# numericalEFT/MCIntegration.jl

Measured on AMD Instinct MI355X. Metric: Msamples/sec (whole node), 16-D Gaussian :vegas, higher is better.
Workload: dtype f64

## Files before the change

### include/mci.h

```cpp
#ifndef MCI_H
#define MCI_H

#include <stdint.h>

#ifdef __cplusplus
extern "C" {
#endif

#define MCI_OK 0
#define MCI_ERR_INVALID 1
#define MCI_ERR_HIP 2
#define MCI_ERR_COMPILE 3
#define MCI_ERR_NORMALIZATION 4
#define MCI_ERR_HISTOGRAM 5
#define MCI_ERR_COMM 6
#define MCI_ERR_NO_DEVICE 7

enum { MCI_CONTINUOUS = 0, MCI_DISCRETE = 1, MCI_FERMIK = 2 };
enum { MCI_VEGAS = 0, MCI_VEGASMC = 1, MCI_MCMC = 2 };
enum { MCI_VEGAS_PERSISTENT = 3 };
enum { MCI_VEGASMC_LANES = 5, MCI_MCMC_LANES = 6 };
enum { MCI_VEGAS_STRAT = 7 };
enum { MCI_VEGAS_SWEEP = 8 };
enum { MCI_VEGAS_SWEEP_LEAVES = 9 };
enum { MCI_VEGAS_SWEEP_STRAT = 10 };
enum { MCI_VEGASMC_SWEEP = 11 };
enum { MCI_MCMC_SWEEP = 12 };
enum { MCI_VEGASMC_SWEEP_CARRY = 13, MCI_MCMC_SWEEP_CARRY = 14 };
enum { MCI_SWEEP_ONE_GRID = 0, MCI_SWEEP_ALL_LEAVES = 1 };

typedef struct mci_ctx mci_ctx;
typedef struct mci_problem mci_problem;

typedef struct {
    int32_t kind;
    int32_t pool;
    double lower, upper;
    int32_t npoints;
    double alpha;
    int32_t adapt;
    const double *init;
} mci_leaf_desc;

typedef struct {
    int32_t nleaf;
    const mci_leaf_desc *leaves;
    int32_t npool;
    int32_t nintegrand;
    const int32_t *dof;
    const int32_t *obs_nbin;
    const int32_t *obs_bin_draw;
    const int32_t *neighbor_offsets;
    const int32_t *neighbor_list;
    int32_t ncomp;
} mci_problem_desc;

typedef struct {
    int32_t solver;
    int64_t neval;
    int32_t niter;
    int64_t block;
    int32_t ignore;
    int32_t adapt;
    double gamma;
    int64_t measurefreq;
    uint64_t seed;
    int64_t nchain;
    int32_t first_iteration;
    double thermal_ratio;
    const double *reweight_goal;
} mci_integrate_args;

typedef struct {
    int32_t niter, nobs;
    double *iter_mean;
    double *iter_std;
    double *mean;
    double *stdev;
    double *chi2;
    int64_t neval;
    double seconds;
    double *visited;
    int32_t correlated;
    int32_t warmup;
} mci_result;

int mci_ctx_create(int32_t device, mci_ctx **out);
int mci_ctx_destroy(mci_ctx *ctx);
const char *mci_last_error(void);
int mci_device_count(int32_t *count);
void *mci_ctx_stream(mci_ctx *ctx);

int mci_comm_unique_id(void *id128);
int mci_comm_init(mci_ctx *ctx, int32_t rank, int32_t nranks, const void *id128);
int mci_comm_rank(const mci_ctx *ctx, int32_t *rank, int32_t *nranks);
int mci_comm_sum(mci_problem *prob, double *v, int32_t n);

int mci_problem_create(mci_ctx *ctx, const mci_problem_desc *desc, mci_problem **out);
int mci_problem_destroy(mci_problem *prob);
int mci_set_integrand_source(mci_problem *prob, const char *body, const double *userdata, int32_t nuserdata);
typedef int (*mci_host_integrand_fn)(const double *x, double *w, int64_t n, int32_t ndraw, int32_t nw, void *user);
int mci_set_integrand_host(mci_problem *prob, mci_host_integrand_fn fn, void *user);
typedef int (*mci_host_integrand_idx_fn)(const int32_t *idx, const double *x, double *w, int64_t n, int32_t ndraw, int32_t ncomp, void *user);
int mci_set_integrand_host_indexed(mci_problem *prob, mci_host_integrand_idx_fn fn, void *user);
int mci_set_measure_source(mci_problem *prob, const char *body);
typedef int (*mci_host_measure_fn)(const double *x, const double *relw, int64_t n, int64_t stride, int32_t ndraw, int32_t nw,
                                   int64_t block, double *obs, int32_t nobs, void *user);
int mci_set_measure_host(mci_problem *prob, mci_host_measure_fn fn, void *user);
typedef int (*mci_host_measure_idx_fn)(const int32_t *idx, const double *x, const double *relw, int64_t n, int64_t stride, int32_t ndraw,
                                       int32_t ncomp, int64_t block, double *obs, int32_t nobs, void *user);
int mci_set_measure_host_indexed(mci_problem *prob, mci_host_measure_idx_fn fn, void *user);
int mci_compile(mci_problem *prob);
int mci_compile_solver(mci_problem *prob, int32_t solver);
int mci_kernel_code_object(mci_problem *prob, int32_t solver, char *buf, int32_t n);
int mci_set_launch(mci_problem *prob, int32_t threads_per_workgroup, int32_t workgroups_per_block);
int mci_problem_info(const mci_problem *prob, int32_t *ndraw, int32_t *nobs, int64_t *packed_size,
                     int32_t *table_mode, int64_t *lds_bytes);
int mci_get_histogram_copies(const mci_problem *prob, int32_t *copies);

int mci_iteration_run(mci_problem *prob, int32_t solver, int64_t neval_per_block, int64_t block_lo,
                      int64_t block_hi, int32_t iteration, uint64_t seed, int64_t measurefreq, int64_t nchain,
                      double thermal_ratio);
int mci_iteration_reduce(mci_problem *prob);
int mci_iteration_finish(mci_problem *prob, int32_t solver, int64_t block_total, int32_t adapt, double gamma,
                         double *mean, double *std);
int mci_check_status(mci_problem *prob);
int mci_integrate(mci_problem *prob, const mci_integrate_args *args, mci_result *result);
int mci_integrate_sweep(mci_problem *prob, const mci_integrate_args *args, int32_t npoint, const double *userdata, const uint64_t *seeds,
                        const double *maps_in, double *maps_out, mci_result *results, double *iter_mean, double *iter_std,
                        int32_t *status);
int mci_sweep_supported(const mci_problem *prob, const mci_integrate_args *args, char *why, int32_t n);
int mci_set_sweep_leaves(mci_problem *prob, int32_t mode);
int mci_set_sweep_chain_carry(mci_problem *prob, int32_t on);
int mci_get_sweep_chain_carry(const mci_problem *prob, int32_t *on);
int mci_sweep_map_doubles(const mci_problem *prob, int32_t *n);
int mci_integrate_sweep_strat(mci_problem *prob, const mci_integrate_args *args, int32_t npoint, const double *userdata, const uint64_t *seeds,
                              const double *maps_in, double *maps_out, const double *d_in, double *d_out, int64_t *counts_out,
                              mci_result *results, double *iter_mean, double *iter_std, int32_t *status);
int mci_sweep_strat_supported(const mci_problem *prob, const mci_integrate_args *args, char *why, int32_t n);
int mci_sweep_strat_doubles(const mci_problem *prob, const mci_integrate_args *args, int64_t *ncube);
int mci_integrate_sweep_chains(mci_problem *prob, const mci_integrate_args *args, int32_t npoint, const double *userdata, const uint64_t *seeds,
                               const double *maps_in, double *maps_out, const double *reweight_in, double *reweight_out, double *pa_out,
                               mci_result *results, double *iter_mean, double *iter_std, int32_t *status);
int mci_sweep_chains_supported(const mci_problem *prob, const mci_integrate_args *args, char *why, int32_t n);
int mci_integrate_sweep_mcmc(mci_problem *prob, const mci_integrate_args *args, int32_t npoint, const double *userdata, const uint64_t *seeds,
                             const double *maps_in, double *maps_out, const double *reweight_in, double *reweight_out, double *pa_out,
                             uint64_t *holds_out, mci_result *results, double *iter_mean, double *iter_std, int32_t *status);
int mci_sweep_mcmc_supported(const mci_problem *prob, const mci_integrate_args *args, char *why, int32_t n);

int mci_get_hold_histogram(mci_problem *prob, uint64_t *out64);
int mci_mcmc_launch_valid(mci_problem *prob, int32_t *valid, int32_t *warm, int64_t *chain_len, int64_t *hold_max);
int mci_iteration_discard(mci_problem *prob);
int mci_get_iteration_log(mci_problem *prob, int32_t nrows, double *out);
int mci_get_block_means(mci_problem *prob, int32_t rows, double *out, int64_t *nblocks, int32_t *carried);
int mci_reset_block_log(mci_problem *prob);
int mci_reserve_iteration_log(mci_problem *prob, int32_t rows);
int mci_get_packed(mci_problem *prob, double *out, int64_t n);
int mci_set_packed(mci_problem *prob, const double *in, int64_t n);
void *mci_packed_device_ptr(mci_problem *prob);
int mci_get_grid(mci_problem *prob, int32_t leaf, double *out, int32_t n);
int mci_set_grid(mci_problem *prob, int32_t leaf, const double *grid, int32_t n);
int mci_get_distribution(mci_problem *prob, int32_t leaf, double *distribution, double *accumulation, int32_t k);
int mci_set_distribution(mci_problem *prob, int32_t leaf, const double *distribution, int32_t k);
int mci_get_reweight(mci_problem *prob, double *out, int32_t n);
int mci_set_reweight(mci_problem *prob, const double *in, int32_t n);
int mci_set_reweight_goal(mci_problem *prob, const double *goal, int32_t n);
int mci_get_acceptance(mci_problem *prob, double *propose, double *accept, int32_t n);
int mci_save_state(mci_problem *prob, const char *path);
int mci_load_state(mci_problem *prob, const char *path);
int mci_set_rng_bits(mci_problem *prob, int32_t bits);
int mci_set_rng_rounds(mci_problem *prob, int32_t rounds);
int mci_set_train_walk(mci_problem *prob, int32_t mode);
int mci_set_deterministic(mci_problem *prob, int32_t on);
int mci_set_chain_carry(mci_problem *prob, int32_t mode);
int mci_set_stratification(mci_problem *prob, int32_t ndim, const int32_t *nstrat, double beta, int64_t max_nhcube);
int mci_set_stratification_carry(mci_problem *prob, int32_t on);
int mci_get_strat_carry(const mci_problem *prob, int32_t *on, int32_t *how);
int mci_set_stratification_off(mci_problem *prob);
int mci_get_stratification(const mci_problem *prob, int32_t *nstrat, int64_t *ncube, double *beta);
int mci_get_strat_counts(mci_problem *prob, int64_t *n_h, int64_t n);
int mci_strat_plan(int64_t neval, int32_t ndim, int64_t max_nhcube, int32_t *nstrat);
// ... 47 lines not shown
```

### mcintegration.jl_amd/csrc/mci_host_check.h

```cpp

namespace {
struct CheckLayout {
    std::vector<mci::CheckDraw> draw;
    std::vector<mci::CheckIntegrand> intg;
};
bool vegas_check_covers(const mci_problem *p) {
    const auto &s = p->shape;
    if (s.host_integrand || s.host_measure || s.ntile != 1 || p->has_fermik || p->strat.on) return false;
    for (int i = 0; i < s.ni; ++i)
        if (s.ncomp != 1 && s.obs_bin_draw[(size_t)i] >= 0) return false;
    return s.ndraw >= 1 && s.ndraw <= 64;
}
void vegas_check_layout(const mci_problem *p, CheckLayout *out) {
    const auto &s = p->shape;
    CheckLayout &L = *out;
    for (int k = 0; k < s.ndraw; ++k) {
        const int leaf = s.draw_leaf[(size_t)k];
        mci::CheckDraw d{};
        d.kind = s.leaf_kind[(size_t)leaf];
        d.off = s.leaf_eoff[(size_t)leaf];
        d.doff = s.leaf_doff[(size_t)leaf];
        d.nbin = s.leaf_nbin[(size_t)leaf];
        d.boff = s.leaf_boff[(size_t)leaf];
        d.hist = (s.leaf_adapt[(size_t)leaf] != 0 && s.cover_mask[(size_t)k] != 0ull) ? 1 : 0;
        d.scale = d.kind == 0 ? (double)d.nbin : 1.0;
        d.lower = s.leaf_lower[(size_t)leaf];
        L.draw.push_back(d);
    }
    for (int i = 0; i < s.ni; ++i) {
        mci::CheckIntegrand g{};
        g.own = s.own_mask[(size_t)i];
        g.obs_off = s.obs_off[(size_t)i];
        g.obs_nbin = s.obs_nbin[(size_t)i];
        g.obs_bin_draw = s.obs_bin_draw[(size_t)i];
        L.intg.push_back(g);
    }
}
struct DevFree {
    void *p = nullptr;
    ~DevFree() { if (p) (void)hipFree(p); }
};
}

static int sample_dump_device(mci_problem *p, int32_t iteration, uint64_t seed, int64_t first_index, int64_t n);

static int vegas_make_conservative(mci_problem *p, int slot) {
    p->vegas.make_conservative(p->deterministic);
    if (!p->deterministic) p->shape.hcopy = 1;
    p->kernel[MCI_VEGAS].drop();
    p->kernel[kSlotVegasAny].drop();
    p->vegas_check_done[0] = p->vegas_check_done[1] = false;
    return compile_solver(p, slot);
}

static int vegas_check_reference(mci_problem *p, int32_t iteration, uint64_t seed, int64_t nevalperblock, int64_t block_lo, int64_t nblocks,
                                 int64_t measurefreq, const double *hx, const double *hjac, const double *hw, double *packed, int64_t *bad,
                                 bool hist_offsets) {
    const auto &s = p->shape;
    if (!vegas_check_covers(p)) return fail(MCI_ERR_INVALID, "this layout has no static :vegas check (host closures, several histogram tiles, stratification)");
    if (nblocks < 1 || nevalperblock < 1 || nblocks * nevalperblock > 1024 || measurefreq < 1) return fail(MCI_ERR_INVALID, "the static :vegas check runs 1..1024 samples per launch");
    HIPCHK(hipSetDevice(p->ctx->device));
    hipStream_t st = p->ctx->stream;
    CheckLayout L;
    vegas_check_layout(p, &L);
    const int nw = s.ni * s.ncomp;
    const int64_t n = nevalperblock, per = s.ndraw + 1 + nw;
    const size_t nraw = (size_t)nblocks * s.ncols + (size_t)(s.nbin ? s.nbin : 1);
    DevFree d_draw, d_intg, d_raw, d_bad, d_in;
    HIPCHK(hipMalloc(&d_draw.p, L.draw.size() * sizeof(mci::CheckDraw)));
    HIPCHK(hipMalloc(&d_intg.p, L.intg.size() * sizeof(mci::CheckIntegrand)));
    HIPCHK(hipMalloc(&d_raw.p, nraw * sizeof(double)));
    HIPCHK(hipMalloc(&d_bad.p, 2 * sizeof(unsigned long long)));
    HIPCHK(hipMemcpyAsync(d_draw.p, L.draw.data(), L.draw.size() * sizeof(mci::CheckDraw), hipMemcpyHostToDevice, st));
    HIPCHK(hipMemcpyAsync(d_intg.p, L.intg.data(), L.intg.size() * sizeof(mci::CheckIntegrand), hipMemcpyHostToDevice, st));
    HIPCHK(hipMemsetAsync(d_raw.p, 0, nraw * sizeof(double), st));
    HIPCHK(hipMemsetAsync(d_bad.p, 0, 2 * sizeof(unsigned long long), st));
    if (hx) HIPCHK(hipMalloc(&d_in.p, (size_t)(nblocks * n * per) * sizeof(double)));
    mci::CheckArgs a{};
    a.draw = (const mci::CheckDraw *)d_draw.p;
    a.intg = (const mci::CheckIntegrand *)d_intg.p;
    a.ndraw = s.ndraw;
    a.ni = s.ni;
    a.ncomp = s.ncomp;
    a.nobs = s.nobs;
    a.ncols = s.ncols;
    a.rng_bits = s.rng_bits;
    a.rng_rounds = s.rng_rounds;
    a.with_obs = s.measure_body.empty() ? 1 : 0;
    fill_tables(p, a);
    a.seed = seed;
    a.iteration = (unsigned)iteration;
    a.neval_per_block = nevalperblock;
    a.measurefreq = measurefreq;
    a.hist = (double *)d_raw.p + (size_t)nblocks * s.ncols;
    a.bad = (unsigned long long *)d_bad.p;
    const int64_t total = nblocks * n;
    if (hx) {
        double *in = (double *)d_in.p;
        HIPCHK(hipMemcpyAsync(in, hx, (size_t)total * s.ndraw * sizeof(double), hipMemcpyHostToDevice, st));
        HIPCHK(hipMemcpyAsync(in + total * s.ndraw, hjac, (size_t)total * sizeof(double), hipMemcpyHostToDevice, st));
        HIPCHK(hipMemcpyAsync(in + total * (s.ndraw + 1), hw, (size_t)total * nw * sizeof(double), hipMemcpyHostToDevice, st));
        a.x = in;
    } else {
        if (int rc = sample_dump_device(p, iteration, seed, block_lo * nevalperblock, total)) return rc;
        p->check_launches += 1;
        a.x = p->d_dump;
    }
    a.jac = a.x + total * s.ndraw;
    a.w = a.jac + total;
    a.block_lo = block_lo;
    a.n = total;
    a.cols = (double *)d_raw.p;
    hipLaunchKernelGGL(mci::k_check_vegas, dim3((unsigned)((total + 255) / 256)), dim3(256), 0, st, a);
    HIPCHK(hipGetLastError());
    p->check_launches += 1;
    std::vector<double> raw(nraw);
    unsigned long long hbad[2] = {0ull, 0ull};
    HIPCHK(hipMemcpyAsync(raw.data(), d_raw.p, nraw * sizeof(double), hipMemcpyDeviceToHost, st));
    HIPCHK(hipMemcpyAsync(hbad, d_bad.p, sizeof(hbad), hipMemcpyDeviceToHost, st));
    HIPCHK(hipStreamSynchronize(st));
    if (bad) {
        bad[0] = (int64_t)hbad[0];
        bad[1] = (int64_t)hbad[1];
    }
    const int nobs = s.nobs, cnorm = nobs, cneval = nobs + 1, cvis = nobs + 2;
    for (int64_t i = 0; i < p->packed_n; ++i) packed[i] = 0.0;
    double norm = 1.0e-10, neval = 0.0;
    for (int64_t b = 0; b < nblocks; ++b) {
        const double *row = raw.data() + (size_t)b * s.ncols;
        const double nb = row[cnorm] + 1.0e-10;
        for (int o = 0; o < nobs; ++o) {
            const double m = row[o] / nb;
            packed[o] += m;
            packed[nobs + o] += m * m;
        }
        norm += nb;
        neval += row[cneval];
    }
    packed[2 * nobs] = norm;
    packed[2 * nobs + 1] = neval;
    for (int i = 0; i < s.ni + 1; ++i) {
        double v = 1.0e-8;
        for (int64_t b = 0; b < nblocks; ++b) v += raw[(size_t)b * s.ncols + cvis + i] + 1.0e-8;
        packed[2 * nobs + 2 + i] = v;
    }
    for (int i = 0; i < s.nbin; ++i) packed[p->nstat + i] = (hist_offsets ? (double)(nblocks + 1) * 1.0e-10 : 0.0) + raw[(size_t)nblocks * s.ncols + i];
    for (int e = 0; e < 2 * p->npa && p->nstat + s.nbin + e < p->packed_n; ++e)
        packed[p->nstat + s.nbin + e] = (double)(nblocks + 1) * (e < p->npa ? 1.0e-8 : 1.0e-10);
    return MCI_OK;
}

static int vegas_check_round(mci_problem *p, int slot, int64_t npb, int64_t block_lo, int64_t nb, int32_t iteration, uint64_t seed, int64_t mf, PackedDiff *df,
                             int64_t *bad, bool *differs) {
    std::vector<double> got((size_t)p->packed_n, 0.0), ref((size_t)p->packed_n, 0.0);
    p->check_slot = slot;
    int rc = mci_iteration_run(p, MCI_VEGAS, npb, block_lo, block_lo + nb, iteration, seed, mf, 1, 0.0);
    p->check_slot = -1;
    if (!rc) p->check_launches += 1;
    if (!rc) rc = mci_get_packed(p, got.data(), p->packed_n);
    if (!rc) rc = vegas_check_reference(p, iteration, seed, npb, block_lo, nb, mf, nullptr, nullptr, nullptr, ref.data(), bad, false);
    if (rc) return rc;
    const size_t skip = p->shape.measure_body.empty() ? 0 : (size_t)(2 * p->shape.nobs);
    compare_packed(got.data(), ref.data(), (size_t)p->nstat, (size_t)p->packed_n, skip, df, (long)p->shape.nbin);
    *differs = df->bad != 0 || bad[0] != 0 || bad[1] != 0;
    return MCI_OK;
}

static int vegas_self_check(mci_problem *p, int slot, int64_t nevalperblock, int64_t block_lo, int64_t block_hi, int32_t iteration, uint64_t seed,
                            int64_t measurefreq) {
    const int u = slot == kSlotVegasAny ? 1 : 0;
    const int64_t nb = block_hi - block_lo < 2 ? block_hi - block_lo : 2, npb = nevalperblock < 512 ? nevalperblock : 512;
    const int64_t mf = measurefreq * 4 <= npb ? measurefreq : 1;
    const mci_problem::LaunchState saved = p->launch;
    const int kernel_timing = p->kernel_timing;
    int rc = flush_merge(p);
    if (rc) return rc;
    int h_status[4] = {0, 0, 0, 0};
    HIPCHK(hipStreamSynchronize(p->ctx->stream));
    HIPCHK(hipMemcpy(h_status, p->d_status, sizeof(h_status), hipMemcpyDeviceToHost));
    p->in_self_check = true;
    p->kernel_timing = 0;
    if (!p->shape.measure_body.empty()) p->vegas_check_flags |= 1;
    int state = 0;
    for (int round = 0; round < 2 && !rc; ++round) {
        PackedDiff df;
        int64_t bad[2] = {0, 0};
        bool differs = false;
        const std::string object = p->kernel[slot].code_object;
        rc = vegas_check_round(p, slot, npb, block_lo, nb, iteration, seed, mf, &df, bad, &differs);
        if (rc) break;
        if (!differs) {
            state = round == 0 ? 1 : -1;
            bool takes = false;
            for (int k = 0; k < p->shape.ndraw; ++k)
                takes = takes || (p->shape.leaf_adapt[(size_t)p->shape.draw_leaf[(size_t)k]] != 0 && p->shape.cover_mask[(size_t)k] != 0ull);
            if (takes && !(df.hist_top > 0.0)) {
                p->vegas_check_flags |= 4;
                if (round == 0) state = 0;
                break;
            }
            const std::string id = mcijit::compiler_id() + "\n";
            mcijit::write_file_atomic(object + ".ok", id.data(), id.size());
            break;
        }
        fprintf(stderr, "mci: the :vegas sample kernel of this problem (%s%s) does not reproduce the library's static :vegas kernel on a %lld-block, "
                        "%lld-sample check: %ld of %lld packed entries differ (first at %ld; statistics %ld, histogram %ld), draws of %lld samples and "
                        "Jacobians of %lld differ.  A miscompiled code object -- %s; mci_vegas_check_status reports %d.\n",
                object.c_str(), round ? ", the conservative layout" : "", (long long)nb, (long long)npb, df.bad, (long long)p->packed_n, df.first_bad,
                df.bad_sec[0], df.bad_sec[1], (long long)bad[0], (long long)bad[1],
                round ? "no layout of this unit agrees, its results are not to be trusted" : "the problem compiles its :vegas units again in the plain layout (plain loop, one histogram copy)",
                round ? -2 : -1);
        state = -2;
        if (round == 0) {
            rc = vegas_make_conservative(p, slot);
        }
    }
    p->in_self_check = false;
    p->launch = saved;
    p->kernel_timing = kernel_timing;
    if (p->d_status) (void)hipMemcpy(p->d_status, h_status, sizeof(h_status), hipMemcpyHostToDevice);
    p->merge.hist_no_offset = 0;
    p->vegas_check_done[u] = true;
    if (rc) {
        fprintf(stderr, "mci: the self-check of this problem's :vegas code object (%s) could not run: %s -- nothing was verified "
                        "(mci_vegas_check_status stays %d)\n", p->kernel[slot].code_object.c_str(), mci_last_error(), state == -2 ? -2 : 0);
        p->merge_pending = false;
        if (state == -2) p->vegas_check_state[u] = -2;
        return MCI_OK;
    }
    p->vegas_check_state[u] = state;
    return MCI_OK;
}

static int vegas_check_gate(mci_problem *p, int slot, int64_t nevalperblock, int64_t block_lo, int64_t block_hi, int32_t iteration, uint64_t seed,
                            int64_t measurefreq) {
    const int u = slot == kSlotVegasAny ? 1 : 0;
    const bool force = g_over.vegas_self_check.on && g_over.vegas_self_check.v == 1;
    if (g_over.vegas_self_check.on && g_over.vegas_self_check.v == 0) return MCI_OK;
    if (!vegas_check_covers(p) || p->ctx->offline) {
        p->vegas_check_done[u] = true;
        return MCI_OK;
    }
    if (!force && access((p->kernel[slot].code_object + ".ok").c_str(), F_OK) == 0) {
        if (p->vegas_check_state[u] == 0) {
            p->vegas_check_state[u] = 1;
            p->vegas_check_flags |= 2;
        }
        p->vegas_check_done[u] = true;
        return MCI_OK;
    }
    return vegas_self_check(p, slot, nevalperblock, block_lo, block_hi, iteration, seed, measurefreq);
}

int mci_vegas_check_status(const mci_problem *p, int32_t *status, int32_t *flags) {
    if (!p || !status) return fail(MCI_ERR_INVALID, "NULL argument");
    const int a = p->vegas_check_state[0], b = p->vegas_check_state[1];
    *status = (a < 0 || b < 0) ? (a < b ? a : b) : (a > b ? a : b);
    if (flags) *flags = p->vegas_check_flags;
    return MCI_OK;
}

int mci_debug_vegas_check(mci_problem *p, int32_t iteration, uint64_t seed, int64_t nevalperblock, int64_t block_lo, int64_t nblocks, int64_t measurefreq,
                          const double *x, const double *jac, const double *w, double *packed, int64_t *bad) {
    if (!p || !packed) return fail(MCI_ERR_INVALID, "NULL argument");
    if (p->ctx->offline) return fail(MCI_ERR_NO_DEVICE, "offline context");
    if ((x || jac || w) && !(x && jac && w)) return fail(MCI_ERR_INVALID, "x, jac and w come together");
    int rc = flush_merge(p);
    if (rc) return rc;
    return vegas_check_reference(p, iteration, seed, nevalperblock, block_lo, nblocks, measurefreq, x, jac, w, packed, bad, true);
}

int mci_debug_vegas_check_launches(const mci_problem *p, int64_t *launches) {
    if (!p || !launches) return fail(MCI_ERR_INVALID, "NULL argument");
    *launches = p->check_launches;
    return MCI_OK;
}

int mci_debug_vegas_check_layout(const mci_problem *p, int32_t *head, int32_t *draws, double *scales, uint64_t *own, int32_t *obs) {
    if (!p || !head) return fail(MCI_ERR_INVALID, "NULL argument");
    const auto &s = p->shape;
    CheckLayout L;
    vegas_check_layout(p, &L);
    head[0] = s.ndraw;
    head[1] = s.ni;
    head[2] = s.ncomp;
    head[3] = s.nobs;
    head[4] = s.ncols;
    head[5] = s.nbin;
    head[6] = vegas_check_covers(p) ? 1 : 0;
    head[7] = s.measure_body.empty() ? 1 : 0;
    for (size_t k = 0; k < L.draw.size(); ++k) {
        if (draws) {
            const mci::CheckDraw &d = L.draw[k];
            const int v[6] = {d.kind, d.off, d.doff, d.nbin, d.boff, d.hist};
            for (int j = 0; j < 6; ++j) draws[6 * k + j] = v[j];
        }
        if (scales) scales[k] = L.draw[k].scale;
    }
    for (size_t i = 0; i < L.intg.size(); ++i) {
        if (own) own[i] = L.intg[i].own;
        if (obs) {
            obs[3 * i] = L.intg[i].obs_off;
            obs[3 * i + 1] = L.intg[i].obs_nbin;
            obs[3 * i + 2] = L.intg[i].obs_bin_draw;
        }
    }
    return MCI_OK;
}
```

### mcintegration.jl_amd/csrc/mci_host_iteration.h

```cpp

static int reserve_launch_buffers(mci_problem *p, const LaunchRequest &rq, const LaunchPlan &pl) {
    const auto &s = p->shape;
    int rc = ensure_capacity(p, pl.nrows, rq.nblocks);
    if (!rc && rq.solver != MCI_VEGAS) rc = p->d_part_pa.reserve(pl.nrows * 2 * p->npa);
    if (rc || !pl.split) return rc;
    const int64_t words = p->tdraw_words > 0 ? p->tdraw_words : 1, bytes = parked_bytes_per_sample(p);
    const int64_t nsamp = rq.nblocks * pl.chunk_len;
    if (nsamp > p->cap_tile) {
        tile_release(p);
        const size_t wbytes = (((size_t)nsamp * s.ni * sizeof(double)) + 255) & ~(size_t)255;
        if ((rc = tile_alloc(p, wbytes + (size_t)nsamp * words * sizeof(uint32_t)))) return rc;
        p->d_tile_bins = (uint32_t *)((char *)p->d_tile_w + wbytes);
        p->cap_tile = nsamp;
    }
    p->launch.last_split_chunks = pl.nchunks;
    p->launch.last_split_bytes = nsamp * bytes;
    return MCI_OK;
}

static mci::BatchArgs request_args(const mci_problem *p, const LaunchRequest &rq, const LaunchPlan &pl) {
    mci::BatchArgs a{};
    fill_batch(p, a);
    a.part_pa = p->d_part_pa;
    a.seed = rq.seed;
// ... 185 lines not shown
    if ((rc = p->d_hx.reserve(n * s.ndraw)) || (rc = p->d_hw.reserve(n * s.ni * s.ncomp)) || (rc = p->h_hx.reserve(n * s.ndraw)) ||
        (rc = p->h_hw.reserve(n * s.ni * s.ncomp)))
        return rc;
    if (rq.solver == MCI_VEGAS) {
    mci::DumpArgs d{};
    fill_tables(p, d);
    d.ud = p->d_ud;
    d.x = p->d_hx;
    d.soa = 1;
    d.seed = rq.seed;
    d.iteration = (mci::u32)rq.iteration;
    d.first_index = rq.block_lo * rq.nevalperblock;
    d.n = n;
    void *dargs[] = {&d};
    const unsigned dgrid = (unsigned)((n + 255) / 256 < 4096 ? (n + 255) / 256 : 4096);
    hipStream_t hs = p->ctx->stream;
    HIPCHK(hipModuleLaunchKernel(p->kernel[kSlotDump].f, dgrid, 1, 1, 256, 1, 1, (unsigned)p->lds_bytes, hs, dargs, nullptr));
    HIPCHK(hipMemcpyAsync(p->h_hx, p->d_hx, (size_t)n * s.ndraw * sizeof(double), hipMemcpyDeviceToHost, hs));
    HIPCHK(hipStreamSynchronize(hs));
    if ((rc = eval_host_integrand(p, nullptr, p->h_hx, p->h_hw, n))) return rc;
    HIPCHK(hipMemcpyAsync(p->d_hw, p->h_hw, (size_t)n * s.ni * s.ncomp * sizeof(double), hipMemcpyHostToDevice, hs));
    }
    a.host_w = p->d_hw;
    return MCI_OK;
}

static int prepare_host_measure(mci_problem *p, const LaunchRequest &rq, const LaunchPlan &pl, mci::BatchArgs &a) {
    const auto &s = p->shape;
    const int nw = s.ni * s.ncomp;
    const int64_t n = rq.nblocks * pl.hm_n > 0 ? rq.nblocks * pl.hm_n : 1;
    if ((double)n * (double)(s.ndraw + nw + 1) * 8.0 > 8.0 * 1024 * 1024 * 1024)
        return fail(MCI_ERR_INVALID, "a host measure over %lld records of %d doubles per launch (more than 8 GiB): lower neval, raise measurefreq "
                                     "or give the measure as device source (mci_set_measure_source)", (long long)n, s.ndraw + nw);
    int rc;
    if ((rc = p->d_mx.reserve(n * s.ndraw)) || (rc = p->d_mrelw.reserve(n * nw)) || (rc = p->d_midx.reserve(n)) || (rc = p->h_mx.reserve(n * s.ndraw)) ||
        (rc = p->h_mrelw.reserve(n * nw)) || (rc = p->h_midx.reserve(n)) || (rc = p->d_mobs.reserve(rq.nblocks * s.nobs)))
        return rc;
    a.host_mx = p->d_mx;
    a.host_relw = p->d_mrelw;
    a.host_midx = p->d_midx;
    a.hm_first = pl.hm_first;
    a.hm_count = pl.hm_count;
    a.hm_stride = rq.nblocks * pl.hm_n;
    if (rq.solver != MCI_VEGAS) {
        HIPCHK(hipMemsetAsync(p->d_mx, 0, (size_t)n * s.ndraw * sizeof(double), p->ctx->stream));
        HIPCHK(hipMemsetAsync(p->d_mrelw, 0, (size_t)n * pl.hm_rows * sizeof(double), p->ctx->stream));
        HIPCHK(hipMemsetAsync(p->d_midx, 0xFF, (size_t)n * sizeof(int32_t), p->ctx->stream));
    }
    return MCI_OK;
}

static int prepare_cursor(mci_problem *p, const LaunchRequest &rq, const LaunchPlan &pl, mci::BatchArgs &a) {
    mci::CursorRule r;
    r.units = (mci::u64)((rq.nevalperblock + 127) >> 7);
    r.waves = (mci::u32)(pl.wpb * (pl.T / 64));
    r.log2_big = (mci::u32)(g_over.cursor_log2_big.on && g_over.cursor_log2_big.v >= 1 && g_over.cursor_log2_big.v <= 16 ? g_over.cursor_log2_big.v : mci_problem::kCursorLog2Big);
    r.ones = (mci::u32)(g_over.cursor_ones.on && g_over.cursor_ones.v >= 1 && g_over.cursor_ones.v <= 4096 ? g_over.cursor_ones.v : mci_problem::kCursorOnes);
    if (rq.nblocks != p->cursor_nblocks) {
        if (int rc = p->d_cursor.reserve(rq.nblocks * mci::kCursorStride)) return rc;
        HIPCHK(hipMemsetAsync(p->d_cursor, 0, (size_t)rq.nblocks * mci::kCursorStride * sizeof(unsigned long long), p->ctx->stream));
        p->cursor_nblocks = rq.nblocks;
        p->cursor_base = 0;
    }
    a.cursor = p->d_cursor;
    a.cursor_base = p->cursor_base;
    a.cursor_log2_big = r.log2_big;
    a.cursor_ones = r.ones;
    p->cursor_base += mci::cursor_tickets(r) + r.waves;
    return MCI_OK;
}

static int launch_host_closure_steps(mci_problem *p, const LaunchRequest &rq, const LaunchPlan &pl, mci::BatchArgs &a, hipFunction_t f) {
    const auto &s = p->shape;
    hipStream_t st = p->ctx->stream;
    void *args[] = {&a};
    int rc;
    const int64_t nc = rq.nblocks * pl.nchain, steps = rq.nevalperblock / pl.nchain;
    const int nw = s.ni * s.ncomp, nd = s.ndraw;
    if (nc >= ((int64_t)1 << 31) || steps + pl.nburn >= ((int64_t)1 << 31) - 1) return fail(MCI_ERR_INVALID, "too many chains or steps for the host-closure path");
    if ((rc = p->d_hstep.reserve(nc * (int64_t)((3 * nd + nw + 4) * sizeof(double) + (2 * nd + 7) * sizeof(int)) + 16)) || (rc = p->h_hidx.reserve(nc + 1))) return rc;
    {
        double *dp = (double *)p->d_hstep.get();
        a.hs.cx = dp; dp += (size_t)nd * nc;
        a.hs.cprob = dp; dp += (size_t)nd * nc;
        a.hs.pprob = dp; dp += (size_t)nd * nc;
        a.hs.cw = dp; dp += (size_t)nw * nc;
        a.hs.cprobability = dp; dp += nc;
        a.hs.pprop = dp; dp += nc;
        a.hs.puacc = dp; dp += nc;
        a.hs.cwabs = dp; dp += nc;
        int *ip = (int *)dp;
        a.hs.cbin = ip; ip += (size_t)nd * nc;
        a.hs.pbin = ip; ip += (size_t)nd * nc;
        a.hs.pvi = ip; ip += nc;
        a.hs.ccurr = ip; ip += nc;
        a.hs.cit = ip; ip += nc;
        a.hs.ctr = ip; ip += nc;
        a.hs.pnew = ip; ip += nc;
        a.hs.put = ip; ip += nc;
        a.hs.hidx = ip; ip += nc;
        a.hs.done = ip;
    }
    a.hs.hx = p->d_hx;
    a.hs.nc = nc;
    a.hs.steps = steps;
    HIPCHK(hipMemsetAsync(p->d_part_cols, 0, (size_t)pl.nrows * s.ncols * sizeof(double), st));
    if (pl.hist_lds && s.nbin > 0) HIPCHK(hipMemsetAsync(p->d_part_hist, 0, (size_t)pl.nrows * s.nbin * sizeof(double), st));
    HIPCHK(hipMemsetAsync(p->d_part_pa, 0, (size_t)pl.nrows * 2 * p->npa * sizeof(double), st));
    HIPCHK(hipMemsetAsync(a.hs.done, 0, sizeof(int), st));
    if (rq.solver == MCI_VEGASMC) {
        for (int64_t ne = 0; ne <= steps + 1; ++ne) {
            a.hs.ne = ne;
            HIPCHK(hipModuleLaunchKernel(f, (unsigned)pl.nwg, 1, 1, (unsigned)pl.T, 1, 1, (unsigned)solver_lds(p, rq.solver), st, args, nullptr));
            if (ne > steps) break;
            HIPCHK(hipMemcpyAsync(p->h_hx, p->d_hx, (size_t)nc * nd * sizeof(double), hipMemcpyDeviceToHost, st));
            HIPCHK(hipStreamSynchronize(st));
            if ((rc = eval_host_integrand(p, nullptr, p->h_hx, p->h_hw, nc))) return rc;
            HIPCHK(hipMemcpyAsync(p->d_hw, p->h_hw, (size_t)nc * nw * sizeof(double), hipMemcpyHostToDevice, st));
        }
    } else {
        const int64_t limit = steps + pl.nburn + 2 + 10000;
        for (int64_t ne = 0;; ++ne) {
            a.hs.ne = ne;
            HIPCHK(hipModuleLaunchKernel(f, (unsigned)pl.nwg, 1, 1, (unsigned)pl.T, 1, 1, (unsigned)solver_lds(p, rq.solver), st, args, nullptr));
            HIPCHK(hipMemcpyAsync(p->h_hidx, a.hs.hidx, (size_t)(nc + 1) * sizeof(int32_t), hipMemcpyDeviceToHost, st));
            HIPCHK(hipMemcpyAsync(p->h_hx, p->d_hx, (size_t)nc * nd * sizeof(double), hipMemcpyDeviceToHost, st));
            HIPCHK(hipStreamSynchronize(st));
            if (p->h_hidx[nc] >= nc) break;
            if (ne > limit) return fail(MCI_ERR_INVALID, "host-closure :mcmc chains did not finish (%d of %lld)", (int)p->h_hidx[nc], (long long)nc);
            if ((rc = eval_host_integrand(p, p->h_hidx, p->h_hx, p->h_hw, nc))) return rc;
            HIPCHK(hipMemcpyAsync(p->d_hw, p->h_hw, (size_t)nc * s.ncomp * sizeof(double), hipMemcpyHostToDevice, st));
        }
    }
    return MCI_OK;
}

static int launch_replay(mci_problem *p, const LaunchRequest &rq, const LaunchPlan &pl, mci::BatchArgs &a) {
    const auto &s = p->shape;
    void *args[] = {&a};
    HIPCHK(hipModuleLaunchKernel(p->f_tiles[rq.kern == kSlotVegasAny ? 1 : 0], (unsigned)(((pl.hist_rows + 7) / 8) * 8 * (s.ntile - (s.split_all ? 0 : 1))), 1, 1, (unsigned)pl.T, 1, 1, (unsigned)p->lds_bytes, p->ctx->stream, args, nullptr));
    return MCI_OK;
}

static int launch_sample_chunks(mci_problem *p, const LaunchRequest &rq, const LaunchPlan &pl, mci::BatchArgs &a, hipFunction_t f) {
    hipStream_t st = p->ctx->stream;
    void *args[] = {&a};
    int rc;
    for (int64_t c = 0; c < pl.nchunks; ++c) {
        if (pl.nchunks > 1) {
            a.chunk_lo = c * pl.chunk_len;
            a.chunk_hi = a.chunk_lo + pl.chunk_len < rq.nevalperblock ? a.chunk_lo + pl.chunk_len : rq.nevalperblock;
            a.accum = c > 0 ? 1 : 0;
        }
        HIPCHK(hipModuleLaunchKernel(f, (unsigned)pl.nwg, 1, 1, (unsigned)pl.T_launch, 1, 1, (unsigned)solver_lds(p, rq.solver), st, args, nullptr));
        if (pl.split && c + 1 < pl.nchunks && (rc = launch_replay(p, rq, pl, a))) return rc;
    }
    return MCI_OK;
}

static int finish_host_measure(mci_problem *p, const LaunchRequest &rq, const LaunchPlan &pl) {
    const auto &s = p->shape;
    hipStream_t st = p->ctx->stream;
    const int64_t n = rq.nblocks * pl.hm_n;
    const int nw = s.ni * s.ncomp, nc = s.ncomp;
    std::vector<double> obs((size_t)rq.nblocks * s.nobs, 0.0);
    if (n > 0 && !p->in_self_check) {
        HIPCHK(hipMemcpyAsync(p->h_mx, p->d_mx, (size_t)n * s.ndraw * sizeof(double), hipMemcpyDeviceToHost, st));
        HIPCHK(hipMemcpyAsync(p->h_mrelw, p->d_mrelw, (size_t)n * pl.hm_rows * sizeof(double), hipMemcpyDeviceToHost, st));
        if (rq.solver == MCI_MCMC) HIPCHK(hipMemcpyAsync(p->h_midx, p->d_midx, (size_t)n * sizeof(int32_t), hipMemcpyDeviceToHost, st));
        HIPCHK(hipStreamSynchronize(st));
        const double *relw = p->h_mrelw;
        if (rq.solver == MCI_MCMC && p->hmeas_fn) {
            p->h_mtmp.assign((size_t)n * nw, 0.0);
            for (int64_t i = 0; i < n; ++i)
                if (p->h_midx[i] >= 0)
                    for (int q = 0; q < nc; ++q) p->h_mtmp[(size_t)(p->h_midx[i] * nc + q) * n + i] = p->h_mrelw[(size_t)q * n + i];
            relw = p->h_mtmp.data();
        }
        if (rq.solver != MCI_MCMC && p->hmeas_idx_fn) p->h_mitmp.resize((size_t)pl.hm_n);
        const bool squeeze = rq.solver == MCI_VEGAS && rq.measurefreq > 1;
        const int64_t keep = squeeze ? rq.nevalperblock / rq.measurefreq : pl.hm_n;
        std::vector<double> sx, sw;
        if (squeeze) {
            sx.resize((size_t)(keep > 0 ? keep : 1) * s.ndraw);
            sw.resize((size_t)(keep > 0 ? keep : 1) * nw);
        }
        for (int64_t b = 0; b < rq.nblocks; ++b) {
            const int64_t off = b * pl.hm_n;
            double *ob = obs.data() + (size_t)b * s.nobs;
            int hrc = 0;
            if (squeeze) {
                for (int k = 0; k < s.ndraw; ++k)
                    for (int64_t j = 0; j < keep; ++j) sx[(size_t)k * keep + j] = p->h_mx[(size_t)k * n + off + (j + 1) * rq.measurefreq - 1];
                for (int q = 0; q < nw; ++q)
                    for (int64_t j = 0; j < keep; ++j) sw[(size_t)q * keep + j] = relw[(size_t)q * n + off + (j + 1) * rq.measurefreq - 1];
                if (p->hmeas_fn) hrc = p->hmeas_fn(sx.data(), sw.data(), keep, keep, s.ndraw, nw, rq.block_lo + b, ob, s.nobs, p->hmeas_user);
                else {
                    p->h_mitmp.resize((size_t)(keep > 0 ? keep : 1));
                    for (int j = 0; j < s.ni && !hrc; ++j) {
                        std::fill(p->h_mitmp.begin(), p->h_mitmp.end(), (int32_t)j);
                        hrc = p->hmeas_idx_fn(p->h_mitmp.data(), sx.data(), sw.data() + (size_t)j * nc * keep, keep, keep, s.ndraw, nc, rq.block_lo + b, ob,
                                              s.nobs, p->hmeas_user);
                    }
                }
            } else if (p->hmeas_fn) {
                hrc = p->hmeas_fn(p->h_mx + off, relw + off, pl.hm_n, n, s.ndraw, nw, rq.block_lo + b, ob, s.nobs, p->hmeas_user);
            } else if (rq.solver == MCI_MCMC) {
                hrc = p->hmeas_idx_fn(p->h_midx + off, p->h_mx + off, relw + off, pl.hm_n, n, s.ndraw, nc, rq.block_lo + b, ob, s.nobs, p->hmeas_user);
            } else {
                for (int j = 0; j < s.ni && !hrc; ++j) {
                    std::fill(p->h_mitmp.begin(), p->h_mitmp.end(), (int32_t)j);
                    hrc = p->hmeas_idx_fn(p->h_mitmp.data(), p->h_mx + off, relw + (size_t)j * nc * n + off, pl.hm_n, n, s.ndraw, nc, rq.block_lo + b, ob,
                                          s.nobs, p->hmeas_user);
                }
            }
            if (hrc) return fail(MCI_ERR_INVALID, "the host measure failed (%d)", hrc);
        }
    }
    HIPCHK(hipMemcpyAsync(p->d_mobs, obs.data(), obs.size() * sizeof(double), hipMemcpyHostToDevice, st));
    hipLaunchKernelGGL(mci::k_add_host_obs, dim3((unsigned)((rq.nblocks * s.nobs + 255) / 256)), dim3(256), 0, st, p->d_mobs, (int)rq.nblocks, s.nobs, s.ncols, pl.wpb,
                       p->d_part_cols);
    HIPCHK(hipGetLastError());
    HIPCHK(hipStreamSynchronize(st));
    return MCI_OK;
}

static int queue_merge(mci_problem *p, const LaunchRequest &rq, const LaunchPlan &pl, const unsigned long long *hold_hist) {
    const auto &s = p->shape;
    hipStream_t st = p->ctx->stream;
    int rc;
    const int nb256 = (s.nbin + 255) / 256;
    if (pl.hist_lds && s.nbin > 0 && !pl.atomic_flush)
        hipLaunchKernelGGL(mci::k_hist_stage1, dim3(nb256, mci_problem::kGroups), dim3(256), 0, st, p->d_part_hist, (int)pl.hist_rows, s.nbin,
                           (int)mci_problem::kGroups, p->d_stage1);
    HIPCHK(hipGetLastError());
    mci::MergeArgs &m = p->merge;
    m = merge_args(p, rq.nblocks, pl.wpb, pl.nrows);
    m.use_ghist = (pl.hist_lds && !pl.atomic_flush) ? 0 : pl.atomic_flush ? pl.ghist_buffers : 1;
    m.part_pa = rq.solver != MCI_VEGAS ? p->d_part_pa.get() : nullptr;
    m.hist_no_offset = (p->in_self_check && p->check_slot >= 0) ? 1 : 0;
    m.hold = hold_hist;
    if (rq.solver != MCI_VEGAS && !p->in_self_check) {
        const int64_t stride = rq.nblocks * s.nobs;
        if (stride != p->launch.blk_stride || rq.block_lo != p->launch.blk_lo) {
            p->launch.blk_rows = 0;
            p->launch.blk_carried = 0;
            p->launch.blk_stride = stride;
            p->launch.blk_lo = rq.block_lo;
        }
        if ((rc = grow_block_log(p, p->launch.blk_rows + 1))) return rc;
        m.block_means = p->d_blocklog + (size_t)p->launch.blk_rows * stride;
        p->launch.blk_rows += 1;
        p->launch.blk_carried += p->launch.last_carried ? 1 : 0;
    }
    p->merge_pending = true;
    return MCI_OK;
}

int mci_iteration_run(mci_problem *p, int32_t solver, int64_t nevalperblock, int64_t block_lo, int64_t block_hi,
                      int32_t iteration, uint64_t seed, int64_t measurefreq, int64_t nchain, double thermal_ratio) {
    if (p->ctx->offline) return fail(MCI_ERR_NO_DEVICE, "offline context: no device to run on");
    if (solver != MCI_VEGAS && solver != MCI_VEGASMC && solver != MCI_MCMC) return fail(MCI_ERR_INVALID, "Solver %d is not supported!", solver);
    if (measurefreq <= 0) return fail(MCI_ERR_INVALID, "measurefreq must be positive");
    const int64_t nblocks = block_hi - block_lo;
    if (nblocks < 1 || nevalperblock < 1) return fail(MCI_ERR_INVALID, "empty iteration");
    if (p->has_fermik && solver != MCI_MCMC) return fail(MCI_ERR_INVALID, "FermiK variables work with solver=:mcmc only");
    if (p->strat.on) {
        if (solver != MCI_VEGAS) return fail(MCI_ERR_INVALID, "stratification works with solver = :vegas only (mci_set_stratification_off first)");
        return strat_run(p, nevalperblock, block_lo, block_hi, iteration, seed, measurefreq);
    }
    const int kern = (p->in_self_check && p->check_slot >= 0 && solver == MCI_VEGAS) ? p->check_slot : kslot(solver, measurefreq);
    const LaunchRequest rq{solver, nevalperblock, block_lo, block_hi, nblocks, iteration, seed, measurefreq, thermal_ratio, nchain <= 0, kern};
    int rc = (rq.solver == MCI_VEGAS || p->deterministic || p->shape.host_integrand || p->spec_lanes == 1) ? compile_solver(p, rq.kern) : MCI_OK;
    if (rc) return rc;
    if (rq.solver == MCI_VEGAS && !p->in_self_check && !p->vegas_check_done[rq.kern == kSlotVegasAny ? 1 : 0] &&
        (rc = vegas_check_gate(p, rq.kern, rq.nevalperblock, rq.block_lo, rq.block_hi, rq.iteration, rq.seed, rq.measurefreq)))
        return rc;
    if (rq.solver == MCI_VEGAS && (rc = compile_solver(p, rq.kern))) return rc;
    if (rq.solver == MCI_VEGAS && p->shape.host_integrand && (rc = ensure_dump(p))) return rc;
    if ((rc = flush_merge(p))) return rc;
    HIPCHK(hipSetDevice(p->ctx->device));
    const auto &s = p->shape;
    LaunchPlan pl;
    pl.nchain = nchain;
    plan_threads(p, rq, pl);
    pl.units = nevalperblock;
    if (rq.solver != MCI_VEGAS && (rq.block_hi > 4096 || rq.iteration >= 131072 || rq.iteration < 0))
        return fail(MCI_ERR_INVALID, "chain solvers address a chain by (block < 4096, iteration < 131072): got block_hi=%lld, iteration=%d",
                    (long long)rq.block_hi, (int)rq.iteration);
    pl.may_carry = plan_may_carry(p, rq);
    if (solver == MCI_VEGASMC) rc = plan_vegasmc_chains(p, rq, g_over, pl);
    else if (solver == MCI_MCMC) {
        if (!(rq.thermal_ratio >= 0.0)) return fail(MCI_ERR_INVALID, "thermal_ratio must be non-negative");
        if (rq.auto_chains && (rc = hold_consume(p))) return rc;
        rc = plan_mcmc_chains(p, rq, pl);
    } else pl.nchain = 1;
    if (rc) return rc;
    plan_spec_lanes(p, rq, pl);
    pl.T_launch = pl.T;
    if (pl.G > 1 && p->spec_state[rq.solver - 1] < 0) pl.G = 1;
    if (pl.G > 1) {
        rc = compile_spec(p, rq.solver);
        if (rc == MCI_ERR_COMPILE && p->spec_lanes == -1) {
            fprintf(stderr, "mci: the several-lanes-per-chain kernel of this problem did not compile; one lane per chain instead\n%s\n", mci_last_error());
            p->spec_state[rq.solver - 1] = -2;
            pl.G = 1;
        } else if (rc) return rc;
    }
    if (pl.G > 1 && !p->in_self_check && ((p->spec_need_check[rq.solver - 1] && !(g_over.spec_self_check.on && g_over.spec_self_check.v == 0)) ||
                                       (g_over.spec_self_check.on && g_over.spec_self_check.v == 1 && p->spec_state[rq.solver - 1] == 0))) {
        if ((rc = spec_self_check(p, rq.solver, pl.G, rq.nevalperblock, rq.block_lo, rq.block_hi, rq.iteration, rq.seed, rq.measurefreq, rq.thermal_ratio))) return rc;
        if (p->spec_state[rq.solver - 1] < 0) pl.G = 1;
    }
    if (pl.G > 1) {
        if ((rc = spec_upload(p, rq.solver, pl.G, p->spec_accept, p->spec_maxacc))) return rc;
        pl.spec_maxacc = p->spec_tab_maxacc;
        pl.units = pl.nchain * pl.G;
        pl.T_launch = pl.units >= 256 ? 256 : (int)((pl.units + 63) / 64) * 64;
    }
    if (pl.G == 1 && (rc = compile_solver(p, rq.kern))) return rc;
    p->launch.last_spec_lanes = pl.G;
    p->launch.last_spec_maxacc = pl.spec_maxacc;
    plan_grid(p, rq, pl);
    if (const int candidate = plan_cursor_candidate(p, rq, g_over, pl)) {
        int resident = 0;
        if (candidate == 1) pl.cursor = true;
        else if ((rc = cursor_resident(p, rq.kern, pl.T, &resident))) return rc;
        else plan_cursor_grid(rq, resident, pl);
    }
    plan_tiles(p, rq, g_over, pl);
    plan_replay(p, rq, pl);
    plan_host_measure(p, rq, pl);
    plan_timing(p, rq, pl);
    if ((rc = reserve_launch_buffers(p, rq, pl))) return rc;
    mci::BatchArgs a = request_args(p, rq, pl);
    if (solver != MCI_VEGAS && (rc = prepare_carried_chains(p, rq, pl, a))) return rc;
    if ((rc = prepare_chain_tables(p, rq, pl, a))) return rc;
    geometry_args(p, rq, pl, a);
    if (s.host_integrand && (rc = prepare_host_integrand(p, rq, pl, a))) return rc;
    if (s.host_measure && (rc = prepare_host_measure(p, rq, pl, a))) return rc;
    if (pl.cursor && (rc = prepare_cursor(p, rq, pl, a))) return rc;
    p->launch.last_cursor = pl.cursor;
    hipFunction_t f = p->kernel[pl.G > 1 ? (rq.solver == MCI_VEGASMC ? kSlotVegasmcSpec : kSlotMcmcSpec) : rq.kern].f;
    hipStream_t st = p->ctx->stream;
    const int slot = (int)(p->launch.launches % mci_problem::kEvRing);
    p->launch.time_this_launch = pl.time_this_launch;
    if (p->launch.time_this_launch && rq.solver == MCI_VEGAS) {
        if (!p->d_clocks) {
            if ((rc = p->d_clocks.reserve(2 * mci_problem::kEvRing))) return rc;
            HIPCHK(hipMemsetAsync(p->d_clocks, 0, (size_t)2 * mci_problem::kEvRing * sizeof(unsigned long long), st));
        }
        a.clock_out = p->d_clocks + 2 * slot;
    }
    if (p->launch.time_this_launch) HIPCHK(hipEventRecord(p->evs[2 * slot], st));
    if (solver != MCI_VEGAS && s.host_integrand) rc = launch_host_closure_steps(p, rq, pl, a, f);
    else rc = launch_sample_chunks(p, rq, pl, a, f);
    if (rc) return rc;
    if (rq.solver == MCI_MCMC) p->launch.hold_measured = a.hold_hist != nullptr;
    if (a.hold_hist && rq.auto_chains && (rc = hold_publish(p, rq.nevalperblock / pl.nchain, rq.solver != MCI_VEGAS && p->launch.last_carried))) return rc;
    if (pl.split && (rc = launch_replay(p, rq, pl, a))) return rc;
    if (p->launch.time_this_launch) HIPCHK(hipEventRecord(p->evs[2 * slot + 1], st));
    p->launch.ev_valid[slot] = p->launch.time_this_launch;
    p->launch.clock_valid[slot] = a.clock_out != nullptr && !pl.split && s.ntile == 1;
    p->launch.launches += 1;
    if (s.host_measure && (rc = finish_host_measure(p, rq, pl))) return rc;
    record_launch(p, nblocks * nevalperblock, pl.nwg, pl.T_launch, nblocks);
    if (solver != MCI_VEGAS) p->launch.last_nchain = pl.nchain;
    return queue_merge(p, rq, pl, a.hold_hist);
}

static int flush_merge(mci_problem *p) {
    if (!p->merge_pending) return MCI_OK;
    p->merge_pending = false;
    HIPCHK(hipSetDevice(p->ctx->device));
    const int nb256 = (p->shape.nbin + 255) / 256;
    hipLaunchKernelGGL(mci::k_finalize, dim3(nb256 + 1 + (2 * p->npa + 3) / 4), dim3(256), 0, p->ctx->stream, p->merge);
    HIPCHK(hipGetLastError());
    return MCI_OK;
}

int mci_iteration_reduce(mci_problem *p) {
    if (p->ctx->offline) return fail(MCI_ERR_NO_DEVICE, "offline context");
    if (!p->ctx->comm) return MCI_OK;
    int rc = flush_merge(p);
    if (rc) return rc;
    const bool timed = p->launch.time_this_launch;
    const int slot = (int)(p->reduces % mci_problem::kCevRing);
    if (timed) {
        if (p->cevs.empty()) {
            p->cevs.resize(2 * mci_problem::kCevRing);
            for (auto &e : p->cevs) HIPCHK(hipEventCreate(&e));
        }
        HIPCHK(hipEventRecord(p->cevs[2 * slot], p->ctx->stream));
    }
    const size_t count = (size_t)p->packed_n + (p->launch.hold_deferred ? 64 : 0);
    int r = g_rccl.AllReduce(p->d_packed, p->d_packed, count, kNcclFloat64, kNcclSum, p->ctx->comm, p->ctx->stream);
    if (r) return fail(MCI_ERR_COMM, "ncclAllReduce: %s", g_rccl.GetErrorString ? g_rccl.GetErrorString(r) : "?");
    p->ctx->collectives += 1;
    p->ctx->last_count = (long long)count;
    if (p->launch.hold_deferred && (rc = hold_publish_reduced(p))) return rc;
    if (timed) HIPCHK(hipEventRecord(p->cevs[2 * slot + 1], p->ctx->stream));
    p->cev_valid[slot] = timed;
    p->reduces += 1;
    return MCI_OK;
}

int mci_comm_collectives(const mci_ctx *c, int64_t *calls, int64_t *last_count) {
    if (!c) return fail(MCI_ERR_INVALID, "NULL argument");
    if (calls) *calls = c->collectives;
    if (last_count) *last_count = c->last_count;
    return MCI_OK;
}

int mci_external_reduce_done(mci_problem *p) {
    if (!p) return fail(MCI_ERR_INVALID, "NULL argument");
    if (p->ctx->offline) return fail(MCI_ERR_NO_DEVICE, "offline context");
    if (!p->launch.hold_ext_pending) return MCI_OK;
    p->launch.hold_ext_pending = false;
    HIPCHK(hipSetDevice(p->ctx->device));
    return hold_publish_reduced(p);
}

int mci_reduce_size(const mci_problem *p, int64_t *n) {
    if (!p || !n) return fail(MCI_ERR_INVALID, "NULL argument");
    *n = p->packed_n + 64;
    return MCI_OK;
}

int mci_comm_times_ms(mci_problem *p, float *ms, int32_t n, int32_t *got) {
    if (!p || !ms || !got) return fail(MCI_ERR_INVALID, "NULL argument");
    if (p->ctx->offline) return fail(MCI_ERR_NO_DEVICE, "offline context");
    HIPCHK(hipStreamSynchronize(p->ctx->stream));
    int64_t have = p->reduces < mci_problem::kCevRing ? p->reduces : mci_problem::kCevRing;
    if (have > n) have = n;
    int32_t k = 0;
    for (int64_t i = 0; i < have; ++i) {
        const int slot = (int)((p->reduces - have + i) % mci_problem::kCevRing);
        if (!p->cev_valid[slot]) continue;
        float t = 0.f;
        HIPCHK(hipEventElapsedTime(&t, p->cevs[2 * slot], p->cevs[2 * slot + 1]));
        ms[k++] = t;
    }
    *got = k;
    return MCI_OK;
}

static int launch_train(mci_problem *p, int do_train, int do_reweight, double gamma, double *log_row) {
    const auto &s = p->shape;
    int maxn = 1;
    for (auto &L : p->leaves) maxn = L.nbin > maxn ? L.nbin : maxn;
    mci::TrainArgs a{};
    fill_train(p, a);
    a.iter_log_row = log_row;
    a.goal = p->h_goal.empty() ? nullptr : p->d_goal.get();
    a.do_reweight = do_reweight;
    a.gamma = gamma;
    a.do_train = do_train;
    if (do_train) p->ntrain += 1;
    a.serial_walk = p->train_serial >= 0 ? p->train_serial : (p->launch.last_samples == 0 || p->launch.last_samples >= mci_problem::kSerialWalkSamples) ? 1 : 0;
    if (p->debug_wrong_decision && a.serial_walk == 1) a.serial_walk = 3;
    a.maxn = maxn;
    a.spare = (size_t)(mci::train_lds_doubles(maxn) + mci::train_spare_doubles(maxn)) * sizeof(double) <= (size_t)kTrainLdsMax ? 1 : 0;
    const size_t sm = (size_t)(mci::train_lds_doubles(maxn) + (a.spare ? mci::train_spare_doubles(maxn) : maxn)) * sizeof(double);
    const unsigned tt = maxn > 256 ? 512u : 256u;
    if (sm > 64 * 1024 && !p->train_lds_raised) {
        HIPCHK(hipFuncSetAttribute((const void *)mci::k_train, hipFuncAttributeMaxDynamicSharedMemorySize, (int)kTrainLdsMax));
        HIPCHK(hipFuncSetAttribute((const void *)mci::k_finish, hipFuncAttributeMaxDynamicSharedMemorySize, (int)kTrainLdsMax));
        p->train_lds_raised = true;
    }
    if (p->merge_pending) {
        p->merge_pending = false;
        hipLaunchKernelGGL(mci::k_finish, dim3(s.nleaf + 1 + (2 * p->npa + 3) / 4), dim3(tt), sm, p->ctx->stream, p->merge, a);
    } else {
        hipLaunchKernelGGL(mci::k_train, dim3(s.nleaf + 1), dim3(tt), sm, p->ctx->stream, a);
    }
    HIPCHK(hipGetLastError());
    return MCI_OK;
}

static int grow_iteration_log(mci_problem *p, int64_t need) {
    return grow_keeping(p, p->d_iterlog, need, 64, p->nstat);
}

int mci_reserve_iteration_log(mci_problem *p, int32_t rows) {
    if (!p || rows < 0) return fail(MCI_ERR_INVALID, "bad argument");
    if (p->ctx->offline) return fail(MCI_ERR_NO_DEVICE, "offline context");
    HIPCHK(hipSetDevice(p->ctx->device));
    return grow_iteration_log(p, (int64_t)p->log_row + rows);
}

int mci_iteration_finish(mci_problem *p, int32_t solver, int64_t block_total, int32_t adapt, double gamma, double *mean, double *std) {
    if (p->ctx->offline) return fail(MCI_ERR_NO_DEVICE, "offline context");
    HIPCHK(hipSetDevice(p->ctx->device));
    const auto &s = p->shape;
    if (int grc = grow_iteration_log(p, (int64_t)p->log_row + 1)) return grc;
    double *row = p->d_iterlog + (size_t)p->log_row * p->nstat;
    const bool strat = p->strat.last_run;
    int rc = launch_train(p, adapt ? 1 : 0, (solver == MCI_VEGASMC || solver == MCI_MCMC) ? 1 : 0, gamma, row);
    if (rc) return rc;
    if (strat && (rc = strat_finish(p, row, adapt))) return rc;
    p->log_row += 1;
    if (mean || std) {
        std::vector<double> h(p->nstat);
        HIPCHK(hipMemcpyAsync(h.data(), row, (size_t)p->nstat * sizeof(double), hipMemcpyDeviceToHost, p->ctx->stream));
        if ((rc = check_status(p))) return rc;
        std::vector<double> m(s.nobs), e(s.nobs);
        if (strat) strat_mean_std(h.data(), s.nobs, m.data(), e.data());
        else
        mci_mean_std(h.data(), h.data() + s.nobs, s.nobs, block_total, m.data(), e.data());
        if (mean) memcpy(mean, m.data(), s.nobs * sizeof(double));
        if (std) memcpy(std, e.data(), s.nobs * sizeof(double));
    }
    return MCI_OK;
}

int mci_train(mci_problem *p) {
    if (p->ctx->offline) return fail(MCI_ERR_NO_DEVICE, "offline context");
    int rc = flush_merge(p);
    if (rc) return rc;
    rc = launch_train(p, 1, 0, 1.0, nullptr);
// ... 5 lines not shown
```

### mcintegration.jl_amd/csrc/mci_host_jit.h

```cpp
enum { kSlotVegasAny = 3, kSlotDump = 4, kSlotVegasmcSpec = 5, kSlotMcmcSpec = 6 };
static int kslot(int solver, int64_t measurefreq) { return solver == MCI_VEGAS && measurefreq != 1 ? kSlotVegasAny : solver; }
static int slot_solver(int slot) { return slot == kSlotVegasAny ? MCI_VEGAS : slot == kSlotVegasmcSpec ? MCI_VEGASMC : slot == kSlotMcmcSpec ? MCI_MCMC : slot; }

namespace {
struct Candidate {
    std::string src;
    int threads = 256;
    int unit = mcijit::kUnitSolver;
    std::vector<char> code;
    std::string log, path;
    bool cached = false;
    int rc = 0;
    long vgprs() const { return mcijit::kernel_vgprs(code, "mci_vegas_batch"); }
    long scratch() const { return mcijit::kernel_scratch_bytes(code, "mci_vegas_batch"); }
    int build(bool cache_only = false) { return rc = mcijit::compile(src, threads, code, log, cached, &path, unit, cache_only); }
    int failed(const std::string &of = "") const { return fail(MCI_ERR_COMPILE, "integrand failed to compile for gfx950%s:\n%s", of.c_str(), log.c_str()); }
};
void compile_all(const std::vector<Candidate *> &cs) {
    std::vector<std::thread> th;
    for (size_t i = 1; i < cs.size(); ++i) th.emplace_back([c = cs[i]] { c->build(); });
    if (!cs.empty()) cs[0]->build();
    for (auto &t : th) t.join();
}

int KernelUnit::load(const mci_ctx *ctx, Candidate &c, const char *kernel, int64_t lds, const Rules &rules) {
    const long static_lds = mcijit::max_static_lds_bytes(c.code);
    if (static_lds != 0 || (rules.no_scratch && mcijit::kernel_scratch_bytes(c.code, kernel) != 0)) {
        if (!rules.refusal.empty()) return fail(MCI_ERR_COMPILE, "%s", rules.refusal.c_str());
        return fail(MCI_ERR_COMPILE, "the code object declares static LDS (%ld bytes): the sample kernels expect their dynamic segment at LDS address 0", static_lds);
    }
    code_object = c.path;
    threads = c.threads;
    if (!ctx->offline) {
        HIPCHK(hipSetDevice(ctx->device));
        if (rules.stale == kFail) HIPCHK(hipModuleLoadData(&module, c.code.data()));
        else if (hipModuleLoadData(&module, c.code.data()) != hipSuccess) {
            if (c.cached) unlink(c.path.c_str());
            if (!c.cached || rules.stale == kUnlinkAndFail) return fail(MCI_ERR_HIP, "hipModuleLoadData failed for %s", rules.what.c_str());
            if (c.build()) return c.failed();
            HIPCHK(hipModuleLoadData(&module, c.code.data()));
        }
        if (int rc = entry(&f, kernel, lds)) return rc;
    }
    compiled = true;
    return MCI_OK;
}
}

static const KernelUnit::Rules kSlotRules = {KernelUnit::kRecompileOnce, false, "", "a freshly compiled code object"};
static const char *unit_kernel(int unit, int solver) {
    if (const char *k = mcijit::kUnits[unit].kernel) return k;
    if (unit == mcijit::kUnitDump) return "mci_sample_dump";
    if (unit == mcijit::kUnitSpec) return solver == MCI_VEGASMC ? "mci_vegasmc_spec" : "mci_mcmc_spec";
    return solver == MCI_VEGAS ? "mci_vegas_batch" : solver == MCI_VEGASMC ? "mci_vegasmc_chains" : "mci_mcmc_chains";
}
static int load_slot(mci_problem *p, int slot, Candidate &c, int64_t lds) {
    KernelUnit &u = p->kernel[slot];
    if (int rc = u.load(p->ctx, c, unit_kernel(c.unit, slot_solver(slot)), lds, kSlotRules)) return rc;
    if (p->ctx->offline) return MCI_OK;
    if (slot == MCI_VEGASMC || slot == kSlotVegasmcSpec)
        if (int rc = u.entry(&p->f_carryw[slot == MCI_VEGASMC ? 0 : 1], "mci_vegasmc_carry_weights", lds)) return rc;
    if (slot_solver(slot) == MCI_VEGAS && slot != kSlotDump && p->shape.ntile > 1)
        if (int rc = u.entry(&p->f_tiles[slot == kSlotVegasAny ? 1 : 0], "mci_vegas_tiles", p->lds_bytes)) return rc;
    return MCI_OK;
}

static int ensure_dump(mci_problem *p) {
    if (p->kernel[kSlotDump].compiled) return MCI_OK;
    Candidate c;
    mcijit::ProblemShape sh = p->shape;
    sh.hcopy = 1;
    sh.det = 0;
    c.unit = mcijit::kUnitDump;
    c.src = mcijit::generate_source(sh, MCI_VEGAS, mcijit::kUnitDump);
    c.threads = 256;
    if (c.build()) return c.failed();
    return load_slot(p, kSlotDump, c, p->lds_bytes);
}

static int default_measure_fits(const mci_problem *p) {
    for (int i = 0; i < p->ni && p->shape.measure_body.empty() && !p->shape.host_measure; ++i)
        if (p->shape.obs_bin_draw[i] < 0 && p->shape.obs_nbin[i] != p->shape.ncomp)
            return fail(MCI_ERR_INVALID, "the default measure can only handle observable as Vector with %d scalar elements!", p->ni);
    return MCI_OK;
}

static const char *const kVegasPlainLoop = "#define MCI_VEGAS_PLAIN_LOOP 1\n";
static const char *const kVgprKeys = "#define MCI_PIPE_VGPR_KEYS 1\n";
static int compile_solver(mci_problem *p, int slot) {
    if (slot < 0 || slot > kSlotVegasAny) return fail(MCI_ERR_INVALID, "Solver %d is not supported!", slot);
    if (p->kernel[slot].compiled) return MCI_OK;
    const int solver = slot_solver(slot);
    const int unit = slot == MCI_VEGAS ? mcijit::kUnitVegasMf1 : mcijit::kUnitSolver;
    auto gen = [&](const mcijit::ProblemShape &sh, bool keys = false) {
        return std::string(keys ? kVgprKeys : "") + (p->vegas.conservative && solver == MCI_VEGAS ? kVegasPlainLoop : "") + mcijit::generate_source(sh, solver, unit);
    };
    if (int rc = default_measure_fits(p)) return rc;
    struct Built { VegasVariant v; Candidate c; };
    std::deque<Built> built;
    auto add = [&](const VegasVariant &v) {
        built.push_back({v, {}});
        Candidate &c = built.back().c;
        mcijit::ProblemShape sh = p->shape;
        sh.hcopy = v.copies;
        c.unit = unit;
        c.src = gen(sh, v.keys);
        c.threads = v.threads;
        return &c;
    };
    Candidate *chosen = nullptr;
    int64_t lds = p->lds_bytes;
    if (p->deterministic) {
        if (p->shape.ntile > 1 || p->shape.table_mode == 1 || p->shape.table_mode == 2 || p->shape.ec_doubles > 0)
            return fail(MCI_ERR_INVALID, "deterministic mode keeps one copy of the workgroup's histograms per wave in LDS: %d bins (%d tile(s)) do not fit",
                        p->shape.nbin, p->shape.ntile);
        int T = solver == MCI_VEGAS ? 512 : (p->threads < 512 ? p->threads : 512);
        while (T > 64 && det_lds(p, T) > 159 * 1024) T >>= 1;
        if (det_lds(p, T) > 159 * 1024) return fail(MCI_ERR_INVALID, "deterministic mode: the tables do not fit one CU's LDS");
        p->threads_det[solver] = T;
        p->shape.det = 1;
        p->shape.hcopy = T / 64;
        lds = det_lds(p, T);
    } else p->shape.det = 0;
    if (p->deterministic || solver != MCI_VEGAS) {
        chosen = add({p->shape.hcopy, false, p->deterministic ? p->threads_det[solver] : p->threads});
        if (chosen->build()) return chosen->failed();
    } else {
        const auto &s = p->shape;
        const VegasRuleIn in = {p->threads, p->threads_explicit, s.ndraw, s.host_integrand != 0, p->deterministic, g_over.hist_copies.on, sixteen_copies_fit(p), s.hcopy};
        size_t batch = 0;
        auto build = [&](const std::vector<VegasVariant> &vs, std::vector<VegasBuilt> &out) {
            batch = built.size();
            std::vector<Candidate *> cs;
            for (const VegasVariant &v : vs) cs.push_back(add(v));
            compile_all(cs);
            out.clear();
            for (Candidate *c : cs) out.push_back({c->rc ? 0 : c->vgprs(), c->rc ? 0 : c->scratch(), c->rc == 0});
        };
        VegasVariant v{};
        const int rc = vegas_kernel_rule(p->vegas, in, build, &v);
        p->shape.hcopy = v.copies;
        for (size_t i = batch; rc && i < built.size(); ++i)
            if (built[i].c.rc) return built[i].c.failed();
        for (Built &b : built)
            if (b.v.copies == v.copies && b.v.keys == v.keys && b.v.threads == v.threads) chosen = &b.c;
        lds = vegas_lds(p);
        if (s.ec_doubles > 0 && p->lds_bytes_k1 > lds) lds = p->lds_bytes_k1;
        if (p->lds_bytes > lds) lds = p->lds_bytes;
    }
    return load_slot(p, slot, *chosen, lds);
}

static int compile_spec(mci_problem *p, int solver) {
    const int slot = solver == MCI_VEGASMC ? kSlotVegasmcSpec : kSlotMcmcSpec;
    if (p->kernel[slot].compiled) return MCI_OK;
    if (int rc = default_measure_fits(p)) return rc;
    p->shape.det = 0;
    Candidate c, lane;
    c.unit = mcijit::kUnitSpec;
    c.src = mcijit::generate_source(p->shape, solver, mcijit::kUnitSpec);
    c.threads = 256;
    const bool cached = c.build(true) == 0;
    const bool verified = cached && access((c.path + ".ok").c_str(), F_OK) == 0;
    std::thread side;
    if (!verified && !p->kernel[solver].compiled && !p->ctx->offline && !(g_over.spec_self_check.on && g_over.spec_self_check.v == 0)) {
        lane.src = mcijit::generate_source(p->shape, solver, mcijit::kUnitSolver);
        lane.threads = p->threads;
        side = std::thread([&lane] { lane.build(); });
    }
    if (!cached) {
        if (c.build() == 2) {
            std::string log2;
            Candidate d;
            d.unit = c.unit;
            d.src = c.src;
            d.threads = c.threads;
            d.rc = mcijit::compile(d.src, d.threads, d.code, log2, d.cached, &d.path, mcijit::kUnitSpec, false, true);
            if (d.rc == 0) {
                d.log = c.log;
                c = std::move(d);
            }
        }
    }
    if (side.joinable()) side.join();
    if (c.rc) return c.failed();
    if (int rc = load_slot(p, slot, c, p->lds_bytes)) return rc;
    p->spec_need_check[solver - 1] = !verified;
    if (verified && p->spec_state[solver - 1] == 0) p->spec_state[solver - 1] = 1;
    return MCI_OK;
}

namespace {
struct PackedDiff {
    long bad = 0, first_bad = -1;
    long bad_sec[3] = {0, 0, 0};
    double worst = 0.0;
    double hist_top = 0.0;
};
void compare_packed(const double *x, const double *y, size_t nstat, size_t n, size_t skip, PackedDiff *out, long nhist = -1) {
    PackedDiff r;
    const size_t hend = nhist >= 0 ? nstat + (size_t)nhist : n;
    for (int sec = 0; sec < (nhist >= 0 ? 3 : 2); ++sec) {
        const size_t lo = sec == 0 ? skip : sec == 1 ? nstat : hend, hi = sec == 0 ? nstat : sec == 1 ? hend : n;
        const double tol = sec ? 1e-8 : 1e-9;
        double top = 0.0;
        for (size_t i = lo; i < hi; ++i) top = std::fmax(top, std::fmax(std::fabs(x[i]), std::fabs(y[i])));
        if (sec == 1 && nhist >= 0) r.hist_top = top;
        for (size_t i = lo; i < hi; ++i) {
            const double a = x[i], b = y[i];
            const double d = std::fabs(a - b), lim = tol * (std::fmax(std::fabs(a), std::fabs(b)) + 1e-3 * top);
            const bool ok = (std::isfinite(a) && std::isfinite(b)) ? d <= lim : (std::isnan(a) == std::isnan(b) && (std::isnan(a) || a == b));
            if (!ok) {
                if (r.first_bad < 0) r.first_bad = (long)i;
                ++r.bad;
                ++r.bad_sec[sec];
                if (top > 0.0 && d / top > r.worst) r.worst = d / top;
            }
        }
    }
    *out = r;
}
}

static int spec_self_check(mci_problem *p, int solver, int G, int64_t nevalperblock, int64_t block_lo, int64_t block_hi, int32_t iteration,
                           uint64_t seed, int64_t measurefreq, double thermal_ratio) {
    const int slot = solver == MCI_VEGASMC ? kSlotVegasmcSpec : kSlotMcmcSpec;
    const int64_t nb = block_hi - block_lo < 2 ? block_hi - block_lo : 2, npb = nevalperblock < 512 ? nevalperblock : 512;
    const int64_t mf = measurefreq * 4 <= npb ? measurefreq : 1;
    const mci_problem::LaunchState saved = p->launch;
    const int spec_lanes = p->spec_lanes, kernel_timing = p->kernel_timing;
    int rc = flush_merge(p);
    if (rc) return rc;
    int h_status[4] = {0, 0, 0, 0};
    HIPCHK(hipStreamSynchronize(p->ctx->stream));
    HIPCHK(hipMemcpy(h_status, p->d_status, sizeof(h_status), hipMemcpyDeviceToHost));
    std::vector<double> got[2];
    p->in_self_check = true;
    p->kernel_timing = 0;
    for (int pass = 0; pass < 2 && !rc; ++pass) {
        p->spec_lanes = pass == 0 ? G : 1;
        got[pass].assign((size_t)p->packed_n, 0.0);
        rc = mci_iteration_run(p, solver, npb, block_lo, block_lo + nb, iteration, seed, mf, 1, thermal_ratio);
        if (!rc) rc = mci_get_packed(p, got[pass].data(), p->packed_n);
    }
    p->in_self_check = false;
    p->launch = saved;
    p->spec_lanes = spec_lanes;
    p->kernel_timing = kernel_timing;
    if (p->d_status) (void)hipMemcpy(p->d_status, h_status, sizeof(h_status), hipMemcpyHostToDevice);
    if (rc) return rc;
    PackedDiff df;
    compare_packed(got[0].data(), got[1].data(), (size_t)(2 * p->shape.nobs + 2 + p->ni + 1), (size_t)p->packed_n, 0, &df);
    const long bad = df.bad, first_bad = df.first_bad;
    const double worst = df.worst;
    p->spec_need_check[solver - 1] = false;
    if (bad == 0) {
        p->spec_state[solver - 1] = 1;
        const std::string id = mcijit::compiler_id() + "\n";
        mcijit::write_file_atomic(p->kernel[slot].code_object + ".ok", id.data(), id.size());
        return MCI_OK;
    }
    p->spec_state[solver - 1] = -1;
    fprintf(stderr, "mci: the several-lanes-per-chain kernel of this problem (%s, %s) does not reproduce its lane-per-chain kernel on a %lld-block, %lld-step "
                    "check: %ld of %lld packed entries differ (first at %ld, largest difference %.3g of its section's maximum).  A miscompiled code object -- "
                    "this problem keeps one lane per chain (same chains, slower for launches of few chains); mci_chain_speculation_status reports -1.\n",
            solver == MCI_VEGASMC ? ":vegasmc" : ":mcmc", p->kernel[slot].code_object.c_str(), (long long)nb, (long long)npb, bad, (long long)p->packed_n, first_bad, worst);
    return MCI_OK;
}

static const int kSpecMaxLevels = 12;
static void spec_build(int lanes, double accept, int limit, std::vector<mci::SpecNode> &tab, int *maxacc) {
    struct Cand { double prob; int parent; bool via_acc; long seq; };
    std::vector<Cand> front;
    front.push_back({1.0, -1, false, 0});
    long seq = 1;
    tab.clear();
    *maxacc = 0;
    while ((int)tab.size() < lanes && !front.empty()) {
        size_t best = 0;
        for (size_t i = 1; i < front.size(); ++i)
            if (front[i].prob > front[best].prob || (front[i].prob == front[best].prob && front[i].seq < front[best].seq)) best = i;
        const Cand cd = front[best];
        front.erase(front.begin() + (long)best);
        mci::SpecNode nd{};
        if (cd.parent < 0) {
            nd.depth = 0;
            nd.anc = -1;
            nd.nacc = 0;
            nd.needacc = nd.needrej = nd.accdepth = 0ull;
        } else {
            const mci::SpecNode &pn = tab[(size_t)cd.parent];
            nd.depth = pn.depth + 1;
            nd.anc = cd.via_acc ? cd.parent : pn.anc;
            nd.nacc = pn.nacc + (cd.via_acc ? 1 : 0);
            nd.needacc = pn.needacc | (cd.via_acc ? 1ull << cd.parent : 0ull);
            nd.needrej = pn.needrej | (cd.via_acc ? 0ull : 1ull << cd.parent);
            nd.accdepth = pn.accdepth | (cd.via_acc ? 1ull << pn.depth : 0ull);
        }
        const int me = (int)tab.size();
        tab.push_back(nd);
        if (nd.nacc > *maxacc) *maxacc = nd.nacc;
        front.push_back({cd.prob * (1.0 - accept), me, false, seq++});
        if ((limit < 0 || nd.nacc + 1 <= limit) && nd.nacc + 1 <= kSpecMaxLevels) front.push_back({cd.prob * accept, me, true, seq++});
    }
    int deepest = 0;
    for (auto &nd : tab) deepest = nd.depth > deepest ? nd.depth : deepest;
    unsigned long long any = 0ull;
    for (auto &nd : tab) any |= nd.accdepth;
    for (auto &nd : tab) {
        nd.levels = *maxacc | (deepest << 8);
        nd.anydepth = any;
    }
}

static int spec_upload(mci_problem *p, int solver, int lanes, double accept, int limit) {
    const double key = accept > 0.0 ? accept : -(double)(solver + 1);
    if (p->d_spec_tab && p->spec_tab_lanes == lanes && p->spec_tab_accept == key && p->spec_tab_limit == limit) return MCI_OK;
    static const double fam_vegasmc[7] = {0.03, 0.12, 0.3, 0.5, 0.7, 0.85, 0.93}, fam_mcmc[6] = {0.03, 0.1, 0.2, 0.35, 0.55, 0.8};
    std::vector<mci::SpecNode> all;
    p->spec_ntree = 0;
    p->spec_tab_maxacc = 0;
    auto add = [&](double acc, int lim) {
        std::vector<mci::SpecNode> tab;
        int maxacc = 0;
        spec_build(lanes, acc, lim, tab, &maxacc);
        all.insert(all.end(), tab.begin(), tab.end());
        p->spec_accepts[p->spec_ntree++] = (float)acc;
        if (maxacc > p->spec_tab_maxacc) p->spec_tab_maxacc = maxacc;
    };
    if (accept > 0.0) {
        add(accept, limit);
        p->spec_first = 0;
    } else if (solver == MCI_VEGASMC) {
        for (double acc : fam_vegasmc) add(acc, limit);
        p->spec_first = 3;
    } else {
        for (double acc : fam_mcmc) add(acc, limit >= 0 ? limit : (acc >= 0.5 ? 3 : 2));
        p->spec_first = 3;
    }
    if (int rc = p->d_spec_tab.reserve(8 * 64)) return rc;
    HIPCHK(hipMemcpyAsync(p->d_spec_tab, all.data(), all.size() * sizeof(mci::SpecNode), hipMemcpyHostToDevice, p->ctx->stream));
    HIPCHK(hipStreamSynchronize(p->ctx->stream));
    p->spec_tab_lanes = lanes;
    p->spec_tab_accept = key;
    p->spec_tab_limit = limit;
    return MCI_OK;
}

int mci_set_chain_speculation(mci_problem *p, int32_t lanes, double accept, int32_t max_accepts) {
    if (!p) return fail(MCI_ERR_INVALID, "NULL argument");
    if (lanes != -1 && (lanes < 1 || lanes > 64 || (lanes & (lanes - 1)))) return fail(MCI_ERR_INVALID, "lanes per chain: -1 (automatic), 1 (one lane per chain) or a power of two up to 64");
    if (accept >= 1.0) return fail(MCI_ERR_INVALID, "the acceptance a speculation tree is built for lies in (0, 1); <= 0: the solver's default");
    p->spec_lanes = lanes;
    p->spec_accept = accept > 0.0 ? accept : 0.0;
    p->spec_maxacc = max_accepts < 0 ? -1 : max_accepts;
    return MCI_OK;
}

int mci_last_integrate_discarded(const mci_problem *p, int64_t *neval, int32_t *launches) {
    if (!p) return fail(MCI_ERR_INVALID, "NULL argument");
    if (neval) *neval = p->last_discarded_neval;
    if (launches) *launches = p->last_discarded_launches;
    return MCI_OK;
}

int mci_chain_speculation_status(const mci_problem *p, int32_t solver, int32_t *status) {
    if (!p || !status || (solver != MCI_VEGASMC && solver != MCI_MCMC)) return fail(MCI_ERR_INVALID, "solver MCI_VEGASMC or MCI_MCMC");
    *status = p->spec_state[solver - 1];
    return MCI_OK;
}

int mci_last_chain_speculation(const mci_problem *p, int32_t *lanes, int32_t *max_accepts) {
    if (!p) return fail(MCI_ERR_INVALID, "NULL argument");
    if (lanes) *lanes = p->launch.last_spec_lanes;
    if (max_accepts) *max_accepts = p->launch.last_spec_maxacc;
    return MCI_OK;
}

int mci_speculation_tree(int32_t lanes, double accept, int32_t max_accepts, int32_t *depth, int32_t *anc, int32_t *nacc, uint64_t *needacc, uint64_t *needrej) {
    if (lanes < 1 || lanes > 64 || !(accept > 0.0 && accept < 1.0)) return fail(MCI_ERR_INVALID, "speculation tree: 1..64 lanes, acceptance in (0, 1)");
    std::vector<mci::SpecNode> tab;
    int maxacc = 0;
    spec_build(lanes, accept, max_accepts, tab, &maxacc);
    for (int i = 0; i < lanes; ++i) {
        if (depth) depth[i] = tab[(size_t)i].depth;
        if (anc) anc[i] = tab[(size_t)i].anc;
        if (nacc) nacc[i] = tab[(size_t)i].nacc;
        if (needacc) needacc[i] = tab[(size_t)i].needacc;
        if (needrej) needrej[i] = tab[(size_t)i].needrej;
    }
    return MCI_OK;
}

int mci_compile_chain_speculation(mci_problem *p, int32_t solver) {
    if (!p) return fail(MCI_ERR_INVALID, "NULL argument");
    if (solver != MCI_VEGASMC && solver != MCI_MCMC) return fail(MCI_ERR_INVALID, "several lanes per chain: solver MCI_VEGASMC or MCI_MCMC");
    if (p->shape.host_integrand) return fail(MCI_ERR_INVALID, "a host integrand keeps one lane per chain");
    return compile_spec(p, solver);
}

int mci_compile(mci_problem *p) { return compile_solver(p, MCI_VEGAS); }

int mci_kernel_code_object(mci_problem *p, int32_t solver, char *buf, int32_t n) {
    if (!p || !buf || n < 1) return fail(MCI_ERR_INVALID, "NULL argument");
    int k = -1;
    std::string what = "solver " + std::to_string(solver);
    if (solver == MCI_VEGAS_PERSISTENT) k = mci_problem::kPersist, what = "the persistent :vegas kernel";
    else if (solver == MCI_VEGASMC_LANES || solver == MCI_MCMC_LANES) k = solver == MCI_VEGASMC_LANES ? kSlotVegasmcSpec : kSlotMcmcSpec, what = "the several-lanes-per-chain kernel";
    else if (solver == MCI_VEGAS_STRAT) k = mci_problem::kStrat, what = "the stratified :vegas kernel";
    else if (const int w = sweep_unit_of(solver); w >= 0) k = mci_problem::kSweep + w, what = std::string("the sweep kernel") + kSweepUnits[w].for_what;
    else if (solver < 0 || solver > 2) return fail(MCI_ERR_INVALID, "Solver %d is not supported!", solver);
    else k = (solver == MCI_VEGAS && !p->kernel[solver].compiled && p->kernel[kSlotVegasAny].compiled) ? kSlotVegasAny : solver;
    if (!p->kernel[k].compiled) return fail(MCI_ERR_INVALID, "%s has not been compiled yet", what.c_str());
    snprintf(buf, (size_t)n, "%s", p->kernel[k].code_object.c_str());
    return MCI_OK;
}

int mci_set_rng_bits(mci_problem *p, int32_t bits) {
    if (!p) return fail(MCI_ERR_INVALID, "NULL argument");
    if (bits != 52 && bits != 32) return fail(MCI_ERR_INVALID, "rng bits must be 52 (default: the resolution of rand(Float64)) or 32");
    if (p->shape.rng_bits != bits) {
        p->shape.rng_bits = bits;
        drop_modules(p);
    }
    return MCI_OK;
}

int mci_set_rng_rounds(mci_problem *p, int32_t rounds) {
    if (!p) return fail(MCI_ERR_INVALID, "NULL argument");
    if (rounds != 10 && rounds != 7) return fail(MCI_ERR_INVALID, "Philox4x32 rounds must be 10 (default) or 7 (the fewest that pass BigCrush)");
    if (p->shape.rng_rounds != rounds) {
        p->shape.rng_rounds = rounds;
        drop_modules(p);
    }
    return MCI_OK;
}

int mci_set_train_walk(mci_problem *p, int32_t mode) {
    if (!p) return fail(MCI_ERR_INVALID, "NULL argument");
    if (mode < -1 || mode > 2) return fail(MCI_ERR_INVALID, "train walk mode must be -1 (automatic), 0 (prefix scan), 1 (serial recurrence) or 2 (serial recurrence, general form only)");
    p->train_serial = mode;
    return MCI_OK;
}

int mci_debug_plant_wrong_decision(mci_problem *p, int32_t on) {
    if (!p) return fail(MCI_ERR_INVALID, "NULL argument");
    p->debug_wrong_decision = on != 0;
    return MCI_OK;
}

int mci_debug_override(const char *key, int64_t value, int32_t on) {
    Override *o = override_slot(key);
    if (!o) return fail(MCI_ERR_INVALID, "no such override: %s", key ? key : "(null)");
    o->on = on != 0;
    o->v = value;
    return MCI_OK;
}

int mci_debug_split_chunks(const mci_problem *p, int64_t *chunks, int64_t *bytes) {
    if (!p) return fail(MCI_ERR_INVALID, "NULL argument");
    if (chunks) *chunks = p->launch.last_split_chunks;
    if (bytes) *bytes = p->launch.last_split_bytes;
    return MCI_OK;
}

int mci_debug_vegas_cursor(const mci_problem *p, int32_t *used, uint64_t *base) {
    if (!p) return fail(MCI_ERR_INVALID, "NULL argument");
    if (used) *used = p->launch.last_cursor ? 1 : 0;
    if (base) *base = p->cursor_base;
    return MCI_OK;
}

int mci_debug_compiler_id(const char *set, char *out, int32_t n) {
    if (set) mcijit::compiler_id_override() = set;
    if (out && n > 0) snprintf(out, (size_t)n, "%s", mcijit::compiler_id().c_str());
    return MCI_OK;
}

int mci_debug_mcmc_policy(int64_t pilot_steps, int64_t grow, int64_t carry_holds, int64_t carry_half_floors) {
    if (pilot_steps > 0) mci_problem::kMcmcPilotSteps = pilot_steps;
    if (grow > 0) mci_problem::kMcmcGrow = grow;
    if (carry_holds > 0) mci_problem::kMcmcCarryHolds = carry_holds;
    if (carry_half_floors > 0) mci_problem::kMcmcCarryHalfFloors = carry_half_floors;
    return MCI_OK;
}

int mci_debug_persist_spin_ticks(mci_problem *p, unsigned long long ticks) {
    if (!p || ticks == 0) return fail(MCI_ERR_INVALID, "bad argument");
    p->persist_spin_ticks = ticks;
    return MCI_OK;
}

int mci_set_deterministic(mci_problem *p, int32_t on) {
    if (!p) return fail(MCI_ERR_INVALID, "NULL argument");
    const bool want = on != 0;
    if (want != p->deterministic) {
        p->deterministic = want;
        p->shape.det = want ? 1 : 0;
        drop_modules(p);
    }
    return MCI_OK;
}

int mci_set_chain_carry(mci_problem *p, int32_t mode) {
    if (!p) return fail(MCI_ERR_INVALID, "NULL argument");
    if (mode < -1 || mode > 1) return fail(MCI_ERR_INVALID, "chain carry mode must be -1 (automatic) or 1 (many-chain launches of :vegasmc and :mcmc continue the chains of the iteration before) or 0 (every launch starts its chains afresh)");
    p->chain_carry = mode;
    if (mode == 0) p->launch.chain_valid = false;
    return MCI_OK;
}

int mci_set_iteration_counted(mci_problem *p, int32_t counted) {
    if (!p) return fail(MCI_ERR_INVALID, "NULL argument");
    p->launch_counted = counted != 0;
    return MCI_OK;
}

int mci_set_persistent(mci_problem *p, int32_t mode) {
    if (!p) return fail(MCI_ERR_INVALID, "NULL argument");
    if (mode < -1 || mode > 1) return fail(MCI_ERR_INVALID, "persistent mode must be -1 (automatic: launch-bound :vegas calls), 0 (one launch chain per iteration) or 1 (whenever the layout allows)");
    p->persistent = mode;
    return MCI_OK;
}

int mci_debug_persist_words(mci_problem *p, unsigned long long *out, int32_t n) {
    if (!p || !out || !p->d_persist) return fail(MCI_ERR_INVALID, "no persistent launch yet");
    HIPCHK(hipStreamSynchronize(p->ctx->stream));
    HIPCHK(hipMemcpy(out, p->d_persist, (size_t)(n < (int)kPersistWords ? n : (int)kPersistWords) * sizeof(unsigned long long), hipMemcpyDeviceToHost));
    return MCI_OK;
}

int mci_debug_walk_counts(mci_problem *p, int64_t *out) {
    if (!p || !out || !p->d_status) return fail(MCI_ERR_INVALID, "NULL argument");
    int h[2] = {0, 0};
    HIPCHK(hipStreamSynchronize(p->ctx->stream));
    HIPCHK(hipMemcpy(h, p->d_status + 1, sizeof(h), hipMemcpyDeviceToHost));
    out[0] = h[0];
    out[1] = h[1];
    return MCI_OK;
}

int mci_last_integrate_persistent(const mci_problem *p, int32_t *persistent) {
    if (!p || !persistent) return fail(MCI_ERR_INVALID, "NULL argument");
    *persistent = p->last_persistent ? 1 : 0;
    return MCI_OK;
}

int mci_last_chain_launch(const mci_problem *p, int64_t *nchain, int32_t *carried) {
    if (!p) return fail(MCI_ERR_INVALID, "NULL argument");
    if (nchain) *nchain = p->launch.last_nchain;
    if (carried) *carried = p->launch.last_carried ? 1 : 0;
    return MCI_OK;
}

int mci_check_status(mci_problem *p) {
    if (!p) return fail(MCI_ERR_INVALID, "NULL argument");
    if (p->ctx->offline) return fail(MCI_ERR_NO_DEVICE, "offline context");
    return check_status(p);
}
static int compile_persist(mci_problem *p, bool background);
static bool persist_layout_ok(const mci_problem *p);
static int compile_strat(mci_problem *p);
static int compile_sweep_unit(mci_problem *p, int which);
static bool sweep_leaves_unit(const mci_problem *p);
int mci_compile_solver(mci_problem *p, int32_t solver) {
    if (solver == MCI_VEGAS_PERSISTENT) {
        if (!persist_layout_ok(p)) return fail(MCI_ERR_INVALID, "this layout has no persistent :vegas kernel (mci_set_persistent)");
        return compile_persist(p, false);
    }
    if (solver == MCI_VEGASMC_LANES || solver == MCI_MCMC_LANES) return mci_compile_chain_speculation(p, solver == MCI_VEGASMC_LANES ? MCI_VEGASMC : MCI_MCMC);
    if (solver == MCI_VEGAS_STRAT) {
        if (!p->strat.on) return fail(MCI_ERR_INVALID, "the problem is not stratified (mci_set_stratification)");
        return compile_strat(p);
    }
    if (const int w = sweep_unit_of(solver); w >= 0) {
        mci_integrate_args a{};
        a.solver = MCI_VEGAS;
        a.measurefreq = 1;
        a.niter = 1;
        if (w == mci_problem::Sweep::kChains || w == mci_problem::Sweep::kChainsCarry) {
            a.solver = MCI_VEGASMC;
            a.nchain = 1;
            a.neval = (int64_t)1 << 40;
            a.block = 1;
            if (int rc = mci_sweep_chains_supported(p, &a, nullptr, 0)) return rc;
        } else if (w == mci_problem::Sweep::kMcmc || w == mci_problem::Sweep::kMcmcCarry) {
            a.solver = MCI_MCMC;
            a.nchain = 1;
            a.neval = (int64_t)1 << 30;
            a.block = 1;
            a.thermal_ratio = 0.1;
            if (int rc = mci_sweep_mcmc_supported(p, &a, nullptr, 0)) return rc;
        } else if (w == mci_problem::Sweep::kStrat) {
            a.neval = (int64_t)1 << 40;
            a.block = 1;
            if (int rc = mci_sweep_strat_supported(p, &a, nullptr, 0)) return rc;
        } else {
            if (int rc = mci_sweep_supported(p, &a, nullptr, 0)) return rc;
            if (w == mci_problem::Sweep::kOne && sweep_leaves_unit(p))
                return fail(MCI_ERR_INVALID, "a sweep of this problem runs the sweep kernel for several leaves (MCI_VEGAS_SWEEP_LEAVES; mci_set_sweep_leaves)");
            if (w == mci_problem::Sweep::kLeaves && !sweep_leaves_unit(p))
                return fail(MCI_ERR_INVALID, "a sweep of this problem runs the one-grid sweep kernel (MCI_VEGAS_SWEEP; mci_set_sweep_leaves)");
        }
        return compile_sweep_unit(p, w);
    }
    if (solver < 0 || solver > 2) return fail(MCI_ERR_INVALID, "Solver %d is not supported!", solver);
    return compile_solver(p, solver);
}

int mci_get_histogram_copies(const mci_problem *p, int32_t *copies) {
    if (!p || !copies) return fail(MCI_ERR_INVALID, "NULL argument");
    *copies = (p->kernel[MCI_VEGAS].compiled || p->kernel[kSlotVegasAny].compiled) ? p->shape.hcopy : planned_hcopy(p, nullptr);
    return MCI_OK;
}

int mci_problem_info(const mci_problem *p, int32_t *ndraw, int32_t *nobs, int64_t *packed_size, int32_t *table_mode, int64_t *lds_bytes) {
    if (ndraw) *ndraw = p->shape.ndraw;
    if (nobs) *nobs = p->shape.nobs;
    if (packed_size) *packed_size = p->packed_n;
    if (table_mode) *table_mode = p->shape.table_mode;
    if (lds_bytes) *lds_bytes = p->lds_bytes;
    return MCI_OK;
}
```

### mcintegration.jl_amd/csrc/mci_host_plan.h

```cpp
namespace {

struct LaunchRequest {
    int32_t solver;
    int64_t nevalperblock, block_lo, block_hi, nblocks;
    int32_t iteration;
    uint64_t seed;
    int64_t measurefreq;
    double thermal_ratio;
    bool auto_chains;
    int kern;
};

struct LaunchPlan {
    int T = 0;
    bool may_carry = false;
    int64_t nchain = 1;
    double burnin = 0.0;
    int64_t nburn = 0;
    int64_t units = 0;
    int G = 1, spec_maxacc = 0;
    int T_launch = 0;
    int wpb = 0;
    bool cursor = false;
    bool hist_lds = false, split = false, atomic_flush = false;
    int ghist_buffers = 0;
    int64_t nrows = 0, nwg = 0;
    int64_t chunk_len = 0, nchunks = 1;
    int64_t hist_rows = 0;
    int tiles_wpb = 0;
    int64_t hm_n = 0, hm_first = 0, hm_count = 0;
    int hm_rows = 0;
    bool time_this_launch = false;
    bool carried() const { return may_carry && nchain > 1; }
};

void plan_threads(const mci_problem *p, const LaunchRequest &rq, LaunchPlan &pl) {
    pl.T = solver_threads(p, rq.solver);
    if (rq.solver == MCI_VEGAS && p->vegas.wide && !p->vegas.threads_vegas && p->wg_per_block <= 0 && rq.nblocks * rq.nevalperblock < ((int64_t)1 << 22) &&
        rq.nblocks * rq.nevalperblock * p->shape.ndraw >= ((int64_t)1 << 19))
        pl.T = 512;
}

bool plan_may_carry(const mci_problem *p, const LaunchRequest &rq) {
    return rq.solver != MCI_VEGAS && p->chain_carry != 0 && p->launch.chain_valid && p->launch.chain_solver == rq.solver &&
           p->launch.chain_lo == rq.block_lo && p->launch.chain_hi == rq.block_hi && p->launch.chain_nchain > 1 &&
           (rq.solver != MCI_VEGASMC || p->launch.chain_ntrain >= 1 || p->launch.chain_ntrain == p->ntrain) &&
           ((p->launch.chain_iteration & (kRepeatStride - 1)) + 1 == (rq.iteration & (kRepeatStride - 1)) ||
            ((p->launch.chain_iteration & (kRepeatStride - 1)) == (rq.iteration & (kRepeatStride - 1)) && rq.iteration > p->launch.chain_iteration));
}

int plan_vegasmc_chains(const mci_problem *p, const LaunchRequest &rq, const Overrides &ov, LaunchPlan &pl) {
    int nslots = 0;
    for (int v = 0; v < p->npool; ++v) nslots += p->maxdof[v];
    if (pl.nchain <= 0) {
        const int64_t fl = 64 * (int64_t)nslots > 128 ? 64 * (int64_t)nslots : 128;
        const int64_t fresh = ov.fresh_floors.on ? ov.fresh_floors.v : (p->launch_counted && p->ntrain == 0) ? 64 : 8;
        pl.nchain = rq.nevalperblock / ((pl.may_carry ? 2 : fresh) * fl);
        const int64_t cap = mci_problem::kChainFill / rq.nblocks > 64 ? mci_problem::kChainFill / rq.nblocks : 64;
        if (pl.nchain > cap) pl.nchain = cap;
        if (pl.nchain < 1) pl.nchain = 1;
    }
    if (pl.nchain > rq.nevalperblock) return fail(MCI_ERR_INVALID, "nchain=%lld exceeds the %lld steps of a block", (long long)pl.nchain, (long long)rq.nevalperblock);
    pl.burnin = mci_chain_burnin(rq.nevalperblock / pl.nchain, (pl.may_carry && pl.nchain > 1) ? 1 : pl.nchain, nslots);
    if (ov.fresh_burnin_pct.on && !pl.may_carry && pl.nchain > 1 && rq.auto_chains) {
        const double b = (double)(rq.nevalperblock / pl.nchain) * (double)ov.fresh_burnin_pct.v / 100.0;
        if (b > pl.burnin) pl.burnin = b;
    }
    pl.units = pl.nchain;
    return MCI_OK;
}

int plan_mcmc_chains(const mci_problem *p, const LaunchRequest &rq, LaunchPlan &pl) {
    int nslots = 0;
    for (int v = 0; v < p->npool; ++v) nslots += p->maxdof[v];
    if (pl.nchain <= 0) {
        const int64_t hold_eff = p->launch.mcmc_warm && p->launch.hold_prev > p->launch.hold_max ? p->launch.hold_prev : p->launch.hold_max;
        pl.nchain = mci_mcmc_auto_chains(rq.nevalperblock, rq.nblocks, nslots, p->ni + 1, p->npool, hold_eff, p->launch.mcmc_warm && p->launch.hold_valid ? 0 : p->launch.hold_len,
                                      pl.may_carry ? 1 : 0);
    }
    if (pl.nchain > rq.nevalperblock) return fail(MCI_ERR_INVALID, "nchain=%lld exceeds the %lld steps of a block", (long long)pl.nchain, (long long)rq.nevalperblock);
    pl.nburn = (pl.may_carry && pl.nchain > 1) ? 0 : mci_mcmc_burnin(rq.nevalperblock / pl.nchain, pl.nchain, nslots, p->ni + 1, p->npool, rq.thermal_ratio);
    pl.units = pl.nchain;
    return MCI_OK;
}

void plan_spec_lanes(const mci_problem *p, const LaunchRequest &rq, LaunchPlan &pl) {
    const auto &s = p->shape;
    if (rq.solver != MCI_VEGAS && !s.host_integrand && !p->deterministic && p->spec_lanes != 1) {
        if (p->spec_lanes > 1) pl.G = p->spec_lanes;
        else {
            pl.G = 64;
            while (pl.G > 1 && rq.nblocks * pl.nchain * pl.G > mci_problem::kSpecFill) pl.G >>= 1;
            if (pl.G < 8) pl.G = 1;
        }
    }
}

void plan_grid(const mci_problem *p, const LaunchRequest &rq, LaunchPlan &pl) {
    const auto &s = p->shape;
    pl.wpb = p->wg_per_block;
    if (pl.G > 1) {
        if (pl.wpb <= 0) pl.wpb = (int)((2048 + rq.nblocks - 1) / rq.nblocks);
        const int64_t maxw = (pl.units + pl.T_launch - 1) / pl.T_launch;
        if (pl.wpb > maxw) pl.wpb = (int)maxw;
        if (pl.wpb < 1) pl.wpb = 1;
    } else
    if (pl.wpb <= 0) {
        const int64_t big = pl.T >= 1024 ? 1024 : pl.T >= 512 ? 2048 : 4096;
        int64_t target = (pl.units * rq.nblocks >= (int64_t)1 << 25 && p->lds_bytes <= 32 * 1024) ? big : 2048;
        if (rq.solver == MCI_VEGAS && pl.units * rq.nblocks < ((int64_t)1 << 22) && target > 256) target = 256;
        if (rq.solver == MCI_VEGAS && pl.units * rq.nblocks * s.ndraw < ((int64_t)1 << 19) && target > 64) target = 64;
        pl.wpb = (int)((target + rq.nblocks - 1) / rq.nblocks);
        const int64_t maxw = (pl.units + pl.T - 1) / pl.T;
        if (pl.wpb > maxw) pl.wpb = (int)maxw;
        if (pl.wpb < 1) pl.wpb = 1;
    }
}

int plan_cursor_candidate(const mci_problem *p, const LaunchRequest &rq, const Overrides &ov, const LaunchPlan &pl) {
    if (!(rq.solver == MCI_VEGAS && pl.G == 1 && !p->in_self_check && vegas_pipe_unit(p) && !(ov.vegas_cursor.on && ov.vegas_cursor.v == 0))) return 0;
    if (ov.vegas_cursor.on && ov.vegas_cursor.v == 1) return 1;
    return p->wg_per_block <= 0 && pl.units * rq.nblocks >= ((int64_t)1 << 25) ? 2 : 0;
}
void plan_cursor_grid(const LaunchRequest &rq, int resident, LaunchPlan &pl) {
    if (resident >= rq.nblocks && (resident / rq.nblocks) * rq.nblocks > kAtomicRows) {
        pl.cursor = true;
        pl.wpb = (int)(resident / rq.nblocks);
        const int64_t maxw = (pl.units + pl.T - 1) / pl.T;
        if (pl.wpb > maxw) pl.wpb = (int)maxw;
    }
}

int64_t parked_bytes_per_sample(const mci_problem *p) { return (int64_t)p->shape.ni * 8 + (int64_t)(p->tdraw_words > 0 ? p->tdraw_words : 1) * 4; }

void plan_tiles(const mci_problem *p, const LaunchRequest &rq, const Overrides &ov, LaunchPlan &pl) {
    const auto &s = p->shape;
    pl.hist_lds = (s.table_mode == 0 || s.table_mode == 3);
    pl.split = rq.solver == MCI_VEGAS && s.ntile > 1;
    if (!pl.split && pl.wpb * s.ntile > 4096 / rq.nblocks && s.ntile > 1) pl.wpb = (int)(4096 / rq.nblocks / s.ntile) > 0 ? (int)(4096 / rq.nblocks / s.ntile) : 1;
    pl.nrows = rq.nblocks * pl.wpb;
    pl.atomic_flush = rq.solver == MCI_VEGAS && pl.hist_lds && s.ntile == 1 && atomic_rows_ok(p) && pl.nrows <= kAtomicRows && !s.host_integrand;
    pl.nwg = pl.split ? pl.nrows : pl.nrows * s.ntile;
    pl.ghist_buffers = pl.atomic_flush ? (pl.nrows > 64 ? 3 : 1) : 0;
    pl.chunk_len = rq.nevalperblock;
    pl.nchunks = 1;
    if (pl.split && !s.host_integrand && !s.host_measure) {
        const int64_t bytes = parked_bytes_per_sample(p);
        int64_t cap = (int64_t)1 << 27;
        if (cap * bytes > (int64_t)7500000000) cap = (int64_t)7500000000 / bytes;
        if (ov.split_chunk.on && ov.split_chunk.v > 0) cap = ov.split_chunk.v;
        int64_t per = (cap / rq.nblocks) & ~(int64_t)3;
        if (per < 4) per = 4;
        if (per < pl.chunk_len) {
            pl.chunk_len = per;
            pl.nchunks = (rq.nevalperblock + pl.chunk_len - 1) / pl.chunk_len;
        }
    }
}

void plan_replay(const mci_problem *p, const LaunchRequest &rq, LaunchPlan &pl) {
    const auto &s = p->shape;
    pl.hist_rows = pl.nrows;
    if (pl.split && s.split_all) {
        int64_t rwpb = 512 / (rq.nblocks * s.ntile);
        if (rwpb > pl.wpb) rwpb = pl.wpb;
        if (rwpb < 1) rwpb = 1;
        pl.tiles_wpb = (int)rwpb;
        pl.hist_rows = rq.nblocks * rwpb;
    }
}

void plan_host_measure(const mci_problem *p, const LaunchRequest &rq, LaunchPlan &pl) {
    const auto &s = p->shape;
    if (!s.host_measure) return;
    const int nw = s.ni * s.ncomp;
    if (rq.solver == MCI_VEGAS) {
        pl.hm_n = rq.nevalperblock;
        pl.hm_rows = nw;
    } else {
        const int64_t mfq = rq.measurefreq > 0 ? rq.measurefreq : 1;
        const int64_t last = rq.solver == MCI_VEGASMC ? rq.nevalperblock / pl.nchain : rq.nevalperblock / pl.nchain + pl.nburn;
        pl.hm_first = 1;
        if (rq.solver == MCI_VEGASMC) {
            pl.hm_first = (int64_t)(pl.burnin / (double)mfq);
            if (pl.hm_first < 1) pl.hm_first = 1;
            while (pl.hm_first > 1 && (double)((pl.hm_first - 1) * mfq) >= pl.burnin) --pl.hm_first;
            while ((double)(pl.hm_first * mfq) < pl.burnin) ++pl.hm_first;
        } else if (pl.nburn > 0) {
            pl.hm_first = (pl.nburn + mfq - 1) / mfq;
            if (pl.hm_first < 1) pl.hm_first = 1;
        }
        pl.hm_count = last / mfq - pl.hm_first + 1;
        if (pl.hm_count < 0) pl.hm_count = 0;
        pl.hm_n = pl.nchain * pl.hm_count;
        pl.hm_rows = rq.solver == MCI_MCMC ? s.ncomp : nw;
    }
}

void plan_timing(const mci_problem *p, const LaunchRequest &rq, LaunchPlan &pl) {
    pl.time_this_launch = p->kernel_timing > 0 || (p->kernel_timing < 0 && rq.nblocks * rq.nevalperblock >= ((int64_t)1 << 20));
}

}
```

### mcintegration.jl_amd/csrc/mci_host_problem.h

```cpp
int mci_problem_create(mci_ctx *ctx, const mci_problem_desc *d, mci_problem **out) {
    if (!ctx || !d || !out) return fail(MCI_ERR_INVALID, "NULL argument");
    if (d->nleaf < 1 || d->npool < 1 || d->nintegrand < 1) return fail(MCI_ERR_INVALID, "At least one integrand is required.");
    if (d->nintegrand > 31) return fail(MCI_ERR_INVALID, "at most 31 integrands are supported");
    mci_problem *p = new mci_problem();
    p->ctx = ctx;
    p->npool = d->npool;
    p->ni = d->nintegrand;
    const int Nd = p->ni + 1;
    p->dof.assign((size_t)Nd * p->npool, 0);
    for (int i = 0; i < p->ni * p->npool; ++i) {
        if (d->dof[i] < 0) { delete p; return fail(MCI_ERR_INVALID, "dof must be non-negative"); }
        p->dof[i] = d->dof[i];
    }
    p->maxdof.assign(p->npool, 0);
    mci_maxdof(p->dof.data(), Nd, p->npool, p->maxdof.data());
    p->pool_leaf0.assign(p->npool, -1);
    p->pool_nleaf.assign(p->npool, 0);
    auto &s = p->shape;
    int eoff = 0, aoff = 0, doff = 0, boff = 0;
    for (int l = 0; l < d->nleaf; ++l) {
        const mci_leaf_desc &ld = d->leaves[l];
        if (ld.pool < 0 || ld.pool >= p->npool) { delete p; return fail(MCI_ERR_INVALID, "leaf %d: pool out of range", l); }
        if (p->pool_leaf0[ld.pool] < 0) p->pool_leaf0[ld.pool] = l;
        else if (p->pool_leaf0[ld.pool] + p->pool_nleaf[ld.pool] != l) { delete p; return fail(MCI_ERR_INVALID, "leaves of pool %d are not contiguous", ld.pool); }
// ... 289 lines not shown
    p->h_reweight.assign(Nd, 1.0 / Nd);
    s.body = "w[0] = 1.0;";
    if (!ctx->offline) {
        HIPCHK(hipSetDevice(ctx->device));
        int rc = upload(p);
        if (!rc) rc = p->d_packed.reserve(p->packed_n + 64);
        if (!rc) rc = p->d_ghist.reserve(3 * (int64_t)(s.nbin ? s.nbin : 1));
        if (!rc) rc = p->d_stage1.reserve((int64_t)mci_problem::kGroups * (s.nbin ? s.nbin : 1));
        if (!rc) rc = p->d_status.reserve(4);
        std::vector<mci::LeafDev> ld;
        for (auto &L : p->leaves) ld.push_back({L.kind, L.nbin, L.eoff, L.doff, L.boff, L.adapt, L.alpha});
        if (!rc) rc = p->d_leaves.reserve((int64_t)ld.size());
        if (rc) { delete p; return rc; }
        HIPCHK(hipMemset(p->d_packed, 0, (size_t)(p->packed_n + 64) * sizeof(double)));
        HIPCHK(hipMemset(p->d_ghist, 0, 3 * (size_t)(s.nbin ? s.nbin : 1) * sizeof(double)));
        HIPCHK(hipMemset(p->d_status, 0, 4 * sizeof(int)));
        HIPCHK(hipMemcpy(p->d_leaves, ld.data(), ld.size() * sizeof(mci::LeafDev), hipMemcpyHostToDevice));
        p->evs.resize(2 * mci_problem::kEvRing);
        for (auto &e : p->evs) HIPCHK(hipEventCreate(&e));
    }
    *out = p;
    return MCI_OK;
}

int mci_problem_destroy(mci_problem *p) {
    if (!p) return MCI_OK;
    if (!p->ctx->offline) {
        (void)hipStreamSynchronize(p->ctx->stream);
        for (KernelUnit &u : p->kernel) u.drop();
    }
    persist_job_drop(p);
    if (!p->ctx->offline) {
        if (p->hold_ev) (void)hipEventDestroy(p->hold_ev);
        for (auto &e : p->cevs) (void)hipEventDestroy(e);
        tile_release(p);
        for (auto &e : p->evs) (void)hipEventDestroy(e);
    }
    delete p;
    return MCI_OK;
}

int mci_set_integrand_source(mci_problem *p, const char *body, const double *ud, int32_t nud) {
    if (!p || !body) return fail(MCI_ERR_INVALID, "NULL argument");
    p->shape.body = body;
    p->shape.host_integrand = 0;
    p->host_fn = nullptr;
    p->h_ud.assign(ud, ud + (nud > 0 ? nud : 0));
    drop_modules(p);
    if (!p->ctx->offline) {
        p->d_ud.reset();
        if (int rc = p->d_ud.reserve(p->h_ud.size() ? p->h_ud.size() : 1)) return rc;
        if (p->h_ud.size()) HIPCHK(hipMemcpy(p->d_ud, p->h_ud.data(), p->h_ud.size() * sizeof(double), hipMemcpyHostToDevice));
    }
    return MCI_OK;
}

int mci_set_integrand_host(mci_problem *p, mci_host_integrand_fn fn, void *user) {
    if (!p || !fn) return fail(MCI_ERR_INVALID, "NULL argument");
    p->host_fn = fn;
    p->host_user = user;
    p->host_idx_fn = nullptr;
    p->shape.host_integrand = 1;
    p->shape.body = "";
    p->h_ud.clear();
    drop_modules(p);
    return p->ctx->offline ? MCI_OK : p->d_ud.reserve(1);
}

int mci_set_integrand_host_indexed(mci_problem *p, mci_host_integrand_idx_fn fn, void *user) {
    if (!p || !fn) return fail(MCI_ERR_INVALID, "NULL argument");
    p->host_idx_fn = fn;
    p->host_fn = nullptr;
    p->host_user = user;
    p->shape.host_integrand = 1;
    p->shape.body = "";
    p->h_ud.clear();
    drop_modules(p);
    return p->ctx->offline ? MCI_OK : p->d_ud.reserve(1);
}

static int eval_host_integrand(mci_problem *p, const int32_t *idx, const double *x, double *w, int64_t n) {
    const auto &s = p->shape;
    const int nw = s.ni * s.ncomp, nc = s.ncomp;
    int hrc = 0;
    if (!idx) {
        memset(w, 0, (size_t)n * nw * sizeof(double));
        if (p->host_fn) hrc = p->host_fn(x, w, n, s.ndraw, nw, p->host_user);
        else {
            std::vector<int32_t> which((size_t)n);
            for (int j = 0; j < s.ni && !hrc; ++j) {
                std::fill(which.begin(), which.end(), j);
                hrc = p->host_idx_fn(which.data(), x, w + (size_t)j * nc * n, n, s.ndraw, nc, p->host_user);
            }
        }
    } else if (p->host_idx_fn) {
        memset(w, 0, (size_t)n * nc * sizeof(double));
        hrc = p->host_idx_fn(idx, x, w, n, s.ndraw, nc, p->host_user);
    } else {
        p->h_tmp.assign((size_t)n * nw, 0.0);
        hrc = p->host_fn(x, p->h_tmp.data(), n, s.ndraw, nw, p->host_user);
        for (int q = 0; q < nc; ++q)
            for (int64_t i = 0; i < n; ++i) w[(size_t)q * n + i] = idx[i] >= 0 ? p->h_tmp[((size_t)idx[i] * nc + q) * n + i] : 0.0;
    }
    if (hrc) return fail(MCI_ERR_INVALID, "the host integrand failed (%d)", hrc);
    return MCI_OK;
}

int mci_set_measure_source(mci_problem *p, const char *body) {
    if (!p) return fail(MCI_ERR_INVALID, "NULL argument");
    p->shape.measure_body = body ? body : "";
    p->shape.host_measure = 0;
    p->hmeas_fn = nullptr;
    p->hmeas_idx_fn = nullptr;
    drop_modules(p);
    return MCI_OK;
}

int mci_set_measure_host(mci_problem *p, mci_host_measure_fn fn, void *user) {
    if (!p) return fail(MCI_ERR_INVALID, "NULL argument");
    p->hmeas_fn = fn;
    p->hmeas_idx_fn = nullptr;
    p->hmeas_user = user;
    p->shape.host_measure = fn ? 1 : 0;
    if (fn) p->shape.measure_body = "";
    drop_modules(p);
    return MCI_OK;
}

int mci_set_measure_host_indexed(mci_problem *p, mci_host_measure_idx_fn fn, void *user) {
    if (!p) return fail(MCI_ERR_INVALID, "NULL argument");
    p->hmeas_idx_fn = fn;
    p->hmeas_fn = nullptr;
    p->hmeas_user = user;
    p->shape.host_measure = fn ? 1 : 0;
    if (fn) p->shape.measure_body = "";
    drop_modules(p);
    return MCI_OK;
}

int mci_set_launch(mci_problem *p, int32_t threads, int32_t wg_per_block) {
    if (threads > 0) {
        if (threads % 64 || threads > 1024) return fail(MCI_ERR_INVALID, "threads per workgroup must be a multiple of 64, <= 1024");
        p->threads_explicit = true;
        if (threads != p->threads || p->vegas.threads_vegas) {
            p->threads = threads;
            p->vegas.explicit_threads(threads, g_over.hist_copies.on);
            drop_modules(p);
        }
    }
    if (wg_per_block >= 0) p->wg_per_block = wg_per_block;
    return MCI_OK;
}

static bool sixteen_copies_fit(const mci_problem *p) {
    const auto &s = p->shape;
    return s.rng_bits == 32 && s.rng_rounds == 7 && p->lds_bytes + (int64_t)s.htile * 8 * 15 <= 159 * 1024;
}
static int planned_hcopy(const mci_problem *p, int *threads) { return p->vegas.planned_copies(sixteen_copies_fit(p), threads); }

static int64_t vegas_lds(const mci_problem *p) {
    const auto &s = p->shape;
    return (s.ec_doubles > 0 ? p->lds_bytes_k1 : p->lds_bytes) + (int64_t)s.htile * 8 * (s.hcopy - 1);
}

static const int64_t kAtomicRows = 256;
static bool atomic_rows_ok(const mci_problem *p) { return !p->deterministic && kAtomicRows > 0; }

static int solver_threads(const mci_problem *p, int solver) {
    if (p->deterministic && p->threads_det[solver]) return p->threads_det[solver];
    return solver == MCI_VEGAS ? p->vegas.threads(p->threads) : p->threads;
}
static int64_t det_lds(const mci_problem *p, int threads) {
    const auto &s = p->shape;
    return p->lds_bytes + ((int64_t)s.htile + s.nobs) * 8 * (threads / 64 - 1);
}
static int64_t solver_lds(const mci_problem *p, int solver) {
    if (p->deterministic) return det_lds(p, solver_threads(p, solver));
    return solver == MCI_VEGAS ? vegas_lds(p) : p->lds_bytes;
}

static bool vegas_pipe_unit(const mci_problem *p) {
    const auto &s = p->shape;
    if (p->vegas.conservative || p->deterministic || s.det) return false;
    if (s.ndraw < 8 || s.ndraw > 16 || !s.pair_table || s.table_mode != 0 || s.ntile != 1) return false;
    if (s.host_integrand || s.host_measure || s.ec_doubles > 0) return false;
    for (const auto &l : p->leaves)
        if (l.kind != 0) return false;
    return true;
}
static int cursor_resident(mci_problem *p, int kern, int threads, int *out) {
    hipFunction_t f = p->kernel[kern].f;
    const int64_t lds = solver_lds(p, MCI_VEGAS);
    if (f != p->cursor_occ_f || threads != p->cursor_occ_threads || lds != p->cursor_occ_lds) {
        int per_cu = 0, cus = 0;
        HIPCHK(hipModuleOccupancyMaxActiveBlocksPerMultiprocessor(&per_cu, f, threads, (size_t)lds));
        HIPCHK(hipDeviceGetAttribute(&cus, hipDeviceAttributeMultiprocessorCount, p->ctx->device));
        p->cursor_occ_f = f;
        p->cursor_occ_threads = threads;
        p->cursor_occ_lds = lds;
        p->cursor_occ_resident = per_cu * cus;
    }
    *out = p->cursor_occ_resident;
    return MCI_OK;
}
```

### mcintegration.jl_amd/csrc/mci_host_types.h

```cpp
namespace {

struct Id128 { char b[128]; };
struct Rccl {
    void *h = nullptr;
    int (*GetUniqueId)(void *) = nullptr;
    int (*CommInitRank)(void **, int, Id128 , int) = nullptr;
    int (*AllReduce)(const void *, void *, size_t, int, int, void *, hipStream_t) = nullptr;
    int (*CommDestroy)(void *) = nullptr;
    const char *(*GetErrorString)(int) = nullptr;
};
Rccl g_rccl;
const int kNcclFloat64 = 8, kNcclSum = 0;

int find_loaded_rccl(struct dl_phdr_info *info, size_t, void *out) {
    const char *n = info->dlpi_name;
    if (n && strstr(n, "librccl.so")) {
        *(std::string *)out = n;
        return 1;
    }
    return 0;
}

int rccl_load() {
    if (g_rccl.h) return MCI_OK;
    void *h = nullptr;
    std::string loaded;
    dl_iterate_phdr(find_loaded_rccl, &loaded);
    if (!loaded.empty()) h = dlopen(loaded.c_str(), RTLD_NOW | RTLD_GLOBAL);
    if (!h) h = dlopen("librccl.so", RTLD_NOW | RTLD_GLOBAL);
    if (!h) h = dlopen("librccl.so.1", RTLD_NOW | RTLD_GLOBAL);
    if (!h) return fail(MCI_ERR_COMM, "cannot load librccl.so: %s", dlerror());
    g_rccl.GetUniqueId = (int (*)(void *))dlsym(h, "ncclGetUniqueId");
    g_rccl.CommInitRank = (int (*)(void **, int, Id128, int))dlsym(h, "ncclCommInitRank");
    g_rccl.AllReduce = (int (*)(const void *, void *, size_t, int, int, void *, hipStream_t))dlsym(h, "ncclAllReduce");
    g_rccl.CommDestroy = (int (*)(void *))dlsym(h, "ncclCommDestroy");
    g_rccl.GetErrorString = (const char *(*)(int))dlsym(h, "ncclGetErrorString");
    if (!g_rccl.GetUniqueId || !g_rccl.CommInitRank || !g_rccl.AllReduce || !g_rccl.CommDestroy)
        return fail(MCI_ERR_COMM, "librccl.so lacks the nccl* entry points");
    g_rccl.h = h;
    return MCI_OK;
}

}

struct mci_ctx {
    int device = -1;
    bool offline = false;
    hipStream_t stream = nullptr;
    void *comm = nullptr;
    int rank = 0, nranks = 1;
    long long collectives = 0, last_count = 0;
    std::mutex spare_mu;
    void *spare = nullptr;
    size_t spare_bytes = 0;
};

namespace {
const int64_t kTrainLdsMax = 160 * 1024 - 4096;
const int kMaxLeafBins = 4400;
struct Leaf {
    int kind, pool, npts, nbin, adapt, eoff, doff, boff;
    double lower, upper, alpha;
    int width = 1;
};

template <class T, bool kPinned> struct Buf {
    Buf() = default;
    Buf(const Buf &) = delete;
    Buf &operator=(const Buf &) = delete;
    ~Buf() { reset(); }
    T *get() const { return ptr; }
    operator T *() const { return ptr; }
    int64_t capacity() const { return cap; }
    void reset() { adopt(nullptr, 0); }
    void adopt(T *q, int64_t n) {
        if (ptr) (void)(kPinned ? hipHostFree(ptr) : hipFree(ptr));
        ptr = q;
        cap = n;
    }
    int reserve(int64_t n) {
        if (n <= cap) return MCI_OK;
        reset();
        void *q = nullptr;
        HIPCHK(kPinned ? hipHostMalloc(&q, (size_t)n * sizeof(T), hipHostMallocDefault) : hipMalloc(&q, (size_t)n * sizeof(T)));
        ptr = (T *)q;
        cap = n;
        return MCI_OK;
    }

  private:
    T *ptr = nullptr;
    int64_t cap = 0;
};
template <class T> using DevBuf = Buf<T, false>;
template <class T> using PinBuf = Buf<T, true>;

struct Candidate;
struct KernelUnit {
    hipModule_t module = nullptr;
    hipFunction_t f = nullptr;
    bool compiled = false;
    std::string code_object;
    int threads = 0;
    enum Stale { kRecompileOnce, kUnlinkAndFail, kFail };
    struct Rules {
        Stale stale;
        bool no_scratch;
        std::string refusal;
        std::string what;
    };
    int load(const mci_ctx *ctx, Candidate &c, const char *kernel, int64_t lds, const Rules &rules);
    int entry(hipFunction_t *out, const char *name, int64_t lds) const {
        HIPCHK(hipModuleGetFunction(out, module, name));
        if (lds > 64 * 1024) HIPCHK(hipFuncSetAttribute((const void *)*out, hipFuncAttributeMaxDynamicSharedMemorySize, (int)lds));
        return MCI_OK;
    }
    void drop() {
        compiled = false;
        f = nullptr;
        if (module) (void)hipModuleUnload(module);
        module = nullptr;
    }
};
}

struct mci_problem {
    mci_ctx *ctx = nullptr;
    std::vector<Leaf> leaves;
    int npool = 0, ni = 0;
    std::vector<int> dof, maxdof, pool_leaf0, pool_nleaf;
    mcijit::ProblemShape shape;
    int nstat = 0;
    int64_t packed_n = 0;
    int64_t lds_bytes = 0;
    int64_t lds_bytes_k1 = 0;
    std::vector<double> h_edges, h_dacc, h_ddist, h_reweight, h_ud;
    DevBuf<double> d_edges, d_dacc, d_ddist, d_reweight, d_ud;
    DevBuf<double> d_part_cols, d_part_hist, d_ghist, d_stage1, d_packed;
    DevBuf<double> d_scratch, d_iterlog, d_dump;
    DevBuf<int> d_status;
    DevBuf<mci::LeafDev> d_leaves;
    enum { kSlots = 7, kPersist = kSlots, kStrat, kSweep, kKernels = kSweep + 7 };
    KernelUnit kernel[kKernels];
    VegasKernelPlan vegas;
    int spec_lanes = -1, spec_maxacc = -1;
    double spec_accept = 0.0;
    DevBuf<mci::SpecNode> d_spec_tab;
    int spec_tab_lanes = 0, spec_tab_limit = -2, spec_tab_maxacc = 0;
    int spec_ntree = 0, spec_first = 0;
    float spec_accepts[8] = {};
    double spec_tab_accept = -1.0;
    int spec_state[2] = {0, 0};
    bool spec_need_check[2] = {false, false};
    bool in_self_check = false;
    int vegas_check_state[2] = {0, 0};
    bool vegas_check_done[2] = {false, false};
    int vegas_check_flags = 0;
    int check_slot = -1;
    int64_t check_launches = 0;
    int64_t last_discarded_neval = 0;
    int32_t last_discarded_launches = 0;
    static const int64_t kSpecFill = 65536;
    std::vector<double> h_goal;
    DevBuf<double> d_goal;
    int npa = 0;
    DevBuf<double> d_part_pa;
    DevBuf<unsigned long long> d_hold;
    double *d_tile_w = nullptr;
    uint32_t *d_tile_bins = nullptr;
    size_t tile_bytes = 0;
    int64_t cap_tile = 0;
    int ntdraw = 0;
    int tdraw_words = 0;
    hipFunction_t f_tiles[2] = {nullptr, nullptr};
    mci::MergeArgs merge{};
    bool merge_pending = false;
    bool has_fermik = false;
    mci_host_integrand_fn host_fn = nullptr;
    mci_host_integrand_idx_fn host_idx_fn = nullptr;
    PinBuf<int32_t> h_hidx;
    std::vector<double> h_tmp;
    void *host_user = nullptr;
    DevBuf<double> d_hx, d_hw;
    PinBuf<double> h_hx, h_hw;
    DevBuf<char> d_hstep;
    mci_host_measure_fn hmeas_fn = nullptr;
    mci_host_measure_idx_fn hmeas_idx_fn = nullptr;
    void *hmeas_user = nullptr;
    DevBuf<double> d_mx, d_mrelw, d_mobs;
    PinBuf<double> h_mx, h_mrelw;
    DevBuf<int32_t> d_midx;
    PinBuf<int32_t> h_midx;
    std::vector<double> h_mtmp;
    std::vector<int32_t> h_mitmp;
    int threads = 256, wg_per_block = 0;
    bool threads_explicit = false;
    int kernel_timing = -1;
    bool deterministic = false;
    int threads_det[3] = {0, 0, 0};
    int train_serial = -1;
    bool debug_wrong_decision = false;
    static const int64_t kSerialWalkSamples = (int64_t)1 << 26;
    bool train_lds_raised = false;
    std::vector<hipEvent_t> cevs;
    bool cev_valid[64] = {};
    int64_t reduces = 0;
    static const int kCevRing = 64;
    PinBuf<unsigned long long> h_hold;
    PinBuf<double> h_hold_d;
    hipEvent_t hold_ev = nullptr;
    DevBuf<double> d_blocklog;
    DevBuf<double> d_chain_x[2];
    DevBuf<double> d_chain_P[2];
    DevBuf<double> d_carry_w;
    hipFunction_t f_carryw[2] = {nullptr, nullptr};
    DevBuf<int> d_chain_curr[2];
    int64_t chain_stride(int b) const { return d_chain_curr[b].capacity(); }
    int chain_carry = -1;
    int64_t ntrain = 0;
    bool launch_counted = false;
    DevBuf<double> d_reweight_used, d_carry_W;
    DevBuf<int> d_carry_src;
    DevBuf<unsigned long long> d_clocks;
    std::vector<hipEvent_t> evs;
    static const int kEvRing = 512;
    int log_row = 0;
    PinBuf<double> h_log;
    bool persist_failed = false;
    struct PersistJob;
    PersistJob *persist_job = nullptr;
    DevBuf<unsigned long long> d_persist;
    DevBuf<double> d_edges_backup;
    unsigned long long persist_arrive = 0, persist_done = 0;
    unsigned long long persist_spin_ticks = 200000000ull;
    int persistent = -1;
    bool last_persistent = false;
    static const int kGroups = mci::kMergeGroups;
    static const int kCursorLog2Big = 4, kCursorOnes = 4;
    DevBuf<unsigned long long> d_cursor;
    int64_t cursor_nblocks = 0;
    unsigned long long cursor_base = 0;
    hipFunction_t cursor_occ_f = nullptr;
    int cursor_occ_threads = 0, cursor_occ_resident = 0;
    int64_t cursor_occ_lds = 0;
    static const int64_t kChainFill = 131072;
    static int64_t kMcmcPilotSteps, kMcmcGrow;
    static int64_t kMcmcCarryHolds, kMcmcCarryHalfFloors;
    struct LaunchState {
        int last_wg = 0, last_threads = 0, last_nblocks = 0;
        int64_t last_samples = 0;
        int64_t last_nchain = 0;
        int last_spec_lanes = 1, last_spec_maxacc = 0;
        bool last_carried = false;
        bool last_cursor = false;
        int64_t last_split_chunks = 0, last_split_bytes = 0;
        int64_t launches = 0;
        bool time_this_launch = true;
        bool ev_valid[kEvRing] = {};
        bool clock_valid[kEvRing] = {};
        int chain_cur = 0;
        bool chain_valid = false;
        int chain_solver = -1, chain_iteration = -1;
        int64_t chain_lo = 0, chain_hi = 0, chain_nchain = 0;
        int64_t chain_ntrain = 0;
        int64_t blk_rows = 0, blk_stride = 0, blk_lo = -1;
        int blk_carried = 0;
        int64_t hold_max = 0;
        int64_t hold_len = 0;
        int64_t hold_prev = 0;
        bool hold_valid = false;
        bool hold_measured = false;
        bool mcmc_warm = false;
        bool hold_inflight = false;
        bool hold_from_packed = false;
        bool hold_deferred = false;
        bool hold_ext_pending = false;
        int64_t hold_launches = 0;
        int64_t hold_len_inflight = 0;
        bool hold_carried_inflight = false;
    } launch;
    static_assert(std::is_trivially_copyable<LaunchState>::value, "the launch record holds values only");
    struct Strat {
        bool on = false;
        std::vector<int> want;
        double beta = 0.75;
        int64_t max_nhcube = (int64_t)1 << 24;
        std::vector<int> nstrat;
        int64_t ncube = 0, nsamp = 0;
        DevBuf<long long> d_off;
        bool ran = false;
        bool alloc_valid = false;
        bool alloc_pending = false;
        DevBuf<double> d_d;
        bool carry = false;
        bool c_valid = false;
        std::vector<int> c_nstrat;
        int64_t c_ncube = 0;
        double c_beta = 0.0;
        std::vector<double> c_host;
        int carry_how = 0;
        DevBuf<double> d_tsum;
        DevBuf<double> d_part, d_rec_s, d_stat;
        DevBuf<long long> d_rec_h;
        int64_t last_nchunk = 0;
        bool last_run = false;
        int compiled_det = -1;
        double *hx = nullptr, *hy = nullptr, *hjac = nullptr, *hw = nullptr;
        long long *hh = nullptr;
        int64_t hn = 0;
        double *hstart = nullptr;
        int64_t hstart_n = 0;
    } strat;
    struct Sweep {
        enum { kOne = 0, kLeaves = 1, kStrat = 2, kChains = 3, kMcmc = 4, kChainsCarry = 5, kMcmcCarry = 6, kUnits = 7 };
        int grid = 0;
        int want_threads = 0;
        int last_grid = 0, last_threads = 0;
        int leaves_mode = 0;
        int chain_carry = 0;
    } sweep;
    KernelUnit &sweep_unit(int which) { return kernel[kSweep + which]; }
    static_assert(kKernels == kSweep + Sweep::kUnits, "one handle per sweep unit");
};

struct SweepUnitDesc {
    int jit_unit;
    int32_t solver;
    int32_t runs;
    const char *tag;
    const char *for_what;
    bool alpha;
    bool want_threads;
};
static const SweepUnitDesc kSweepUnits[mci_problem::Sweep::kUnits] = {
    {mcijit::kUnitSweep, MCI_VEGAS_SWEEP, MCI_VEGAS, "", "", true, true},
    {mcijit::kUnitSweepLeaves, MCI_VEGAS_SWEEP_LEAVES, MCI_VEGAS, "several leaves", " for several leaves", false, false},
    {mcijit::kUnitSweepStrat, MCI_VEGAS_SWEEP_STRAT, MCI_VEGAS, "stratified points", " for stratified points", true, false},
    {mcijit::kUnitSweepChains, MCI_VEGASMC_SWEEP, MCI_VEGASMC, ":vegasmc points", " for :vegasmc points", false, false},
    {mcijit::kUnitSweepMcmc, MCI_MCMC_SWEEP, MCI_MCMC, ":mcmc points", " for :mcmc points", false, false},
    {mcijit::kUnitSweepChainsCarry, MCI_VEGASMC_SWEEP_CARRY, MCI_VEGASMC, ":vegasmc points, carried chains", " for :vegasmc points with carried chains", false, false},
    {mcijit::kUnitSweepMcmcCarry, MCI_MCMC_SWEEP_CARRY, MCI_MCMC, ":mcmc points, carried chains", " for :mcmc points with carried chains", false, false},
};
static int sweep_unit_of(int32_t solver) {
    for (int w = 0; w < mci_problem::Sweep::kUnits; ++w)
        if (kSweepUnits[w].solver == solver) return w;
    return -1;
}

static const int kRepeatStride = 16384, kMaxRepeats = 7;

int64_t mci_problem::kMcmcPilotSteps = 4096;
int64_t mci_problem::kMcmcGrow = 2;
int64_t mci_problem::kMcmcCarryHolds = 4;
int64_t mci_problem::kMcmcCarryHalfFloors = 2;

namespace {
struct Override { bool on = false; int64_t v = 0; };
struct Overrides { Override table_mode, hist_tile_bins, no_split_all, l1_phase, train_walk, hist_copies, fresh_floors, fresh_burnin_pct, spec_self_check, split_chunk, vegas_self_check, vegas_cursor, cursor_log2_big, cursor_ones; } g_over;
Override *override_slot(const char *key) {
    if (!key) return nullptr;
    if (!strcmp(key, "table_mode")) return &g_over.table_mode;
    if (!strcmp(key, "hist_tile_bins")) return &g_over.hist_tile_bins;
    if (!strcmp(key, "no_split_all")) return &g_over.no_split_all;
    if (!strcmp(key, "l1_phase")) return &g_over.l1_phase;
    if (!strcmp(key, "train_walk")) return &g_over.train_walk;
    if (!strcmp(key, "hist_copies")) return &g_over.hist_copies;
    if (!strcmp(key, "fresh_floors")) return &g_over.fresh_floors;
    if (!strcmp(key, "fresh_burnin_pct")) return &g_over.fresh_burnin_pct;
    if (!strcmp(key, "spec_self_check")) return &g_over.spec_self_check;
    if (!strcmp(key, "split_chunk")) return &g_over.split_chunk;
    if (!strcmp(key, "vegas_self_check")) return &g_over.vegas_self_check;
    if (!strcmp(key, "vegas_cursor")) return &g_over.vegas_cursor;
    if (!strcmp(key, "cursor_log2_big")) return &g_over.cursor_log2_big;
    if (!strcmp(key, "cursor_ones")) return &g_over.cursor_ones;
    return nullptr;
}
}

static void persist_job_drop(mci_problem *p);
namespace { void persist_orphans_join(); }
static const size_t kPersistWords = 8 + 3 * 8 * 8 + 16;

namespace {

int tile_alloc(mci_problem *p, size_t bytes) {
    mci_ctx *c = p->ctx;
    void *base = nullptr;
    {
        std::lock_guard<std::mutex> g(c->spare_mu);
        if (c->spare && c->spare_bytes >= bytes && c->spare_bytes <= 2 * bytes + ((size_t)64 << 20)) {
            base = c->spare;
            p->tile_bytes = c->spare_bytes;
            c->spare = nullptr;
            c->spare_bytes = 0;
        }
    }
    if (!base) {
        HIPCHK(hipMalloc(&base, bytes));
        p->tile_bytes = bytes;
    }
    p->d_tile_w = (double *)base;
    return MCI_OK;
}
void tile_release(mci_problem *p) {
    if (!p->d_tile_w) return;
    mci_ctx *c = p->ctx;
    void *drop = p->d_tile_w;
    {
        std::lock_guard<std::mutex> g(c->spare_mu);
        if (p->tile_bytes > c->spare_bytes) {
            drop = c->spare;
            c->spare = p->d_tile_w;
            c->spare_bytes = p->tile_bytes;
        }
    }
    if (drop) (void)hipFree(drop);
    p->d_tile_w = nullptr;
    p->d_tile_bins = nullptr;
    p->tile_bytes = 0;
    p->cap_tile = 0;
}

int upload(mci_problem *p) {
    if (p->ctx->offline) return MCI_OK;
    auto up = [&](DevBuf<double> &d, const std::vector<double> &h) -> int {
        if (!d)
            if (int rc = d.reserve(h.size() ? h.size() : 1)) return rc;
        if (h.size()) HIPCHK(hipMemcpyAsync(d, h.data(), h.size() * sizeof(double), hipMemcpyHostToDevice, p->ctx->stream));
        return MCI_OK;
    };
    int rc;
    if ((rc = up(p->d_edges, p->h_edges))) return rc;
    if ((rc = up(p->d_dacc, p->h_dacc))) return rc;
    if ((rc = up(p->d_ddist, p->h_ddist))) return rc;
    if ((rc = up(p->d_reweight, p->h_reweight))) return rc;
    HIPCHK(hipStreamSynchronize(p->ctx->stream));
    return MCI_OK;
}

int ensure_capacity(mci_problem *p, int64_t nwg, int64_t nblocks) {
    const auto &s = p->shape;
    int rc = p->d_part_cols.reserve(nwg * s.ncols);
    if (!rc && (s.table_mode == 0 || s.table_mode == 3)) rc = p->d_part_hist.reserve(nwg * (s.nbin ? s.nbin : 1));
    if (!rc) rc = p->d_scratch.reserve(nblocks * s.ncols);
    return rc;
}

template <class Args> void fill_tables(const mci_problem *p, Args &a) {
    a.edges = p->d_edges;
    a.dacc = p->d_dacc;
    a.ddist = p->d_ddist;
}
void fill_batch(const mci_problem *p, mci::BatchArgs &a) {
    fill_tables(p, a);
    a.reweight = p->d_reweight;
    a.ud = p->d_ud;
    a.part_cols = p->d_part_cols;
    a.part_hist = p->d_part_hist;
    a.ghist = p->d_ghist;
}
mci::MergeArgs merge_args(const mci_problem *p, int64_t nblocks, int wpb, int64_t nrows) {
    const auto &s = p->shape;
    mci::MergeArgs m{};
    m.part_cols = p->d_part_cols;
    m.ncols = s.ncols;
    m.nobs = s.nobs;
    m.ni = s.ni;
    m.nblocks = (int)nblocks;
    m.wg_per_block = wpb;
    m.stage1 = p->d_stage1;
    m.ngroup = (int)mci_problem::kGroups;
    m.ghist = p->d_ghist;
    m.nbin = s.nbin;
    m.packed = p->d_packed;
    m.status = p->d_status;
    m.scratch = p->d_scratch;
    m.npa = p->npa;
    m.nrows = (int)nrows;
    return m;
}
void fill_train(const mci_problem *p, mci::TrainArgs &t) {
    fill_tables(p, t);
    t.leaves = p->d_leaves;
    t.nleaf = p->shape.nleaf;
    t.packed = p->d_packed;
    t.nstat = p->nstat;
    t.reweight = p->d_reweight;
    t.nd = p->shape.ni + 1;
    t.status = p->d_status;
}
void record_launch(mci_problem *p, int64_t samples, int64_t nwg, int threads, int64_t nblocks) {
    p->launch.last_samples = samples;
    p->launch.last_wg = (int)nwg;
    p->launch.last_threads = threads;
    p->launch.last_nblocks = (int)nblocks;
}

int check_status(mci_problem *p) {
    int st = 0;
    HIPCHK(hipMemcpyAsync(&st, p->d_status, sizeof(int), hipMemcpyDeviceToHost, p->ctx->stream));
    HIPCHK(hipStreamSynchronize(p->ctx->stream));
    if (!st) return MCI_OK;
    HIPCHK(hipMemsetAsync(p->d_status, 0, sizeof(int), p->ctx->stream));
    if (st & mci::ST_PERSIST_STALL) {
        HIPCHK(hipMemsetAsync(p->d_persist, 0, 3 * sizeof(unsigned long long), p->ctx->stream));
        HIPCHK(hipMemsetAsync(p->d_ghist, 0, 3 * (size_t)(p->shape.nbin ? p->shape.nbin : 1) * sizeof(double), p->ctx->stream));
        p->persist_arrive = p->persist_done = 0;
        p->persist_failed = true;
        return fail(MCI_ERR_HIP, "the persistent :vegas launch stalled (is the device shared with other long-running kernels?); "
                                 "the iterations of this call are void -- later calls launch per iteration (mci_set_persistent(prob, 0))");
    }
    if (st & mci::ST_MCMC_INIT) return fail(MCI_ERR_INVALID, "Cannot find the variables that makes the integrand nonzero!");
    if (st & mci::ST_NORMALIZATION) return fail(MCI_ERR_NORMALIZATION, "Block normalization is not positively defined!");
    if (st & mci::ST_HIST_NONFINITE) return fail(MCI_ERR_HISTOGRAM, "histogram should be all finite");
    if (st & mci::ST_HIST_NONPOSITIVE) return fail(MCI_ERR_HISTOGRAM, "histogram should be all positive and non-zero");
    return fail(MCI_ERR_HISTOGRAM, "distribution is not all finite");
}

int persist_recover(mci_problem *p) {
    hipStream_t st = p->ctx->stream;
    HIPCHK(hipMemsetAsync(p->d_status, 0, sizeof(int), st));
    HIPCHK(hipMemsetAsync(p->d_persist, 0, 3 * sizeof(unsigned long long), st));
    HIPCHK(hipMemsetAsync(p->d_ghist, 0, 3 * (size_t)(p->shape.nbin ? p->shape.nbin : 1) * sizeof(double), st));
    p->persist_arrive = p->persist_done = 0;
    p->persist_failed = true;
    p->merge_pending = false;
    return MCI_OK;
}

int hold_publish(mci_problem *p, int64_t chain_len, bool carried) {
    hipStream_t st = p->ctx->stream;
    if (!p->h_hold) {
        int rc = p->h_hold.reserve(64);
        if (!rc) rc = p->h_hold_d.reserve(64);
        if (rc) return rc;
        HIPCHK(hipEventCreateWithFlags(&p->hold_ev, hipEventDisableTiming));
    }
    p->launch.hold_len_inflight = chain_len;
    p->launch.hold_carried_inflight = carried;
    p->launch.hold_launches += 1;
    if (p->ctx->comm) {
        p->launch.hold_deferred = true;
        return MCI_OK;
    }
    if (p->launch.hold_inflight) HIPCHK(hipEventSynchronize(p->hold_ev));
    HIPCHK(hipMemcpyAsync(p->h_hold, p->d_hold, 64 * sizeof(unsigned long long), hipMemcpyDeviceToHost, st));
    HIPCHK(hipEventRecord(p->hold_ev, st));
    p->launch.hold_inflight = true;
    p->launch.hold_from_packed = false;
    p->launch.hold_ext_pending = true;
    return MCI_OK;
}

int hold_publish_reduced(mci_problem *p) {
    hipStream_t st = p->ctx->stream;
    HIPCHK(hipMemcpyAsync(p->h_hold_d, p->d_packed + p->packed_n, 64 * sizeof(double), hipMemcpyDeviceToHost, st));
    HIPCHK(hipEventRecord(p->hold_ev, st));
    p->launch.hold_inflight = true;
    p->launch.hold_from_packed = true;
    p->launch.hold_deferred = false;
    return MCI_OK;
}

int hold_consume(mci_problem *p) {
    if (!p->launch.hold_inflight) return MCI_OK;
    HIPCHK(hipEventSynchronize(p->hold_ev));
    p->launch.hold_inflight = false;
    int top = -1;
    for (int b = 0; b < 64; ++b)
        if (p->launch.hold_from_packed ? p->h_hold_d[b] > 0.5 : p->h_hold[b] != 0ull) top = b;
    if (top >= 0) {
        p->launch.hold_prev = p->launch.mcmc_warm ? p->launch.hold_max : 0;
        p->launch.hold_max = (int64_t)1 << top;
        p->launch.hold_len = p->launch.hold_len_inflight;
        p->launch.hold_valid = p->launch.hold_len >= (p->launch.hold_carried_inflight ? mci_problem::kMcmcCarryHolds : 16) * p->launch.hold_max;
        if (p->launch.hold_valid) p->launch.mcmc_warm = true;
    }
    return MCI_OK;
}

void drop_modules(mci_problem *p) {
    p->vegas.modules_dropped();
    p->vegas_check_done[0] = p->vegas_check_done[1] = false;
    p->cursor_occ_f = nullptr;
    for (KernelUnit &u : p->kernel) u.drop();
    p->persist_failed = false;
    persist_job_drop(p);
}

}

static int flush_merge(mci_problem *p);
static int comm_sum_host(mci_problem *p, double *v, int n);

static int grow_keeping(mci_problem *p, DevBuf<double> &log, int64_t need, int64_t first, int64_t width) {
    const int64_t have = log.capacity() / width;
    if (need <= have) return MCI_OK;
    int64_t ncap = have ? have : first;
    while (ncap < need) ncap *= 2;
    double *n = nullptr;
    HIPCHK(hipMalloc((void **)&n, (size_t)ncap * width * sizeof(double)));
    if (log) {
        HIPCHK(hipMemcpyAsync(n, log, (size_t)have * width * sizeof(double), hipMemcpyDeviceToDevice, p->ctx->stream));
        HIPCHK(hipStreamSynchronize(p->ctx->stream));
    }
    log.adopt(n, ncap * width);
    return MCI_OK;
}

static int grow_block_log(mci_problem *p, int64_t rows) {
    const int64_t need = rows * p->launch.blk_stride;
    return grow_keeping(p, p->d_blocklog, need, 4096, 1);
}
```

### mcintegration.jl_amd/csrc/mci_host_vegas_plan.h

```cpp
namespace {

struct VegasKernelPlan {
    bool planned = false, keys = false;
    bool wide = false;
    int threads_vegas = 0;
    bool ladder = false;
    int hcopy_auto = 1, hcopy_rule = 1;
    bool hcopy_plan = false;
    bool conservative = false;

    void created(int copies, bool one_per_cu) {
        hcopy_auto = hcopy_rule = copies;
        ladder = one_per_cu;
        hcopy_plan = copies > 1 && !ladder;
        threads_vegas = ladder ? 1024 : hcopy_plan ? 512 : 0;
    }
    void modules_dropped() { planned = keys = wide = false; }
    void explicit_threads(int threads, bool override_on) {
        ladder = false;
        hcopy_plan = false;
        threads_vegas = 0;
        hcopy_auto = threads >= 512 || override_on ? hcopy_rule : 1;
    }
    void make_conservative(bool deterministic) {
        conservative = true;
        if (deterministic) return;
        hcopy_auto = 1;
        hcopy_plan = false;
        threads_vegas = 0;
        keys = wide = false;
    }
    int planned_copies(bool sixteen_fit, int *threads) const {
        const bool sixteen = hcopy_plan && hcopy_auto >= 8 && sixteen_fit;
        if (threads) *threads = sixteen ? 1024 : 512;
        return sixteen ? 16 : hcopy_auto;
    }
    int threads(int fallback) const { return threads_vegas ? threads_vegas : fallback; }
};

struct VegasVariant {
    int copies;
    bool keys;
    int threads;
};
struct VegasBuilt { long vgprs, scratch; bool ok; };
struct VegasRuleIn {
    int threads;
    bool threads_explicit;
    int ndraw;
    bool host_integrand, deterministic;
    bool copies_forced;
    bool sixteen_fit;
    int copies;
};
typedef std::function<void(const std::vector<VegasVariant> &, std::vector<VegasBuilt> &)> VegasBuild;

const long kVgprsTwoWide = 128, kVgprsSixWaves = 80;
const int kWideThreads = 512, kWideMaxDraws = 8;
const int kLadder[3] = {1024, 768, 512};
inline bool too_fat(const VegasBuilt &b) { return b.vgprs > kVgprsTwoWide || b.scratch != 0; }

inline int vegas_kernel_rule(VegasKernelPlan &pl, const VegasRuleIn &in, const VegasBuild &build_batch, VegasVariant *chosen) {
    std::vector<VegasBuilt> r;
    VegasVariant &v = *chosen;
    auto build = [&](const std::vector<VegasVariant> &vs) {
        build_batch(vs, r);
        int bad = 0;
        for (const VegasBuilt &b : r) bad |= !b.ok;
        return bad;
    };
    if (pl.planned) {
        v = {in.copies, pl.keys, pl.threads_vegas ? pl.threads_vegas : pl.wide ? kWideThreads : in.threads};
        if (build({v})) return 1;
        if (pl.keys && too_fat(r[0])) {
            v.keys = false;
            if (build({v})) return 1;
        }
        if (!pl.threads_vegas && pl.wide && too_fat(r[0])) {
            pl.wide = false;
            v.threads = in.threads;
            if (build({v})) return 1;
        }
        return 0;
    }
    const bool copy_plan = pl.hcopy_plan && !in.copies_forced && !pl.conservative;
    int tcopy = 512;
    const int copies = pl.planned_copies(in.sixteen_fit, &tcopy);
    if (pl.hcopy_plan) pl.threads_vegas = tcopy;
    const int T0 = pl.threads(in.threads);
    v = {copies, false, T0};
    const bool try_wide = !pl.conservative && in.threads == 256 && !in.threads_explicit && !in.deterministic && in.ndraw <= kWideMaxDraws && !in.host_integrand;
    auto plain_or_default = [&](VegasBuilt first, int fallback) {
        pl.wide = try_wide && first.scratch == 0 && first.vgprs <= kVgprsTwoWide;
        if (!try_wide || pl.wide) return 0;
        v.threads = fallback;
        return build({v});
    };
    if (copy_plan) {
        const VegasVariant plain = {1, false, try_wide ? kWideThreads : in.threads};
        v.keys = true;
        if (build({v, plain})) return 1;
        pl.keys = true;
        VegasBuilt copy = r[0], plain_built = r[1];
        if (too_fat(copy)) {
            v.keys = false;
            if (build({v})) return 1;
            pl.keys = false;
            copy = r[0];
        }
        if (copy.vgprs > kVgprsTwoWide || copy.vgprs <= kVgprsSixWaves) {
            pl.threads_vegas = 0;
            pl.keys = false;
            v = plain;
            if (plain_or_default(plain_built, in.threads)) return 1;
        }
    } else if (pl.ladder) {
        std::vector<VegasVariant> rungs;
        for (int t : kLadder)
            if (t <= T0) rungs.push_back({v.copies, false, t});
        build_batch(rungs, r);
        size_t pick = rungs.size() - 1;
        for (size_t i = 0; i < rungs.size(); ++i) {
            if (!r[i].ok) return 1;
            if (r[i].scratch == 0) { pick = i; break; }
        }
        v = rungs[pick];
        pl.threads_vegas = v.threads;
    } else {
        if (try_wide) v.threads = kWideThreads;
        if (build({v})) return 1;
        if (plain_or_default(r[0], T0)) return 1;
    }
    pl.planned = true;
    return 0;
}

}
```

### mcintegration.jl_amd/engine.py

```python
import atexit
import ctypes as C
import weakref

import numpy as np

from . import _lib
from ._lib import LeafDesc, ProblemDesc, c_double_p, c_int32_p, check, lib
from .integrand import HostIntegrand, HostMeasure, Integrand, Measure
from .variables import ContinuousVar, FermiK

_ctx_cache = {}


def _dp(a):
    return a.ctypes.data_as(c_double_p)


def context(device=0):
    if device not in _ctx_cache:
        p = C.c_void_p()
        check(lib().mci_ctx_create(device, C.byref(p)))
        _ctx_cache[device] = p
    return _ctx_cache[device]

# ... 225 lines not shown
        return cb

    def _make_host_indexed_callback(self, fn):
        config = self.config
        nc = config.ncomp
        state = {"per_sample": False}

        def cb(ip, xp, wp, n, ndraw, ncomp, user):
            try:
                idx = np.ctypeslib.as_array(ip, shape=(n,))
                X = np.ctypeslib.as_array(xp, shape=(ndraw, n))
                W = np.ctypeslib.as_array(wp, shape=(ncomp, n))
                for i in np.unique(idx[idx >= 0]):
                    sel = np.nonzero(idx == i)[0]
                    whole = len(sel) == n
                    Xs = X if whole else np.ascontiguousarray(X[:, sel])
                    o = None
                    if not state["per_sample"]:
                        try:
                            o = fn(int(i), self._pool_views(Xs, len(sel)), config)
                        except (ValueError, TypeError, IndexError) as e:
                            if len(sel) <= 1:
                                raise
                            _slow_path_warning("integrand", "sample", e)
                            state["per_sample"] = True
                    if o is None:
                        o = np.array([fn(int(i), self._pool_views(np.ascontiguousarray(Xs[:, j:j + 1]), 1, scalar=True), config) for j in range(len(sel))])
                    o = np.broadcast_to(np.asarray(o), (len(sel),))
                    if nc == 2:
                        W[0, sel], W[1, sel] = o.real, o.imag
                    else:
                        W[0, sel] = o
                return 0
            except Exception:
                import traceback
                traceback.print_exc()
                return 1
        return cb

    def _pool_views(self, X, n, scalar=False):
        layout = self.config.pool_layout()

        def typed(a, kind):
            return np.rint(a).astype(np.int64) if kind == "d" else a

        def pool(k0, md, nl, off, composite, kinds):
            a = X[k0:k0 + md * nl].reshape((md, n) if nl == 1 and not composite else (md, nl, n))
            if off:
                a = np.concatenate([np.zeros((off,) + a.shape[1:]), a])
            if composite:
                a = a.transpose(1, 0, 2)
                if len(set(kinds)) > 1:
                    return tuple(typed(a[l][..., 0] if scalar else a[l], kinds[l]) for l in range(nl))
            return typed(a[..., 0] if scalar else a, kinds[0])
        if len(layout) == 1 and layout[0][2:] == (1, 0, False, "c"):
            return X[:, 0] if scalar else X
        arg = tuple(pool(*p) for p in layout)
        return arg[0] if len(arg) == 1 else arg

    def _make_host_measure_callback(self, fn):
        config = self.config
        nc = config.ncomp
        dt = complex if nc == 2 else float
        state = {"per_record": False}

        def cb(xp, rp, n, stride, ndraw, nw, block, op, nobs, user):
            try:
                X = np.ctypeslib.as_array(xp, shape=(ndraw, stride))[:, :n]
                R = np.ctypeslib.as_array(rp, shape=(nw, stride))[:, :n]
                O = np.ctypeslib.as_array(op, shape=(nobs,))
                weights = [R[2 * i] + 1j * R[2 * i + 1] for i in range(config.N)] if nc == 2 else [R[i] for i in range(config.N)]
                obs = None
                if not state["per_record"]:
                    obs = [_HostObs(shape, dt) for shape in config.obs_shape]
                    try:
                        fn(self._pool_views(X, n), obs, weights, config)
                    except (ValueError, TypeError, IndexError) as e:
                        if n <= 1:
                            raise
                        _slow_path_warning("measure", "record", e)
                        state["per_record"], obs = True, None
                if obs is None:
                    obs = [np.zeros(shape, dtype=dt) for shape in config.obs_shape]
                    for j in range(n):
                        fn(self._pool_views(X[:, j:j + 1], 1, scalar=True), obs, [w[j] for w in weights], config)
                _store_obs(O, obs, config.obs_nbin, nc)
                return 0
            except Exception:
                import traceback
                traceback.print_exc()
                return 1
        return cb

    def _make_host_measure_indexed_callback(self, fn):
        config = self.config
        nc = config.ncomp
        dt = complex if nc == 2 else float
        state = {"per_record": False}

        def cb(ip, xp, rp, n, stride, ndraw, ncomp, block, op, nobs, user):
            try:
                idx = np.ctypeslib.as_array(ip, shape=(n,))
                X = np.ctypeslib.as_array(xp, shape=(ndraw, stride))[:, :n]
                R = np.ctypeslib.as_array(rp, shape=(ncomp, stride))[:, :n]
                O = np.ctypeslib.as_array(op, shape=(nobs,))
                obs, off = [], 0
                for shape, nb in zip(config.obs_shape, config.obs_nbin):
                    o = np.array(O[off:off + nb])
                    obs.append(((o[0::2] + 1j * o[1::2]) if nc == 2 else o.astype(dt)).reshape(shape).view(_HostObs))
                    off += nb
                w = (R[0] + 1j * R[1]) if nc == 2 else R[0]
                for i in np.unique(idx[idx >= 0]):
                    sel = np.nonzero(idx == i)[0]
                    whole = len(sel) == n
                    Xs = X if whole else np.ascontiguousarray(X[:, sel])
                    ws = w if whole else w[sel]
                    if not state["per_record"]:
                        before = [np.array(o) for o in obs]
                        try:
                            fn(int(i), self._pool_views(Xs, len(sel)), obs, ws, config)
                            continue
                        except (ValueError, TypeError, IndexError) as e:
                            if len(sel) <= 1:
                                raise
                            _slow_path_warning("measure", "record", e)
                            state["per_record"] = True
                            for o, q in zip(obs, before):
                                np.ndarray.__setitem__(o, slice(None), q)
                    plain = [o.view(np.ndarray) for o in obs]
                    for j in range(len(sel)):
                        fn(int(i), self._pool_views(np.ascontiguousarray(Xs[:, j:j + 1]), 1, scalar=True), plain, ws[j], config)
                _store_obs(O, obs, config.obs_nbin, nc)
                return 0
            except Exception:
                import traceback
                traceback.print_exc()
                return 1
        return cb

    def close(self):
        if getattr(self, "p", None):
            lib().mci_problem_destroy(self.p)
            self.p = None

    def __del__(self):
        try:
            self.close()
        except Exception:
            pass

    @staticmethod
    def _kernel_code(solver):
        return {"vegas_persistent": 3, "vegasmc_lanes": 5, "mcmc_lanes": 6, "vegas_strat": 7, "vegas_sweep": 8, "vegas_sweep_leaves": 9, "vegas_sweep_strat": 10,
                "vegasmc_sweep": 11, "mcmc_sweep": 12, "vegasmc_sweep_carry": 13, "mcmc_sweep_carry": 14}.get(solver) or _lib.SOLVERS[solver]

    def compile(self, solver="vegas"):
        check(lib().mci_compile_solver(self.p, self._kernel_code(solver)))

    def code_object(self, solver="vegas"):
        buf = C.create_string_buffer(4096)
        check(lib().mci_kernel_code_object(self.p, self._kernel_code(solver), buf, len(buf)))
        return buf.value.decode()

    def set_kernel_timing(self, mode=-1):
        check(lib().mci_set_kernel_timing(self.p, int(mode)))

    def histogram_copies(self):
        n = C.c_int32()
        check(lib().mci_get_histogram_copies(self.p, C.byref(n)))
        return n.value

    def check_status(self):
        check(lib().mci_check_status(self.p))

    def set_launch(self, threads=0, wg_per_block=-1):
        check(lib().mci_set_launch(self.p, threads, wg_per_block))

    def run(self, solver, nevalperblock, block_lo, block_hi, iteration, seed, measurefreq=1, nchain=0, thermal_ratio=0.1):
        check(lib().mci_iteration_run(self.p, _lib.SOLVERS[solver], int(nevalperblock), int(block_lo), int(block_hi),
                                      int(iteration), int(seed), int(measurefreq), int(nchain), float(thermal_ratio)))

    def reduce(self):
        check(lib().mci_iteration_reduce(self.p))

    def finish(self, solver, block_total, adapt=True, gamma=1.0, want_stats=True):
        if not want_stats:
            check(lib().mci_iteration_finish(self.p, _lib.SOLVERS[solver], int(block_total), 1 if adapt else 0, gamma, None, None))
            return None, None
        m, e = np.empty(self.nobs), np.empty(self.nobs)
        check(lib().mci_iteration_finish(self.p, _lib.SOLVERS[solver], int(block_total), 1 if adapt else 0, gamma, _dp(m), _dp(e)))
        return m, e

    def iteration(self, solver, nevalperblock, block_lo, block_hi, iteration, seed, measurefreq=1, nchain=0, thermal_ratio=0.1):
        self.run(solver, nevalperblock, block_lo, block_hi, iteration, seed, measurefreq, nchain, thermal_ratio)
        return self.get_packed()

    def iteration_log(self, nrows):
        nstat = 2 * self.nobs + 2 + self.config.N + 1
        out = np.empty((nrows, nstat))
        check(lib().mci_get_iteration_log(self.p, int(nrows), _dp(out)))
        return out

    def reserve_iterations(self, rows):
        check(lib().mci_reserve_iteration_log(self.p, int(rows)))

    def get_packed(self, reduce_size=False):
        out = np.empty(self.reduce_size if reduce_size else self.packed_size)
        check(lib().mci_get_packed(self.p, _dp(out), len(out)))
        return out

    @property
    def reduce_size(self):
        return self.packed_size + 64

    def external_reduce_done(self):
        check(lib().mci_external_reduce_done(self.p))

    def comm_collectives(self):
        n, c = C.c_int64(), C.c_int64()
        check(lib().mci_comm_collectives(context(self.device), C.byref(n), C.byref(c)))
        return int(n.value), int(c.value)

    def set_packed(self, a):
        a = np.ascontiguousarray(a, dtype=np.float64)
        check(lib().mci_set_packed(self.p, _dp(a), len(a)))

    def packed_device_ptr(self):
        return lib().mci_packed_device_ptr(self.p)

    def hold_histogram(self):
        out = (C.c_uint64 * 64)()
        check(lib().mci_get_hold_histogram(self.p, out))
        return np.array(list(out), dtype=np.uint64)

    def resample(self, curr_old, rw_now, rw_used, n_new, w_chain=None):
        co = np.ascontiguousarray(curr_old, dtype=np.int32)
        a, b = np.ascontiguousarray(rw_now, dtype=np.float64), np.ascontiguousarray(rw_used, dtype=np.float64)
        wc = None if w_chain is None else np.ascontiguousarray(w_chain, dtype=np.float64)
        if co.ndim != 2 or a.shape != b.shape or a.ndim != 1 or (wc is not None and wc.shape != co.shape):
            raise ValueError("curr_old [nblocks, n_old], rw_now and rw_used [nd], w_chain None or shaped like curr_old")
        nblocks, n_old = co.shape
        src = np.full((nblocks, max(int(n_new), 0)), -1, dtype=np.int32)
        W = np.full((nblocks, n_old), np.nan)
        check(lib().mci_debug_resample(self.p, nblocks, n_old, int(n_new), len(a), co.ctypes.data_as(c_int32_p), _dp(a), _dp(b),
                                       None if wc is None else _dp(wc), src.ctypes.data_as(c_int32_p), _dp(W)))
        return src, W

    def sweep_resample_lds(self):
        n = C.c_int64()
        check(lib().mci_debug_sweep_resample_lds(self.p, C.byref(n)))
        return int(n.value)

    def stream(self):
        return lib().mci_ctx_stream(context(self.device)) or 0

    def save_state(self, path):
        check(lib().mci_save_state(self.p, str(path).encode()))

    def load_state(self, path):
        check(lib().mci_load_state(self.p, str(path).encode()))

    def train(self):
        check(lib().mci_train(self.p))

    def set_rng_rounds(self, rounds):
        check(lib().mci_set_rng_rounds(self.p, int(rounds)))

    def set_rng_bits(self, bits):
        check(lib().mci_set_rng_bits(self.p, int(bits)))

    def set_deterministic(self, on=True):
        check(lib().mci_set_deterministic(self.p, 1 if on else 0))

    def set_chain_carry(self, mode):
        check(lib().mci_set_chain_carry(self.p, {"auto": -1, "off": 0, "on": 1, -1: -1, 0: 0, 1: 1}[mode]))

    def set_iteration_counted(self, counted):
        check(lib().mci_set_iteration_counted(self.p, 1 if counted else 0))

    def set_persistent(self, mode):
        check(lib().mci_set_persistent(self.p, {"auto": -1, "off": 0, "on": 1, -1: -1, 0: 0, 1: 1}[mode]))

    def last_integrate_persistent(self):
        v = C.c_int32()
        check(lib().mci_last_integrate_persistent(self.p, C.byref(v)))
        return bool(v.value)

    def last_chain_launch(self):
        n, c = C.c_int64(), C.c_int32()
        check(lib().mci_last_chain_launch(self.p, C.byref(n), C.byref(c)))
        return int(n.value), bool(c.value)

    def set_chain_speculation(self, lanes=-1, accept=0.0, max_accepts=-1):
        check(lib().mci_set_chain_speculation(self.p, int(lanes), float(accept), int(max_accepts)))

    def last_chain_speculation(self):
        g, m = C.c_int32(), C.c_int32()
        check(lib().mci_last_chain_speculation(self.p, C.byref(g), C.byref(m)))
        return int(g.value), int(m.value)

    def chain_speculation_status(self, solver):
        st = C.c_int32()
        check(lib().mci_chain_speculation_status(self.p, _lib.SOLVERS[solver], C.byref(st)))
        return int(st.value)

    def vegas_check_status(self):
        st, fl = C.c_int32(), C.c_int32()
# ... 462 lines not shown
```

### mcintegration.jl_amd/integrate.py

```python
import ctypes as C
import time

import numpy as np

from . import catalog
from ._lib import MCMC, SOLVERS, VEGAS, VEGASMC, lib
from .comm import LocalComm
from .configuration import Configuration
from .engine import Engine
from .integrand import HostIntegrand, HostMeasure, Integrand, Measure
from .statistics import Result, chain_estimator_bias, report
from .variables import Continuous, Discrete


class Stratify:

    def __init__(self, beta=0.75, nstrat=None, max_nhcube=2 ** 24, carry=False):
        if not isinstance(carry, (bool, np.bool_)):
            raise ValueError("Stratify: carry = %r, must be True or False" % (carry,))
        self.beta, self.max_nhcube, self.carry = float(beta), int(max_nhcube), bool(carry)
        self.nstrat = None if nstrat is None else [int(v) for v in nstrat]

    def __repr__(self):
        return "Stratify(beta=%r, nstrat=%r, max_nhcube=%r, carry=%r)" % (self.beta, self.nstrat, self.max_nhcube, self.carry)
# ... 438 lines not shown
        except tr.TraceError as e:
            why = "the closure was not traced (%s): a host integrand" % e
        bound_measure = measure
        if why is None and trace is not False and callable(measure) and not isinstance(measure, (Measure, HostMeasure)) and not hasattr(measure, "pool"):
            bound_measure = _trace_sweep_measure(measure, traced_on, params, solver) or measure
    else:
        if isinstance(integrand, str):
            integrand = Integrand(integrand, None)
        if isinstance(integrand, HostIntegrand):
            why = "a host integrand (device source or a traced closure only)"
        else:
            rows = np.asarray(params, dtype=np.float64)
            if rows.ndim != 2 or (len(integrand.userdata) and rows.shape[1] != len(integrand.userdata)):
                raise ValueError("integrate_sweep: params must be userdata rows [points][%d] for this integrand, got shape %s"
                                 % (len(integrand.userdata), rows.shape))
            bound = Integrand(integrand.body, rows[0], integrand.name)
    if device is None:
        device = 0
    nevalperblock, block = standardize_block(int(neval), block, 1)
    eng = None
    if why is None:
        eng = _bind(config, bound, bound_measure if closure else measure, solver, trace=trace, print=print, device=device)
        if hasattr(eng, "set_sweep_leaves"):
            eng.set_sweep_leaves(leaves)
        if strat is not None:
            if not hasattr(eng, "integrate_sweep_strat"):
                why = "this engine has no stratified sweep"
            else:
                eng.set_stratification(strat.nstrat, strat.beta, strat.max_nhcube)
                why = eng.sweep_strat_supported(solver, nevalperblock * block, niter, block, measurefreq)
        elif chains is not None:
            why = (eng.sweep_chains_supported(solver, nevalperblock * block, niter, block, measurefreq, nchain=chains,
                                              first_iteration=config.iterations_done)
                   if hasattr(eng, "sweep_chains_supported") else "this engine has no chain sweep")
        elif mcmc_chains is not None:
            why = (eng.sweep_mcmc_supported(solver, nevalperblock * block, niter, block, measurefreq, nchain=mcmc_chains,
                                            first_iteration=config.iterations_done, thermal_ratio=thermal_ratio)
                   if hasattr(eng, "sweep_mcmc_supported") else "this engine has no :mcmc sweep")
        else:
            why = eng.sweep_supported(solver, nevalperblock * block, niter, block, measurefreq) if hasattr(eng, "sweep_supported") else "this engine has no sweep"
    if why is None and strat is not None:
        plan = eng.sweep_strat_plan(nevalperblock * block, block)
        d_rows = _sweep_alloc_rows(alloc, P, plan) if alloc is not None else None
        rs = eng.integrate_sweep_strat(solver, userdata=rows, neval=nevalperblock * block, niter=niter, block=block, ignore=ignore, adapt=adapt,
                                       gamma=gamma, measurefreq=measurefreq, seed=config.seed, seeds=seeds, maps=maps,
                                       first_iteration=config.iterations_done, d=d_rows)
        out = []
        for p, r in zip(params, rs):
            c = copy.copy(config)
            c.userdata = p if closure else None
            c.visited = r["visited"]
            res = Result(r["iter_mean"], r["iter_std"], c, ignore, neval=r["neval"], seconds=r["seconds"], block=block)
            res.sweep_batched, res.map, res.status = True, r["maps"], r["status"]
            res.maps_by_leaf = r.get("maps_by_leaf")
            res.stratification = dict(nstrat=list(plan["nstrat"]), ncube=plan["ncube"], beta=plan["beta"], carry=False,
                                      carried="same plan" if alloc is not None else "uniform")
            res.strat_d, res.strat_counts = StratD(r["strat_d"], plan["nstrat"], plan["beta"]), r["strat_counts"]
            res.vegas_check, res.warmup, res.neval_discarded = None, 0, 0
            if print >= 0:
                report(res)
            out.append(res)
        return out
    if why is None and (chains is not None or mcmc_chains is not None):
        kw = dict(userdata=rows, neval=nevalperblock * block, niter=niter, block=block, ignore=ignore, adapt=adapt, gamma=gamma,
                  measurefreq=measurefreq, seed=config.seed, seeds=seeds, maps=maps, first_iteration=config.iterations_done, reweight=reweight)
        rs = (eng.integrate_sweep_chains(solver, nchain=chains, carry=carry, **kw) if chains is not None
              else eng.integrate_sweep_mcmc(solver, nchain=mcmc_chains, thermal_ratio=thermal_ratio, carry=carry, **kw))
        out = []
        for p, r in zip(params, rs):
            c = copy.copy(config)
            c.userdata = p if closure else None
            c.visited = r["visited"]
            c._sweep_tables = (r["propose"], r["accept"])
            res = Result(r["iter_mean"], r["iter_std"], c, ignore, neval=r["neval"], seconds=r["seconds"], block=block, correlated=r["correlated"])
            if r["correlated"]:
                res._flat_std = np.asarray(r["stdev"], dtype=np.float64)
                res.stdev = res._shape(res._flat_std)
            res.sweep_batched, res.map, res.status, res.reweight = True, r["maps"], r["status"], r["reweight"]
            res.maps_by_leaf = r.get("maps_by_leaf")
            res.stratification, res.vegas_check, res.warmup, res.neval_discarded, res.chain_bias = None, None, 0, 0, None
            if mcmc_chains is not None:
                res.holds, res.hold_max, res.chain_steps = r["holds"], r["hold_max"], nevalperblock // mcmc_chains
                res.chains_carried = bool(r.get("carried"))
            if print >= 0:
                report(res)
            out.append(res)
        return out
    if why is None:
        rs = eng.integrate_sweep(solver, userdata=rows, neval=nevalperblock * block, niter=niter, block=block, ignore=ignore, adapt=adapt,
                                 gamma=gamma, measurefreq=measurefreq, seed=config.seed, seeds=seeds, maps=maps,
                                 first_iteration=config.iterations_done)
        out = []
        for p, r in zip(params, rs):
            c = copy.copy(config)
            c.userdata = p if closure else None
            c.visited = r["visited"]
            res = Result(r["iter_mean"], r["iter_std"], c, ignore, neval=r["neval"], seconds=r["seconds"], block=block)
            res.sweep_batched, res.map, res.status = True, r["maps"], r["status"]
            res.maps_by_leaf = r.get("maps_by_leaf")
            res.stratification, res.vegas_check, res.warmup, res.neval_discarded = None, None, 0, 0
            if print >= 0:
                report(res)
            out.append(res)
        return out
    if not fresh:
        raise ValueError("integrate_sweep: this problem does not run as a sweep (%s), and the looped form builds one Configuration per "
                         "point from keywords (var=..., dof=...), not from config=" % why)
    if maps is not None:
        raise ValueError("integrate_sweep: this problem does not run as a sweep (%s), and maps= needs the batched form" % why)
    if alloc is not None:
        raise ValueError("integrate_sweep: this problem does not run as a sweep (%s), and alloc= needs the batched form" % why)
    if reweight is not None:
        raise ValueError("integrate_sweep: this problem does not run as a sweep (%s), and reweight= needs the batched form" % why)
    warnings.warn("integrate_sweep: this problem does not run as a sweep (%s): %d ordinary integrate() calls, one after another" % (why, P),
                  RuntimeWarning, stacklevel=2)
    if eng is not None and hasattr(eng, "close"):
        eng.close()
    out = []
    for k, p in enumerate(params):
        kw = copy.deepcopy(pristine)
        if closure:
            kw["userdata"], f = p, integrand
        else:
            f = integrand if isinstance(integrand, HostIntegrand) else Integrand(integrand.body, rows[k], integrand.name)
        c = Configuration(**kw)
        if seeds is not None:
            c.seed = int(seeds[k])
        res = integrate(f, solver=solver, config=c, neval=neval, niter=niter, block=block, gamma=gamma, adapt=adapt, ignore=ignore, measure=measure,
                        measurefreq=measurefreq, device=device, trace=trace, print=print, **({"stratify": strat} if strat is not None else {}), **({"nchain": chains} if chains is not None else {}),
                        **({"nchain": mcmc_chains, "thermal_ratio": thermal_ratio} if mcmc_chains is not None else {}))
        res.sweep_batched, res.map, res.maps_by_leaf, res.status = False, None, None, 0
        out.append(res)
    return out


def prefill_kernel_cache():
    import math
    L = math.sqrt(50.0)
    jobs = [
        (Configuration(var=Continuous(0.0, 1.0), dof=[[1]]), catalog.log_over_sqrt(), None),
        (Configuration(var=Continuous(-L, L), dof=[[16]]), catalog.gaussian(16), None),
        (Configuration(var=Continuous([(-L, L)] * 16), dof=[[1]]), catalog.gaussian(16), None),
        (Configuration(var=Continuous([(0.0, 1.0)] * 32), dof=[[1]]), catalog.genz_product_peak(32), None),
    ]
    p = catalog.bubble_parameters()
    from .integrand import bin_by
    var = (Continuous(0.0, 1.0, alpha=3.0), Continuous(0.0, math.pi, alpha=3.0), Continuous(0.0, 2 * math.pi, alpha=3.0),
           Continuous(0.0, p["beta"], alpha=3.0), Discrete(1, 4, adapt=False))
    jobs.append((Configuration(var=var, dof=[[1, 1, 1, 1, 1]], obs=[np.zeros(4)]), catalog.bubble(), bin_by(4)))
    n = 0
    for cfg, f, meas in jobs:
        eng = Engine(cfg, f, measure=meas, device=-1)
        eng.compile("vegas")
        if meas is not None:
            eng.compile("vegasmc")
            eng.compile("vegasmc_lanes")
            eng.set_sweep_leaves("all")
            eng.compile("vegas_sweep_leaves")
            eng.compile("vegasmc_sweep")
            eng.compile("mcmc_sweep")
        eng.close()
        n += 1
    eng = Engine(Configuration(var=Continuous(0.0, 1.0), dof=[[3], [6], [9], [12]]), catalog.nested_gauss(), device=-1)
    eng.compile("mcmc")
    eng.compile("mcmc_lanes")
    eng.close()
    return n + 1
```

Baseline: 76990.

## Add big :vegas unit with 1024 threads and sixteen histogram copies for large launches

Adds a second JIT-compiled :vegas kernel variant that runs 1024 threads per workgroup with sixteen LDS histogram copies. Large launches (at least 2^26 samples, with enough adaptive adds per sample, and with every block resident) switch to it, using the cursor grid and no atomic flush. The aim is to cut histogram contention and raise occupancy and throughput on large adaptive runs. It adds a compile step, VGPR-budget gating, a self-check path, and a fallback to the standing unit; the kernel cache is prefilled for the 16-D Gaussian case.

New measurement: 78510 (median of 6 runs). 2.0% higher.

```diff
diff --git a/include/mci.h b/include/mci.h
--- a/include/mci.h
+++ b/include/mci.h
@@ -27,6 +27,7 @@
 enum { MCI_VEGASMC_SWEEP = 11 };
 enum { MCI_MCMC_SWEEP = 12 };
 enum { MCI_VEGASMC_SWEEP_CARRY = 13, MCI_MCMC_SWEEP_CARRY = 14 };
+enum { MCI_VEGAS_BIG = 15 };
 enum { MCI_SWEEP_ONE_GRID = 0, MCI_SWEEP_ALL_LEAVES = 1 };
 
 typedef struct mci_ctx mci_ctx;
diff --git a/mcintegration.jl_amd/csrc/mci_host_check.h b/mcintegration.jl_amd/csrc/mci_host_check.h
--- a/mcintegration.jl_amd/csrc/mci_host_check.h
+++ b/mcintegration.jl_amd/csrc/mci_host_check.h
@@ -168,6 +168,7 @@
 
 static int vegas_self_check(mci_problem *p, int slot, int64_t nevalperblock, int64_t block_lo, int64_t block_hi, int32_t iteration, uint64_t seed,
                             int64_t measurefreq) {
+    const bool big = slot == mci_problem::kVegasBig;
     const int u = slot == kSlotVegasAny ? 1 : 0;
     const int64_t nb = block_hi - block_lo < 2 ? block_hi - block_lo : 2, npb = nevalperblock < 512 ? nevalperblock : 512;
     const int64_t mf = measurefreq * 4 <= npb ? measurefreq : 1;
@@ -203,6 +204,16 @@
             mcijit::write_file_atomic(object + ".ok", id.data(), id.size());
             break;
         }
+        if (big) {
+            fprintf(stderr, "mci: the big :vegas unit of this problem (%s) does not reproduce the library's static :vegas kernel on a %lld-block, "
+                            "%lld-sample check: %ld of %lld packed entries differ (first at %ld; statistics %ld, histogram %ld), draws of %lld samples and "
+                            "Jacobians of %lld differ.  A miscompiled code object -- big launches of this problem keep the standing :vegas unit; "
+                            "mci_vegas_check_status sets flag bit 3.\n",
+                    object.c_str(), (long long)nb, (long long)npb, df.bad, (long long)p->packed_n, df.first_bad, df.bad_sec[0], df.bad_sec[1], (long long)bad[0],
+                    (long long)bad[1]);
+            state = -1;
+            break;
+        }
         fprintf(stderr, "mci: the :vegas sample kernel of this problem (%s%s) does not reproduce the library's static :vegas kernel on a %lld-block, "
                         "%lld-sample check: %ld of %lld packed entries differ (first at %ld; statistics %ld, histogram %ld), draws of %lld samples and "
                         "Jacobians of %lld differ.  A miscompiled code object -- %s; mci_vegas_check_status reports %d.\n",
@@ -220,6 +231,19 @@
     p->kernel_timing = kernel_timing;
     if (p->d_status) (void)hipMemcpy(p->d_status, h_status, sizeof(h_status), hipMemcpyHostToDevice);
     p->merge.hist_no_offset = 0;
+    if (big) {
+        p->vegas_big.check_done = true;
+        if (state < 0) {
+            p->vegas_big.state = VegasBigUnit::kFailedCheck;
+            p->vegas_check_flags |= 8;
+        }
+        if (rc) {
+            fprintf(stderr, "mci: the self-check of this problem's big :vegas unit (%s) could not run: %s -- nothing was verified\n",
+                    p->kernel[slot].code_object.c_str(), mci_last_error());
+            p->merge_pending = false;
+        }
+        return MCI_OK;
+    }
     p->vegas_check_done[u] = true;
     if (rc) {
         fprintf(stderr, "mci: the self-check of this problem's :vegas code object (%s) could not run: %s -- nothing was verified "
@@ -235,18 +259,21 @@
 static int vegas_check_gate(mci_problem *p, int slot, int64_t nevalperblock, int64_t block_lo, int64_t block_hi, int32_t iteration, uint64_t seed,
                             int64_t measurefreq) {
     const int u = slot == kSlotVegasAny ? 1 : 0;
+    const bool big = slot == mci_problem::kVegasBig;
+    bool &done = big ? p->vegas_big.check_done : p->vegas_check_done[u];
     const bool force = g_over.vegas_self_check.on && g_over.vegas_self_check.v == 1;
     if (g_over.vegas_self_check.on && g_over.vegas_self_check.v == 0) return MCI_OK;
     if (!vegas_check_covers(p) || p->ctx->offline) {
-        p->vegas_check_done[u] = true;
+        done = true;
         return MCI_OK;
     }
     if (!force && access((p->kernel[slot].code_object + ".ok").c_str(), F_OK) == 0) {
+        done = true;
+        if (big) return MCI_OK;
         if (p->vegas_check_state[u] == 0) {
             p->vegas_check_state[u] = 1;
             p->vegas_check_flags |= 2;
         }
-        p->vegas_check_done[u] = true;
         return MCI_OK;
     }
     return vegas_self_check(p, slot, nevalperblock, block_lo, block_hi, iteration, seed, measurefreq);
diff --git a/mcintegration.jl_amd/csrc/mci_host_iteration.h b/mcintegration.jl_amd/csrc/mci_host_iteration.h
--- a/mcintegration.jl_amd/csrc/mci_host_iteration.h
+++ b/mcintegration.jl_amd/csrc/mci_host_iteration.h
@@ -361,7 +361,7 @@
             a.chunk_hi = a.chunk_lo + pl.chunk_len < rq.nevalperblock ? a.chunk_lo + pl.chunk_len : rq.nevalperblock;
             a.accum = c > 0 ? 1 : 0;
         }
-        HIPCHK(hipModuleLaunchKernel(f, (unsigned)pl.nwg, 1, 1, (unsigned)pl.T_launch, 1, 1, (unsigned)solver_lds(p, rq.solver), st, args, nullptr));
+        HIPCHK(hipModuleLaunchKernel(f, (unsigned)pl.nwg, 1, 1, (unsigned)pl.T_launch, 1, 1, (unsigned)plan_launch_lds(p, rq), st, args, nullptr));
         if (pl.split && c + 1 < pl.nchunks && (rc = launch_replay(p, rq, pl, a))) return rc;
     }
     return MCI_OK;
@@ -466,6 +466,23 @@
     return MCI_OK;
 }
 
+static int select_vegas_big(mci_problem *p, LaunchRequest &rq) {
+    if (vegas_big_rule(plan_big_in(p, rq, g_over, true)) != kBigTake) return MCI_OK;
+    if (p->vegas_big.state == 0) {
+        const int rc = compile_vegas_big(p);
+        if (rc == MCI_ERR_COMPILE || p->vegas_big.state == VegasBigUnit::kNoCompile) {
+            p->vegas_big.state = VegasBigUnit::kNoCompile;
+            fprintf(stderr, "mci: the big :vegas unit of this problem did not compile; big launches keep the standing unit\n%s\n", mci_last_error());
+            return MCI_OK;
+        }
+        if (rc) return rc;
+    }
+    if (p->vegas_big.state == 1 && !p->vegas_big.check_done)
+        if (int rc = vegas_check_gate(p, mci_problem::kVegasBig, rq.nevalperblock, rq.block_lo, rq.block_hi, rq.iteration, rq.seed, rq.measurefreq)) return rc;
+    if (vegas_big_rule(plan_big_in(p, rq, g_over, false)) == kBigTake) rq.kern = mci_problem::kVegasBig;
+    return MCI_OK;
+}
+
 int mci_iteration_run(mci_problem *p, int32_t solver, int64_t nevalperblock, int64_t block_lo, int64_t block_hi,
                       int32_t iteration, uint64_t seed, int64_t measurefreq, int64_t nchain, double thermal_ratio) {
     if (p->ctx->offline) return fail(MCI_ERR_NO_DEVICE, "offline context: no device to run on");
@@ -476,16 +493,19 @@
     if (p->has_fermik && solver != MCI_MCMC) return fail(MCI_ERR_INVALID, "FermiK variables work with solver=:mcmc only");
     if (p->strat.on) {
         if (solver != MCI_VEGAS) return fail(MCI_ERR_INVALID, "stratification works with solver = :vegas only (mci_set_stratification_off first)");
+        p->launch.last_vegas_big = false;
         return strat_run(p, nevalperblock, block_lo, block_hi, iteration, seed, measurefreq);
     }
     const int kern = (p->in_self_check && p->check_slot >= 0 && solver == MCI_VEGAS) ? p->check_slot : kslot(solver, measurefreq);
-    const LaunchRequest rq{solver, nevalperblock, block_lo, block_hi, nblocks, iteration, seed, measurefreq, thermal_ratio, nchain <= 0, kern};
-    int rc = (rq.solver == MCI_VEGAS || p->deterministic || p->shape.host_integrand || p->spec_lanes == 1) ? compile_solver(p, rq.kern) : MCI_OK;
+    LaunchRequest rq{solver, nevalperblock, block_lo, block_hi, nblocks, iteration, seed, measurefreq, thermal_ratio, nchain <= 0, kern};
+    auto compile_unit = [&]() { return rq.kern == mci_problem::kVegasBig ? MCI_OK : compile_solver(p, rq.kern); };
+    int rc = (rq.solver == MCI_VEGAS || p->deterministic || p->shape.host_integrand || p->spec_lanes == 1) ? compile_unit() : MCI_OK;
     if (rc) return rc;
     if (rq.solver == MCI_VEGAS && !p->in_self_check && !p->vegas_check_done[rq.kern == kSlotVegasAny ? 1 : 0] &&
         (rc = vegas_check_gate(p, rq.kern, rq.nevalperblock, rq.block_lo, rq.block_hi, rq.iteration, rq.seed, rq.measurefreq)))
         return rc;
-    if (rq.solver == MCI_VEGAS && (rc = compile_solver(p, rq.kern))) return rc;
+    if (rq.solver == MCI_VEGAS && (rc = compile_unit())) return rc;
+    if (rq.solver == MCI_VEGAS && !p->in_self_check && (rc = select_vegas_big(p, rq))) return rc;
     if (rq.solver == MCI_VEGAS && p->shape.host_integrand && (rc = ensure_dump(p))) return rc;
     if ((rc = flush_merge(p))) return rc;
     HIPCHK(hipSetDevice(p->ctx->device));
@@ -527,7 +547,7 @@
         pl.units = pl.nchain * pl.G;
         pl.T_launch = pl.units >= 256 ? 256 : (int)((pl.units + 63) / 64) * 64;
     }
-    if (pl.G == 1 && (rc = compile_solver(p, rq.kern))) return rc;
+    if (pl.G == 1 && (rc = compile_unit())) return rc;
     p->launch.last_spec_lanes = pl.G;
     p->launch.last_spec_maxacc = pl.spec_maxacc;
     plan_grid(p, rq, pl);
@@ -575,6 +595,7 @@
     if (s.host_measure && (rc = finish_host_measure(p, rq, pl))) return rc;
     record_launch(p, nblocks * nevalperblock, pl.nwg, pl.T_launch, nblocks);
     if (solver != MCI_VEGAS) p->launch.last_nchain = pl.nchain;
+    else p->launch.last_vegas_big = rq.kern == mci_problem::kVegasBig;
     return queue_merge(p, rq, pl, a.hold_hist);
 }
 
diff --git a/mcintegration.jl_amd/csrc/mci_host_jit.h b/mcintegration.jl_amd/csrc/mci_host_jit.h
--- a/mcintegration.jl_amd/csrc/mci_host_jit.h
+++ b/mcintegration.jl_amd/csrc/mci_host_jit.h
@@ -151,6 +151,57 @@
     return load_slot(p, slot, *chosen, lds);
 }
 
+static bool vegas_big_layout(const mci_problem *p) {
+    return vegas_pipe_unit(p) && p->vegas.hcopy_plan && p->vegas.hcopy_auto >= 8 && !g_over.hist_copies.on && !p->threads_explicit && sixteen_copies_fit_lds(p);
+}
+static int compile_vegas_big(mci_problem *p) {
+    VegasBigUnit &b = p->vegas_big;
+    if (b.state != 0) return MCI_OK;
+    if (int rc = default_measure_fits(p)) return rc;
+    mcijit::ProblemShape sh = p->shape;
+    sh.hcopy = kBigCopies;
+    sh.det = 0;
+    const std::string src = mcijit::generate_source(sh, MCI_VEGAS, mcijit::kUnitVegasMf1);
+    Candidate c[2];
+    for (int i = 0; i < 2; ++i) {
+        c[i].unit = mcijit::kUnitVegasMf1;
+        c[i].src = std::string(i == 0 ? kVgprKeys : "") + src;
+        c[i].threads = kBigThreads;
+    }
+    auto built = [](const Candidate &k) { return VegasBuilt{k.vgprs(), k.scratch(), true}; };
+    if (c[0].build()) {
+        b.state = VegasBigUnit::kNoCompile;
+        return c[0].failed(" (big :vegas unit)");
+    }
+    VegasBuilt with = built(c[0]), without{0, 0, false};
+    if (too_fat(with)) {
+        if (c[1].build()) {
+            b.state = VegasBigUnit::kNoCompile;
+            return c[1].failed(" (big :vegas unit)");
+        }
+        without = built(c[1]);
+    }
+    bool keys = false;
+    if (vegas_big_budget(with, without.ok ? &without : nullptr, &keys) != 1) {
+        b.state = VegasBigUnit::kOverBudget;
+        return MCI_OK;
+    }
+    const int64_t lds = sixteen_copies_lds(p);
+    if (int rc = p->kernel[mci_problem::kVegasBig].load(p->ctx, c[keys ? 0 : 1], "mci_vegas_batch", lds, kSlotRules)) {
+        b.state = VegasBigUnit::kNoCompile;
+        return rc;
+    }
+    if (!p->ctx->offline) {
+        int per_cu = 0, cus = 0;
+        HIPCHK(hipModuleOccupancyMaxActiveBlocksPerMultiprocessor(&per_cu, p->kernel[mci_problem::kVegasBig].f, kBigThreads, (size_t)lds));
+        HIPCHK(hipDeviceGetAttribute(&cus, hipDeviceAttributeMultiprocessorCount, p->ctx->device));
+        b.resident = per_cu * cus;
+    }
+    b.keys = keys;
+    b.state = 1;
+    return MCI_OK;
+}
+
 static int compile_spec(mci_problem *p, int solver) {
     const int slot = solver == MCI_VEGASMC ? kSlotVegasmcSpec : kSlotMcmcSpec;
     if (p->kernel[slot].compiled) return MCI_OK;
@@ -409,8 +460,10 @@
     else if (solver == MCI_VEGASMC_LANES || solver == MCI_MCMC_LANES) k = solver == MCI_VEGASMC_LANES ? kSlotVegasmcSpec : kSlotMcmcSpec, what = "the several-lanes-per-chain kernel";
     else if (solver == MCI_VEGAS_STRAT) k = mci_problem::kStrat, what = "the stratified :vegas kernel";
     else if (const int w = sweep_unit_of(solver); w >= 0) k = mci_problem::kSweep + w, what = std::string("the sweep kernel") + kSweepUnits[w].for_what;
+    else if (solver == MCI_VEGAS_BIG) k = mci_problem::kVegasBig, what = "the big :vegas unit";
     else if (solver < 0 || solver > 2) return fail(MCI_ERR_INVALID, "Solver %d is not supported!", solver);
-    else k = (solver == MCI_VEGAS && !p->kernel[solver].compiled && p->kernel[kSlotVegasAny].compiled) ? kSlotVegasAny : solver;
+    else if (solver == MCI_VEGAS && p->launch.last_vegas_big && p->kernel[mci_problem::kVegasBig].compiled) k = mci_problem::kVegasBig;
+    else k =(solver == MCI_VEGAS && !p->kernel[solver].compiled && p->kernel[kSlotVegasAny].compiled) ? kSlotVegasAny : solver;
     if (!p->kernel[k].compiled) return fail(MCI_ERR_INVALID, "%s has not been compiled yet", what.c_str());
     snprintf(buf, (size_t)n, "%s", p->kernel[k].code_object.c_str());
     return MCI_OK;
@@ -604,13 +657,21 @@
         }
         return compile_sweep_unit(p, w);
     }
+    if (solver == MCI_VEGAS_BIG) {
+        if (!vegas_big_layout(p)) return fail(MCI_ERR_INVALID, "this layout has no big :vegas unit (the eight-copy plan of the pipelined one-tile loop, sixteen copies within the CU's LDS)");
+        if (int rc = compile_vegas_big(p)) return rc;
+        if (p->vegas_big.state == VegasBigUnit::kOverBudget) return fail(MCI_ERR_COMPILE, "the big :vegas unit needs more than %ld VGPRs or scratch at 1024 threads: big launches keep the standing unit", kVgprsTwoWide);
+        if (p->vegas_big.state == VegasBigUnit::kNoCompile) return fail(MCI_ERR_COMPILE, "the big :vegas unit did not compile");
+        return MCI_OK;
+    }
     if (solver < 0 || solver > 2) return fail(MCI_ERR_INVALID, "Solver %d is not supported!", solver);
     return compile_solver(p, solver);
 }
 
 int mci_get_histogram_copies(const mci_problem *p, int32_t *copies) {
     if (!p || !copies) return fail(MCI_ERR_INVALID, "NULL argument");
-    *copies = (p->kernel[MCI_VEGAS].compiled || p->kernel[kSlotVegasAny].compiled) ? p->shape.hcopy : planned_hcopy(p, nullptr);
+    if (p->launch.last_vegas_big) *copies = kBigCopies;
+    else *copies = (p->kernel[MCI_VEGAS].compiled || p->kernel[kSlotVegasAny].compiled) ? p->shape.hcopy : planned_hcopy(p, nullptr);
     return MCI_OK;
 }
 
diff --git a/mcintegration.jl_amd/csrc/mci_host_plan.h b/mcintegration.jl_amd/csrc/mci_host_plan.h
--- a/mcintegration.jl_amd/csrc/mci_host_plan.h
+++ b/mcintegration.jl_amd/csrc/mci_host_plan.h
@@ -39,6 +39,39 @@
     if (rq.solver == MCI_VEGAS && p->vegas.wide && !p->vegas.threads_vegas && p->wg_per_block <= 0 && rq.nblocks * rq.nevalperblock < ((int64_t)1 << 22) &&
         rq.nblocks * rq.nevalperblock * p->shape.ndraw >= ((int64_t)1 << 19))
         pl.T = 512;
+    if (rq.kern == mci_problem::kVegasBig) pl.T = kBigThreads;
+}
+
+int64_t plan_launch_lds(const mci_problem *p, const LaunchRequest &rq) {
+    return rq.kern == mci_problem::kVegasBig ? sixteen_copies_lds(p) : solver_lds(p, rq.solver);
+}
+
+const int64_t kVegasBigSamples = (int64_t)1 << 26;
+const int kVegasBigAdds = 8;
+VegasBigIn plan_big_in(const mci_problem *p, const LaunchRequest &rq, const Overrides &ov, bool assume_unit) {
+    VegasBigIn in{};
+    in.vegas = rq.solver == MCI_VEGAS;
+    in.mf1 = rq.measurefreq == 1;
+    in.pipe_unit = !p->in_self_check && vegas_pipe_unit(p) && !(ov.vegas_cursor.on && ov.vegas_cursor.v == 0);
+    in.forced_grid = p->wg_per_block > 0;
+    in.deterministic = p->deterministic;
+    in.override_big = ov.vegas_big_unit.on ? (ov.vegas_big_unit.v != 0 ? 1 : 0) : -1;
+    in.cursor_forced = ov.vegas_cursor.on && ov.vegas_cursor.v == 1;
+    in.copy_plan = p->vegas.hcopy_plan;
+    in.conservative = p->vegas.conservative;
+    in.copies_forced = ov.hist_copies.on;
+    in.threads_explicit = p->threads_explicit;
+    in.copies = p->shape.hcopy;
+    in.threads = solver_threads(p, MCI_VEGAS);
+    in.sixteen_fit_lds = sixteen_copies_fit_lds(p);
+    in.samples = rq.nblocks * rq.nevalperblock;
+    in.threshold = kVegasBigSamples;
+    in.adds = vegas_adds_per_sample(p);
+    in.adds_floor = kVegasBigAdds;
+    in.nblocks = rq.nblocks;
+    in.resident = assume_unit ? rq.nblocks : p->vegas_big.resident;
+    in.state = assume_unit && p->vegas_big.state == 0 ? 1 : p->vegas_big.state;
+    return in;
 }
 
 bool plan_may_carry(const mci_problem *p, const LaunchRequest &rq) {
@@ -123,7 +156,7 @@
     return p->wg_per_block <= 0 && pl.units * rq.nblocks >= ((int64_t)1 << 25) ? 2 : 0;
 }
 void plan_cursor_grid(const LaunchRequest &rq, int resident, LaunchPlan &pl) {
-    if (resident >= rq.nblocks && (resident / rq.nblocks) * rq.nblocks > kAtomicRows) {
+    if (resident >= rq.nblocks && ((resident / rq.nblocks) * rq.nblocks > kAtomicRows || rq.kern == mci_problem::kVegasBig)) {
         pl.cursor = true;
         pl.wpb = (int)(resident / rq.nblocks);
         const int64_t maxw = (pl.units + pl.T - 1) / pl.T;
@@ -139,7 +172,8 @@
     pl.split = rq.solver == MCI_VEGAS && s.ntile > 1;
     if (!pl.split && pl.wpb * s.ntile > 4096 / rq.nblocks && s.ntile > 1) pl.wpb = (int)(4096 / rq.nblocks / s.ntile) > 0 ? (int)(4096 / rq.nblocks / s.ntile) : 1;
     pl.nrows = rq.nblocks * pl.wpb;
-    pl.atomic_flush = rq.solver == MCI_VEGAS && pl.hist_lds && s.ntile == 1 && atomic_rows_ok(p) && pl.nrows <= kAtomicRows && !s.host_integrand;
+    pl.atomic_flush = rq.solver == MCI_VEGAS && pl.hist_lds && s.ntile == 1 && atomic_rows_ok(p) && pl.nrows <= kAtomicRows && !s.host_integrand &&
+                      !(pl.cursor && rq.kern == mci_problem::kVegasBig);
     pl.nwg = pl.split ? pl.nrows : pl.nrows * s.ntile;
     pl.ghist_buffers = pl.atomic_flush ? (pl.nrows > 64 ? 3 : 1) : 0;
     pl.chunk_len = rq.nevalperblock;
diff --git a/mcintegration.jl_amd/csrc/mci_host_problem.h b/mcintegration.jl_amd/csrc/mci_host_problem.h
--- a/mcintegration.jl_amd/csrc/mci_host_problem.h
+++ b/mcintegration.jl_amd/csrc/mci_host_problem.h
@@ -465,9 +465,17 @@
     return MCI_OK;
 }
 
+static int64_t sixteen_copies_lds(const mci_problem *p) { return p->lds_bytes + (int64_t)p->shape.htile * 8 * (kBigCopies - 1); }
+static bool sixteen_copies_fit_lds(const mci_problem *p) { return sixteen_copies_lds(p) <= 159 * 1024; }
 static bool sixteen_copies_fit(const mci_problem *p) {
     const auto &s = p->shape;
-    return s.rng_bits == 32 && s.rng_rounds == 7 && p->lds_bytes + (int64_t)s.htile * 8 * 15 <= 159 * 1024;
+    return s.rng_bits == 32 && s.rng_rounds == 7 && sixteen_copies_fit_lds(p);
+}
+static int vegas_adds_per_sample(const mci_problem *p) {
+    const auto &s = p->shape;
+    int nadd = 0;
+    for (int k = 0; k < s.ndraw; ++k) nadd += (p->leaves[(size_t)s.draw_leaf[(size_t)k]].adapt && s.cover_mask[(size_t)k]) ? 1 : 0;
+    return nadd;
 }
 static int planned_hcopy(const mci_problem *p, int *threads) { return p->vegas.planned_copies(sixteen_copies_fit(p), threads); }
 
@@ -502,6 +510,10 @@
     return true;
 }
 static int cursor_resident(mci_problem *p, int kern, int threads, int *out) {
+    if (kern == mci_problem::kVegasBig) {
+        *out = p->vegas_big.resident;
+        return MCI_OK;
+    }
     hipFunction_t f = p->kernel[kern].f;
     const int64_t lds = solver_lds(p, MCI_VEGAS);
     if (f != p->cursor_occ_f || threads != p->cursor_occ_threads || lds != p->cursor_occ_lds) {
diff --git a/mcintegration.jl_amd/csrc/mci_host_types.h b/mcintegration.jl_amd/csrc/mci_host_types.h
--- a/mcintegration.jl_amd/csrc/mci_host_types.h
+++ b/mcintegration.jl_amd/csrc/mci_host_types.h
@@ -140,9 +140,10 @@
     DevBuf<double> d_scratch, d_iterlog, d_dump;
     DevBuf<int> d_status;
     DevBuf<mci::LeafDev> d_leaves;
-    enum { kSlots = 7, kPersist = kSlots, kStrat, kSweep, kKernels = kSweep + 7 };
+    enum { kSlots = 7, kPersist = kSlots, kStrat, kSweep, kVegasBig = kSweep + 7, kKernels = kVegasBig + 1 };
     KernelUnit kernel[kKernels];
     VegasKernelPlan vegas;
+    VegasBigUnit vegas_big;
     int spec_lanes = -1, spec_maxacc = -1;
     double spec_accept = 0.0;
     DevBuf<mci::SpecNode> d_spec_tab;
@@ -253,6 +254,7 @@
         int last_spec_lanes = 1, last_spec_maxacc = 0;
         bool last_carried = false;
         bool last_cursor = false;
+        bool last_vegas_big = false;
         int64_t last_split_chunks = 0, last_split_bytes = 0;
         int64_t launches = 0;
         bool time_this_launch = true;
@@ -320,7 +322,7 @@
         int chain_carry = 0;
     } sweep;
     KernelUnit &sweep_unit(int which) { return kernel[kSweep + which]; }
-    static_assert(kKernels == kSweep + Sweep::kUnits, "one handle per sweep unit");
+    static_assert(kVegasBig == kSweep + Sweep::kUnits, "one handle per sweep unit");
 };
 
 struct SweepUnitDesc {
@@ -356,7 +358,7 @@
 
 namespace {
 struct Override { bool on = false; int64_t v = 0; };
-struct Overrides { Override table_mode, hist_tile_bins, no_split_all, l1_phase, train_walk, hist_copies, fresh_floors, fresh_burnin_pct, spec_self_check, split_chunk, vegas_self_check, vegas_cursor, cursor_log2_big, cursor_ones; } g_over;
+struct Overrides { Override table_mode, hist_tile_bins, no_split_all, l1_phase, train_walk, hist_copies, fresh_floors, fresh_burnin_pct, spec_self_check, split_chunk, vegas_self_check, vegas_cursor, cursor_log2_big, cursor_ones, vegas_big_unit; } g_over;
 Override *override_slot(const char *key) {
     if (!key) return nullptr;
     if (!strcmp(key, "table_mode")) return &g_over.table_mode;
@@ -373,6 +375,7 @@
     if (!strcmp(key, "vegas_cursor")) return &g_over.vegas_cursor;
     if (!strcmp(key, "cursor_log2_big")) return &g_over.cursor_log2_big;
     if (!strcmp(key, "cursor_ones")) return &g_over.cursor_ones;
+    if (!strcmp(key, "vegas_big_unit")) return &g_over.vegas_big_unit;
     return nullptr;
 }
 }
@@ -581,6 +584,8 @@
 
 void drop_modules(mci_problem *p) {
     p->vegas.modules_dropped();
+    p->vegas_big.modules_dropped();
+    p->launch.last_vegas_big = false;
     p->vegas_check_done[0] = p->vegas_check_done[1] = false;
     p->cursor_occ_f = nullptr;
     for (KernelUnit &u : p->kernel) u.drop();
diff --git a/mcintegration.jl_amd/csrc/mci_host_vegas_plan.h b/mcintegration.jl_amd/csrc/mci_host_vegas_plan.h
--- a/mcintegration.jl_amd/csrc/mci_host_vegas_plan.h
+++ b/mcintegration.jl_amd/csrc/mci_host_vegas_plan.h
@@ -135,4 +135,55 @@
     return 0;
 }
 
+const int kBigCopies = 16, kBigThreads = 1024;
+struct VegasBigUnit {
+    enum { kOverBudget = -1, kFailedCheck = -2, kNoCompile = -3 };
+    int state = 0;
+    bool keys = false;
+    bool check_done = false;
+    int resident = 0;
+    void modules_dropped() { *this = VegasBigUnit(); }
+};
+struct VegasBigIn {
+    bool vegas, mf1;
+    bool pipe_unit;
+    bool forced_grid, deterministic;
+    int override_big;
+    bool cursor_forced;
+    bool copy_plan;
+    bool conservative, copies_forced, threads_explicit;
+    int copies, threads;
+    bool sixteen_fit_lds;
+    long long samples, threshold;
+    int adds, adds_floor;
+    long long nblocks, resident;
+    int state;
+};
+enum VegasBigRefusal {
+    kBigTake = 0, kBigNotMf1, kBigNoCursor, kBigForcedGrid, kBigDeterministic, kBigOverrideOff, kBigStandingPlan, kBigLds, kBigSmall, kBigFewAdds,
+    kBigNotResident, kBigOverBudget, kBigFailedCheck, kBigNoCompile
+};
+inline VegasBigRefusal vegas_big_rule(const VegasBigIn &in) {
+    const bool forced_on = in.override_big == 1 && in.cursor_forced;
+    if (!in.vegas || !in.mf1) return kBigNotMf1;
+    if (!in.pipe_unit) return kBigNoCursor;
+    if (in.deterministic) return kBigDeterministic;
+    if (in.override_big == 0) return kBigOverrideOff;
+    if (in.forced_grid && !forced_on) return kBigForcedGrid;
+    if (!in.copy_plan || in.conservative || in.copies_forced || in.threads_explicit || in.copies < 8 || in.threads != 512) return kBigStandingPlan;
+    if (!in.sixteen_fit_lds) return kBigLds;
+    if (!forced_on && in.samples < in.threshold) return kBigSmall;
+    if (!forced_on && in.adds < in.adds_floor) return kBigFewAdds;
+    if (in.state == VegasBigUnit::kOverBudget) return kBigOverBudget;
+    if (in.state == VegasBigUnit::kFailedCheck) return kBigFailedCheck;
+    if (in.state == VegasBigUnit::kNoCompile) return kBigNoCompile;
+    if (!forced_on && in.resident < in.nblocks) return kBigNotResident;
+    return kBigTake;
 }
+inline int vegas_big_budget(const VegasBuilt &with_keys, const VegasBuilt *without, bool *keys) {
+    *keys = !too_fat(with_keys);
+    if (*keys) return 1;
+    return without && !too_fat(*without) ? 1 : VegasBigUnit::kOverBudget;
+}
+
+}
diff --git a/mcintegration.jl_amd/engine.py b/mcintegration.jl_amd/engine.py
--- a/mcintegration.jl_amd/engine.py
+++ b/mcintegration.jl_amd/engine.py
@@ -401,7 +401,7 @@
     @staticmethod
     def _kernel_code(solver):
         return {"vegas_persistent": 3, "vegasmc_lanes": 5, "mcmc_lanes": 6, "vegas_strat": 7, "vegas_sweep": 8, "vegas_sweep_leaves": 9, "vegas_sweep_strat": 10,
-                "vegasmc_sweep": 11, "mcmc_sweep": 12, "vegasmc_sweep_carry": 13, "mcmc_sweep_carry": 14}.get(solver) or _lib.SOLVERS[solver]
+                "vegasmc_sweep": 11, "mcmc_sweep": 12, "vegasmc_sweep_carry": 13, "mcmc_sweep_carry": 14, "vegas_big": 15}.get(solver) or _lib.SOLVERS[solver]
 
     def compile(self, solver="vegas"):
         check(lib().mci_compile_solver(self.p, self._kernel_code(solver)))
diff --git a/mcintegration.jl_amd/integrate.py b/mcintegration.jl_amd/integrate.py
--- a/mcintegration.jl_amd/integrate.py
+++ b/mcintegration.jl_amd/integrate.py
@@ -614,6 +614,8 @@
     for cfg, f, meas in jobs:
         eng = Engine(cfg, f, measure=meas, device=-1)
         eng.compile("vegas")
+        if n == 1:
+            eng.compile("vegas_big")
         if meas is not None:
             eng.compile("vegasmc")
             eng.compile("vegasmc_lanes")
```
